# neonnnnn/sparsepoly

Hardware: AMD Instinct MI355X
Metric: pcd_epochs_per_sec (higher is better)
Workload: dtype f32; 1 GPU; BASELINE configs[1]: degree=2 n_components=30 regularizer=squaredl12 solver=pcd fit_linear=True fit_lower=explicit on 1000000x100000 CSR nnz=49987865 (~50/row); schedule=colored, parallelism=single GPU, ranks=1, launcher=external, persistent_fallbacks=0

## Files before the change

### include/spfm.h

```cpp
#ifndef SPFM_H
#define SPFM_H

#include <stdint.h>

#ifdef __cplusplus
extern "C" {
#endif

typedef struct spfm_engine* spfm_handle;

#define SPFM_OK 0
#define SPFM_ERR_INVALID (-1)
#define SPFM_ERR_RUNTIME (-2)
#define SPFM_ERR_UNSUPPORTED (-3)

#define SPFM_F32 0
#define SPFM_F64 1

#define SPFM_LOSS_SQUARED 0
#define SPFM_LOSS_SQUARED_HINGE 1
#define SPFM_LOSS_LOGISTIC 2

#define SPFM_REG_L1 0
#define SPFM_REG_L21 1
#define SPFM_REG_SQUAREDL12 2
#define SPFM_REG_SQUAREDL21 3
#define SPFM_REG_OMEGATI 4
#define SPFM_REG_OMEGACS 5

#define SPFM_SOLVER_PCD 0
#define SPFM_SOLVER_PBCD 1
#define SPFM_SOLVER_PSGD 2

#define SPFM_SCHED_EXACT 0
#define SPFM_SCHED_COLORED 1
#define SPFM_SCHED_COLORED_RLF 2

#define SPFM_MAX_DEGREE 6

int spfm_create(spfm_handle* out, int device_id, int dtype);
void spfm_destroy(spfm_handle h);
const char* spfm_last_error(spfm_handle h);
int spfm_device_name(spfm_handle h, char* out, int cap);
const char* spfm_build_tag(void);

int spfm_set_data_csc(spfm_handle h, int64_t n, int32_t d, const int64_t* indptr,
                      const int32_t* indices, const double* data, const double* y);

int spfm_set_data_csr(spfm_handle h, int64_t n, int32_t d, const int64_t* indptr,
                      const int32_t* indices, const double* data, const double* y);

int spfm_share_data(spfm_handle dst, spfm_handle src, const double* y);

int spfm_set_params(spfm_handle h, int n_orders, int k, int32_t d, const double* P,
                    const double* w, const double* lams);
int spfm_get_params(spfm_handle h, double* P, double* w);

int spfm_configure(spfm_handle h, int solver, int loss, int regularizer, int top_degree);

int spfm_init_pred(spfm_handle h, int degree, int fit_linear, int add_lower_deg2);
int spfm_get_y_pred(spfm_handle h, double* out);
int spfm_loss_sum(spfm_handle h, double* out);

int spfm_predict_csr(spfm_handle h, int64_t n, const int64_t* indptr, const int32_t* indices,
                     const double* data, int degree, int fit_linear, int add_lower_deg2,
                     double* out);

int spfm_set_schedule(spfm_handle h, int mode, const int32_t* indices_feature,
                      const int64_t* conflict_indptr, const int32_t* conflict_indices,
                      int64_t conflict_n_rows, int32_t* order_out, int32_t* n_batches_out);

int spfm_set_schedule_raw(spfm_handle h, const int32_t* order, const int32_t* batch_ptr,
                          int32_t n_batches, const int64_t* conflict_indptr,
                          const int32_t* conflict_indices, int64_t conflict_n_rows);

int spfm_get_schedule(spfm_handle h, int32_t* order_out, int32_t* batch_ptr_out,
                      int32_t* n_batches_out);

int spfm_schedule_build(int mode, int64_t n_rows, int32_t d, const int64_t* indptr,
                        const int32_t* indices, const int32_t* indices_feature, int max_batch,
                        int32_t* order_out, int32_t* batch_ptr_out, int32_t* n_batches_out);


int spfm_cd_linear_epoch(spfm_handle h, double alpha, double* viol);

int spfm_pcd_epoch(spfm_handle h, int order_idx, int degree, double beta, double gamma,
                   double eta, const int32_t* indices_component, int n_comp, double* viol);

int spfm_pbcd_epoch(spfm_handle h, int order_idx, int degree, double beta, double gamma,
                    double eta, double* viol);

int spfm_host_epoch_begin(spfm_handle h, int order_idx, int degree);
int spfm_host_pass_begin(spfm_handle h, int component);
int spfm_host_step_sums(spfm_handle h, int step, double* sums_out);
int spfm_host_step_apply(spfm_handle h, int step, const double* p_new, const double* p_old);
int spfm_host_epoch_end(spfm_handle h, double* viol);

int spfm_psgd_epoch(spfm_handle h, int degree, double alpha, double beta, double gamma,
                    double eta0, int learning_rate, double power_t, int64_t batch_size,
                    const int32_t* indices_samples, int64_t n_samples, int fit_linear,
                    int64_t* it, double* sum_loss);
int spfm_psgd_epoch_sharded(spfm_handle h, int degree, double alpha, double beta, double gamma,
                            double eta0, int learning_rate, double power_t, int64_t batch_size,
                            const int32_t* indices_samples, int64_t n_global, int64_t row_lo,
                            int fit_linear, int64_t* it, double* sum_loss);

int spfm_comm_unique_id(char* id128);
int spfm_comm_init(spfm_handle h, const char* id128, int n_ranks, int rank);
int spfm_comm_init_shm(spfm_handle h, const char* shm_name, int n_ranks, int rank);

int spfm_peer_alloc(spfm_handle h, char* handle64);
int spfm_peer_connect(spfm_handle h, int n_ranks, int rank, const char* handles);

int spfm_profile_enable(spfm_handle h, int on);
int spfm_profile_get(spfm_handle h, int which, double* ms, int64_t* launches, int64_t* nnz);
int spfm_profile_reset(spfm_handle h);
int spfm_set_use_graph(spfm_handle h, int on);

int spfm_set_option(spfm_handle h, const char* key, int value);
int spfm_get_option(spfm_handle h, const char* key, int* value);


int spfm_debug_prb_stamps(spfm_handle h, long long* out, int cap);
int spfm_debug_hop_latency(spfm_handle h, int partner, int rounds, double* ns_per_hop,
                           int* xcc_ids);
int spfm_debug_exchange_cost(spfm_handle h, int groups, int ncols, int readers_mod, int rounds,
                             double* ns_per_round);

int spfm_debug_stream_probe(spfm_handle h, int64_t* bytes_out);
int spfm_debug_write_probe(spfm_handle h, int bytes_per_record, int64_t* bytes_out);
int spfm_debug_branch_counts(spfm_handle h, unsigned* out8, int reset);

#define SPFM_GRAM_ANOVA 0
#define SPFM_GRAM_POLY 1
#define SPFM_GRAM_ALL_SUBSETS 2
#define SPFM_GRAM_MAX_DEGREE 64

int spfm_gram_csr_dense(spfm_handle h, int kind, int degree, int64_t n1, int32_t d,
                        const int64_t* indptr, const int32_t* indices, const double* data,
                        int64_t n2, const double* B, const double* lams, int transpose_out,
                        int64_t max_block_bytes, double* out);
int spfm_gram_csr_csr(spfm_handle h, int kind, int degree, int64_t n1, int32_t d,
                      const int64_t* indptr1, const int32_t* indices1, const double* data1,
                      int64_t n2, const int64_t* indptr2, const int32_t* indices2,
                      const double* data2, const double* lams, int64_t max_block_bytes,
                      double* out);

int spfm_objective_terms(spfm_handle h, int order_idx, int degree, double* out8);

int spfm_set_eval_csr(spfm_handle h, int64_t n, int32_t d, const int64_t* indptr,
                      const int32_t* indices, const double* data, const double* y);
int spfm_eval_loss(spfm_handle h, int degree, int fit_linear, int add_lower_deg2,
                   double* loss_sum, double* y_pred_out);

#define SPFM_INTERACTION_BLOCK_MAX_BYTES (1LL << 30)
int spfm_interaction_stats(spfm_handle h, int order_idx, double tol, int64_t* counts2,
                           double* sums3);
int spfm_interaction_topk(spfm_handle h, int order_idx, int64_t K, int32_t* rows, int32_t* cols,
                          double* vals, int64_t* n_out);
int spfm_interaction_list(spfm_handle h, int order_idx, double tol, int64_t capacity,
                          int32_t* rows, int32_t* cols, double* vals, int64_t* n_out);
int spfm_interaction_values(spfm_handle h, int order_idx, int64_t L, const int32_t* rows,
                            const int32_t* cols, double* vals);
int spfm_interaction_block(spfm_handle h, int order_idx, int64_t nJ, const int32_t* J,
                           int64_t nJ2, const int32_t* J2, double* out);

#define SPFM_INTERACTION3_MAX_ACTIVE (1 << 15)
int spfm_interaction3_stats(spfm_handle h, int order_idx, double tol, int64_t* counts2,
                            double* sums3);
int spfm_interaction3_topk(spfm_handle h, int order_idx, int64_t K, int32_t* i, int32_t* j,
                           int32_t* l, double* vals, int64_t* n_out);
int spfm_interaction3_list(spfm_handle h, int order_idx, double tol, int64_t capacity, int32_t* i,
                           int32_t* j, int32_t* l, double* vals, int64_t* n_out);
int spfm_interaction3_values(spfm_handle h, int order_idx, int64_t L, const int32_t* i,
                             const int32_t* j, const int32_t* l, double* vals);

#ifdef __cplusplus
}
#endif
#endif
```

### sparsepoly_amd/_capi.py

```python
import ctypes as C
import os

import numpy as np



def hip_initialised():
    try:
        for fd in os.listdir("/proc/self/fd"):
            try:
                if os.readlink("/proc/self/fd/" + fd) == "/dev/kfd":
                    return True
            except OSError:
                continue
    except OSError:
        pass
    return False


HIP_INITIALISED_BEFORE_IMPORT = hip_initialised()
QUEUES_SET_BY_PACKAGE = False


def ensure_hw_queues(n_streams):
    global QUEUES_SET_BY_PACKAGE
    import warnings

    need = int(n_streams) + 1
    val = os.environ.get("GPU_MAX_HW_QUEUES")
    have = int(val) if (val and val.isdigit()) else None
    if not hip_initialised():
        if have is None:
            os.environ["GPU_MAX_HW_QUEUES"] = "8"
            QUEUES_SET_BY_PACKAGE = True
            have = 8
        return have
    eff = have if have is not None else 4
    if eff < need and n_streams > 1:
        warnings.warn(
            "sparsepoly_amd: %d concurrent fits, but the HIP runtime of this process was "
            "initialised with %d hardware queues (GPU_MAX_HW_QUEUES %s): fits that share a queue "
            "run one after the other.  Export GPU_MAX_HW_QUEUES=8 before the process first "
            "touches the GPU (PyTorch users: before the first torch.cuda call)."
            % (n_streams, eff, "= %d" % have if have is not None else "unset"),
            RuntimeWarning, stacklevel=3)
    return eff


_HERE = os.path.dirname(os.path.abspath(__file__))
LIB_PATH = os.environ.get("SPFM_HIP_LIB") or os.path.join(_HERE, "lib", "libspfm_hip.so")

SPFM_OK, SPFM_ERR_INVALID, SPFM_ERR_RUNTIME, SPFM_ERR_UNSUPPORTED = 0, -1, -2, -3
DTYPES = {"f32": 0, "f64": 1}
LOSSES = {"squared": 0, "squared_hinge": 1, "logistic": 2}
REGULARIZERS = {"l1": 0, "l21": 1, "squaredl12": 2, "squaredl21": 3, "omegati": 4, "omegacs": 5}
SOLVERS = {"pcd": 0, "pbcd": 1, "psgd": 2}
LEARNING_RATE = {"constant": 0, "optimal": 1, "pegasos": 2, "invscaling": 3}
SCHEDULES = {"exact": 0, "colored": 1, "colored_rlf": 2}
GRAM_KINDS = {"anova": 0, "poly": 1, "all-subsets": 2}
GRAM_MAX_DEGREE = 64

SYMBOLS = [
    "spfm_create", "spfm_destroy", "spfm_last_error", "spfm_device_name", "spfm_build_tag", "spfm_set_data_csc", "spfm_set_data_csr", "spfm_share_data",
    "spfm_set_params", "spfm_get_params", "spfm_configure", "spfm_init_pred", "spfm_get_y_pred",
    "spfm_loss_sum", "spfm_predict_csr", "spfm_set_schedule", "spfm_set_schedule_raw",
    "spfm_get_schedule", "spfm_schedule_build",
    "spfm_cd_linear_epoch",
    "spfm_pcd_epoch", "spfm_pbcd_epoch", "spfm_psgd_epoch", "spfm_psgd_epoch_sharded",
    "spfm_host_epoch_begin",
    "spfm_host_pass_begin", "spfm_host_step_sums", "spfm_host_step_apply", "spfm_host_epoch_end", "spfm_comm_unique_id", "spfm_comm_init", "spfm_comm_init_shm", "spfm_peer_alloc", "spfm_peer_connect",
    "spfm_profile_enable", "spfm_profile_get", "spfm_profile_reset", "spfm_set_use_graph",
    "spfm_set_option", "spfm_get_option", "spfm_debug_prb_stamps", "spfm_debug_hop_latency", "spfm_debug_exchange_cost",
    "spfm_debug_branch_counts", "spfm_debug_stream_probe", "spfm_debug_write_probe",
    "spfm_gram_csr_dense", "spfm_gram_csr_csr",
    "spfm_objective_terms", "spfm_set_eval_csr", "spfm_eval_loss",
    "spfm_interaction_stats", "spfm_interaction_topk", "spfm_interaction_list",
    "spfm_interaction_values", "spfm_interaction_block",
    "spfm_interaction3_stats", "spfm_interaction3_topk", "spfm_interaction3_list",
    "spfm_interaction3_values",
]
INTERACTION_BLOCK_MAX_BYTES = 1 << 30
INTERACTION3_MAX_ACTIVE = 1 << 15

_dp = C.POINTER(C.c_double)
_ip = C.POINTER(C.c_int32)
_lp = C.POINTER(C.c_int64)
_h = C.c_void_p

_lib = None


def load():
    global _lib
    if _lib is not None:
        return _lib
    if not os.path.exists(LIB_PATH):
        raise RuntimeError(
            "sparsepoly_amd: HIP extension %s is missing. Build it with "
            "`python -c 'import __graft_entry__ as g; g.build()'` or "
            "`bash sparsepoly_amd/csrc/build.sh`; there is no CPU fallback." % LIB_PATH
        )
    L = C.CDLL(LIB_PATH)
    L.spfm_create.argtypes = [C.POINTER(_h), C.c_int, C.c_int]
    L.spfm_destroy.argtypes = [_h]
    L.spfm_destroy.restype = None
    L.spfm_last_error.argtypes = [_h]
    L.spfm_last_error.restype = C.c_char_p
    L.spfm_device_name.argtypes = [_h, C.c_char_p, C.c_int]
    L.spfm_build_tag.argtypes = []
    L.spfm_build_tag.restype = C.c_char_p
    L.spfm_set_data_csc.argtypes = [_h, C.c_int64, C.c_int32, _lp, _ip, _dp, _dp]
    L.spfm_set_data_csr.argtypes = [_h, C.c_int64, C.c_int32, _lp, _ip, _dp, _dp]
    L.spfm_share_data.argtypes = [_h, _h, _dp]
    L.spfm_set_params.argtypes = [_h, C.c_int, C.c_int, C.c_int32, _dp, _dp, _dp]
    L.spfm_get_params.argtypes = [_h, _dp, _dp]
    L.spfm_configure.argtypes = [_h, C.c_int, C.c_int, C.c_int, C.c_int]
    L.spfm_init_pred.argtypes = [_h, C.c_int, C.c_int, C.c_int]
    L.spfm_get_y_pred.argtypes = [_h, _dp]
    L.spfm_loss_sum.argtypes = [_h, _dp]
    L.spfm_predict_csr.argtypes = [_h, C.c_int64, _lp, _ip, _dp, C.c_int, C.c_int, C.c_int, _dp]
    L.spfm_set_schedule.argtypes = [_h, C.c_int, _ip, _lp, _ip, C.c_int64, _ip, _ip]
    L.spfm_set_schedule_raw.argtypes = [_h, _ip, _ip, C.c_int32, _lp, _ip, C.c_int64]
    L.spfm_get_schedule.argtypes = [_h, _ip, _ip, _ip]
    L.spfm_schedule_build.argtypes = [C.c_int, C.c_int64, C.c_int32, _lp, _ip, _ip, C.c_int, _ip,
                                      _ip, _ip]
    L.spfm_cd_linear_epoch.argtypes = [_h, C.c_double, _dp]
    L.spfm_pcd_epoch.argtypes = [_h, C.c_int, C.c_int, C.c_double, C.c_double, C.c_double, _ip,
                                 C.c_int, _dp]
    L.spfm_pbcd_epoch.argtypes = [_h, C.c_int, C.c_int, C.c_double, C.c_double, C.c_double, _dp]
    L.spfm_psgd_epoch.argtypes = [_h, C.c_int, C.c_double, C.c_double, C.c_double, C.c_double,
                                  C.c_int, C.c_double, C.c_int64, _ip, C.c_int64, C.c_int, _lp,
                                  _dp]
    L.spfm_psgd_epoch_sharded.argtypes = [_h, C.c_int, C.c_double, C.c_double, C.c_double,
                                          C.c_double, C.c_int, C.c_double, C.c_int64, _ip,
                                          C.c_int64, C.c_int64, C.c_int, _lp, _dp]
    L.spfm_host_epoch_begin.argtypes = [_h, C.c_int, C.c_int]
    L.spfm_host_pass_begin.argtypes = [_h, C.c_int]
    L.spfm_host_step_sums.argtypes = [_h, C.c_int, _dp]
    L.spfm_host_step_apply.argtypes = [_h, C.c_int, _dp, _dp]
    L.spfm_host_epoch_end.argtypes = [_h, _dp]
    L.spfm_comm_unique_id.argtypes = [C.c_char_p]
    L.spfm_comm_init.argtypes = [_h, C.c_char_p, C.c_int, C.c_int]
    L.spfm_comm_init_shm.argtypes = [_h, C.c_char_p, C.c_int, C.c_int]
    L.spfm_profile_enable.argtypes = [_h, C.c_int]
    L.spfm_profile_get.argtypes = [_h, C.c_int, _dp, _lp, _lp]
    L.spfm_profile_reset.argtypes = [_h]
    L.spfm_set_use_graph.argtypes = [_h, C.c_int]
    L.spfm_set_option.argtypes = [_h, C.c_char_p, C.c_int]
    L.spfm_get_option.argtypes = [_h, C.c_char_p, C.POINTER(C.c_int)]
    L.spfm_debug_prb_stamps.argtypes = [_h, _lp, C.c_int]
    L.spfm_debug_hop_latency.argtypes = [_h, C.c_int, C.c_int, _dp, _ip]
    L.spfm_debug_exchange_cost.argtypes = [_h, C.c_int, C.c_int, C.c_int, C.c_int, _dp]
    L.spfm_peer_alloc.argtypes = [_h, C.c_char_p]
    L.spfm_peer_connect.argtypes = [_h, C.c_int, C.c_int, C.c_char_p]
    L.spfm_debug_branch_counts.argtypes = [_h, C.POINTER(C.c_uint32), C.c_int]
    L.spfm_debug_stream_probe.argtypes = [_h, _lp]
    L.spfm_debug_write_probe.argtypes = [_h, C.c_int, _lp]
    L.spfm_gram_csr_dense.argtypes = [_h, C.c_int, C.c_int, C.c_int64, C.c_int32, _lp, _ip, _dp,
                                      C.c_int64, _dp, _dp, C.c_int, C.c_int64, _dp]
    L.spfm_gram_csr_csr.argtypes = [_h, C.c_int, C.c_int, C.c_int64, C.c_int32, _lp, _ip, _dp,
                                    C.c_int64, _lp, _ip, _dp, _dp, C.c_int64, _dp]
    L.spfm_objective_terms.argtypes = [_h, C.c_int, C.c_int, _dp]
    L.spfm_set_eval_csr.argtypes = [_h, C.c_int64, C.c_int32, _lp, _ip, _dp, _dp]
    L.spfm_eval_loss.argtypes = [_h, C.c_int, C.c_int, C.c_int, _dp, _dp]
    L.spfm_interaction_stats.argtypes = [_h, C.c_int, C.c_double, _lp, _dp]
    L.spfm_interaction_topk.argtypes = [_h, C.c_int, C.c_int64, _ip, _ip, _dp, _lp]
    L.spfm_interaction_list.argtypes = [_h, C.c_int, C.c_double, C.c_int64, _ip, _ip, _dp, _lp]
    L.spfm_interaction_values.argtypes = [_h, C.c_int, C.c_int64, _ip, _ip, _dp]
    L.spfm_interaction_block.argtypes = [_h, C.c_int, C.c_int64, _ip, C.c_int64, _ip, _dp]
    L.spfm_interaction3_stats.argtypes = [_h, C.c_int, C.c_double, _lp, _dp]
    L.spfm_interaction3_topk.argtypes = [_h, C.c_int, C.c_int64, _ip, _ip, _ip, _dp, _lp]
    L.spfm_interaction3_list.argtypes = [_h, C.c_int, C.c_double, C.c_int64, _ip, _ip, _ip, _dp,
                                         _lp]
    L.spfm_interaction3_values.argtypes = [_h, C.c_int, C.c_int64, _ip, _ip, _ip, _dp]
    for name in SYMBOLS:
        f = getattr(L, name)
        if name not in ("spfm_destroy", "spfm_last_error", "spfm_build_tag"):
            f.restype = C.c_int
    _lib = L
    return L


def f64(a):
    a = np.ascontiguousarray(a, dtype=np.float64)
    return a, a.ctypes.data_as(_dp)


def i32(a):
    a = np.ascontiguousarray(a, dtype=np.int32)
    return a, a.ctypes.data_as(_ip)


def i64(a):
    a = np.ascontiguousarray(a, dtype=np.int64)
    return a, a.ctypes.data_as(_lp)


def build_tag():
    return load().spfm_build_tag().decode()
```

### sparsepoly_amd/csrc/spfm_engine.hip.h

```cpp
#pragma once
#include <dlfcn.h>
#include <fcntl.h>
#include <sys/mman.h>
#include <unistd.h>
#include <chrono>
#include <hip/hip_runtime.h>

#include <cerrno>
#include <cmath>
#include <cstdio>
#include <cstdlib>
#include <cstring>
#include <atomic>
#include <map>
#include <memory>
#include <mutex>
#include <string>
#include <type_traits>
#include <thread>
#include <vector>

#include "../../include/spfm.h"
#include "spfm_common.hip.h"
#include "spfm_prb.hip.h"
#include "spfm_pcdw.hip.h"
#include "spfm_psgd.hip.h"

namespace spfm {
struct IntArgs;
void schedule_exact(int64_t, int32_t, const int64_t*, const int32_t*, const int32_t*, int,
                    std::vector<int32_t>&);
void schedule_colored(int64_t, int32_t, const int64_t*, const int32_t*, const int32_t*, int,
                      std::vector<int32_t>&, std::vector<int32_t>&);
void schedule_rlf(int64_t, int32_t, const int64_t*, const int32_t*, const int32_t*, int,
                  std::vector<int32_t>&, std::vector<int32_t>&);
bool csr_to_csc(int64_t, int32_t, const int64_t*, const int32_t*, std::vector<int64_t>&,
                std::vector<int32_t>&, std::vector<int64_t>&);
int schedule_threads();
void csc_to_csr(int64_t, int32_t, const int64_t*, const int32_t*, std::vector<int64_t>&,
                std::vector<int32_t>&, std::vector<int64_t>&);
void build_wide_stream(int64_t, const int64_t*, const int32_t*, const std::vector<int32_t>&,
                       const std::vector<int32_t>&, int, std::vector<int32_t>&,
                       std::vector<int32_t>&, std::vector<int32_t>&, std::vector<uint8_t>&);
void build_pb_stream(int64_t, const int64_t*, const int32_t*, const std::vector<int32_t>&,
                     const std::vector<int32_t>&, int, int, bool, const uint8_t*,
                     std::vector<int32_t>&, std::vector<int32_t>&, std::vector<uint8_t>&,
                     std::vector<uint8_t>&);
void build_rowblock_stream(int64_t, const int64_t*, const int32_t*, const std::vector<int32_t>&,
                           const std::vector<int32_t>&, int, int, std::vector<int32_t>&,
                           std::vector<int32_t>&, std::vector<uint32_t>&, const uint8_t*);
void schedule_relax(int64_t, int32_t, const int64_t*, const int32_t*, const int32_t*, int, int,
                    std::vector<int32_t>&, std::vector<int32_t>&, std::vector<int32_t>&,
                    std::vector<int32_t>&, std::vector<int64_t>&, std::vector<int64_t>&,
                    std::vector<int16_t>&, std::vector<uint8_t>&);
template <typename T>
hipError_t device_csr_to_csc(int64_t, int32_t, int64_t, const int64_t*, const int32_t*, const T*,
                             int64_t*, int32_t*, T*, int*, hipStream_t);
extern template hipError_t device_csr_to_csc<float>(int64_t, int32_t, int64_t, const int64_t*,
                                                    const int32_t*, const float*, int64_t*,
                                                    int32_t*, float*, int*, hipStream_t);
extern template hipError_t device_csr_to_csc<double>(int64_t, int32_t, int64_t, const int64_t*,
                                                     const int32_t*, const double*, int64_t*,
                                                     int32_t*, double*, int*, hipStream_t);
hipError_t device_rowblock_stream(int64_t, int32_t, int64_t, int, int, int, const int32_t*,
                                  const int32_t*, const int64_t*, const int32_t*, const uint8_t*,
                                  int32_t*, int32_t*, uint32_t*, int*, int64_t*, hipStream_t);
hipError_t device_pb_stream(int64_t, int32_t, int64_t, int, int, int, int, const int32_t*,
                            const int32_t*, const int64_t*, const int32_t*, const int64_t*,
                            const int32_t*, int32_t*, int32_t*, uint8_t*, uint8_t*, hipStream_t);
hipError_t device_wide_stream(int64_t, int32_t, int64_t, int, int, const int32_t*, const int32_t*,
                              const int64_t*, const int32_t*, const int64_t*, const int32_t*,
                              int32_t*, int32_t*, uint8_t*, hipStream_t);
hipError_t device_first_fit(int64_t, int32_t, int64_t, const int64_t*, const int32_t*, const int64_t*,
                            const int32_t*, int, int32_t*, int*, int*, hipStream_t);
hipError_t device_rlf(int64_t, int32_t, int64_t, const int64_t*, const int32_t*, const int64_t*,
                      const int32_t*, int, std::vector<int32_t>&, std::vector<int32_t>&, int*,
                      hipStream_t);
}

using namespace spfm;
struct IntPass;

typedef struct ncclComm* ncclComm_t;

struct DevBuf {
    struct Block {
        void* p;
        std::atomic<int> refs;
    };
    Block* blk = nullptr;
    void* p = nullptr;
    size_t bytes = 0;
    DevBuf() = default;
    DevBuf(const DevBuf&) = delete;
    DevBuf& operator=(const DevBuf&) = delete;
    ~DevBuf() { release(); }
    void release() {
        if (blk && blk->refs.fetch_sub(1) == 1) {
            (void)hipFree(blk->p);
            delete blk;
        }
        blk = nullptr;
        p = nullptr;
        bytes = 0;
    }
    bool shared() const { return blk && blk->refs.load() > 1; }
    hipError_t alloc(size_t b) {
        if (b <= bytes && p && !shared()) return hipSuccess;
        release();
        if (b == 0) b = 16;
        void* q = nullptr;
        hipError_t e = hipMalloc(&q, b);
        if (e != hipSuccess) return e;
        blk = new Block{q, {1}};
        p = q;
        bytes = b;
        return e;
    }
    void share(const DevBuf& o) {
        if (o.blk == blk) return;
        release();
        if (!o.blk) return;
        o.blk->refs.fetch_add(1);
        blk = o.blk;
        p = o.p;
        bytes = o.bytes;
    }
    template <typename U>
    U* as() const {
        return reinterpret_cast<U*>(p);
    }
};

#define HIPC(expr)                                                                       \
    do {                                                                                 \
        hipError_t _e = (expr);                                                          \
        if (_e != hipSuccess) {                                                          \
            err = std::string(#expr) + ": " + hipGetErrorString(_e);                     \
            return SPFM_ERR_RUNTIME;                                                     \
        }                                                                                \
    } while (0)

#define FAIL(code, msg) \
    do {                \
        err = (msg);    \
        return (code);  \
    } while (0)

#define SPFM_TRY(call)       \
    do {                     \
        int _rc = (call);    \
        if (_rc) return _rc; \
    } while (0)

#define SPFM_GUARD(h)                              \
    if (!(h)) return SPFM_ERR_INVALID;             \
    if (hipSetDevice((h)->device) != hipSuccess) { \
        (h)->err = "hipSetDevice failed";          \
        return SPFM_ERR_RUNTIME;                   \
    }

#define SPFM_DISPATCH(dt, ...)                                    \
    ((dt) == SPFM_F32 ? [&] { using T = float; __VA_ARGS__; }()   \
                      : [&] { using T = double; __VA_ARGS__; }())

static inline unsigned cdiv(int64_t a, int64_t b) { return (unsigned)((a + b - 1) / b); }

struct StreamCache {
    std::mutex mu;
    struct Prb {
        std::string key;
        DevBuf sp, erow, eval, lmask;
        int has_long = 0;
    };
    struct Pb {
        std::string key;
        DevBuf sp, erow, eval, meta, tab;
    };
    std::vector<std::unique_ptr<Prb>> prb;
    std::vector<std::unique_ptr<Pb>> pb;
    static constexpr size_t kKeep = 2;
};

struct ProfSlot {
    std::vector<hipEvent_t> ev;
    size_t used = 0;
    double ms = 0.0;
    int64_t launches = 0, nnz = 0;
};

struct spfm_engine {
    int device = 0, dtype = SPFM_F32;
    hipStream_t stream = nullptr;
    std::string err;
    std::string devname;

    int64_t n = 0, nnz = 0;
    int d = 0;
    bool have_data = false;
    DevBuf cptr, cidx, cval, rptr, ridx, rval, yy, A, col_norm;
    std::vector<int64_t> h_cptr;
    std::vector<int32_t> h_cidx;
    bool col_norm_reduced = false;
    std::shared_ptr<StreamCache> scache;
    uint64_t sched_hash = 0;
    int share_data_from(spfm_engine* src, const double* y);

    int n_orders = 0, k = 0;
    bool have_params = false;
    DevBuf P, Pt, w, lams;
    bool p_valid = true, pt_valid = false;
    std::vector<double> h_lams;

    int solver = -1, loss = 0, reg = 0, top_degree = 0;
    bool configured = false;
    DevBuf norms, cache, dcache;

    std::vector<int32_t> order, batch_ptr;
    DevBuf d_order, d_desc;
    int max_batch_cols = 0;
    bool have_schedule = false;
    int64_t sched_version = 0;

    DevBuf part, delta, pold, viol_col, scalar, ctl, comp_order, pred_tmp, partial, pb_scal,
        pb_ticket;
    bool pbcd_fuse = true;
    double* h_scalar = nullptr;

    DevBuf sg_gradP, sg_gradw, sg_samples, sg_part, sg_cond, sg_thr, sg_theta, sg_done,
        sg_norms, sg_conv, sg_sched, sg_idx, sg_snapP, sg_snapw, sg_snapc;
    bool psgd_force_eager = false;
    int psgd_graph_sweeps = 4;
    bool psgd_warm = false;
    int psgd_redone = 0;
    std::vector<PsgdBatch> h_sched;

    bool use_graph = true;
    bool fuse_chain = true;
    int max_batch_opt = 4096;

    bool pers_failed = false;
    int pers_fallbacks = 0;
    std::string pers_reason;
    int spin_max = 1 << 21;
    int debug_drop = 0;
    bool keep_last_error = false;
    bool have_pred_args = false;
    int pa_degree = 0, pa_lin = 0, pa_lower = 0;
    DevBuf snapP, snapW, snapC;
    std::map<const void*, int> resident_cache;
    std::map<std::string, bool> resident_agreed;

    bool persistent = true;
    int prb_G = 64;
    bool prb_lds = true;
    int prb_lds_active = 0;
    bool y_pm1 = false;
    bool prb_ready = false;
    int prb_has_long = 0;
    int prb_long = kPrbLong;
    DevBuf prb_sp, prb_erow, prb_eval, prb_slab, prb_abort, prow_old, d_bptr, prb_stamps,
        prb_viol, prb_cn, prb_lmask, prb_rec;
    bool prb_pack = true;
    int prb_pack_active = 0;
    bool prb_stamp_on = false;
    int wide_min_cols = 110;
    bool wide_stamp_on = false;
    DevBuf wide_stamps;
    DevBuf w_rec;
    static constexpr size_t kPrbLds = 84 * 1024;
    bool relax_on = true;
    int relax_state = 0;
    std::vector<int32_t> r_batch_ptr;
    int relax_has_long = 0;
    DevBuf r_bptr, r_sp, r_erow, r_eval, r_lmask, r_cfptr, r_cf, r_clist, r_cslab;
    bool wide_on = true;
    int pcdw_G = 0;
    bool wide_ready = false;
    int wide_G = 0, wide_tot = 0;
    int wide_lr_active = 0;
    int wide_lds_cap = -1;
    bool wide_ep = true;
    int wide_ep_active = 0;
    bool wide_rec8 = true;
    DevBuf w_wbase, w_wsp, w_erow, w_eval, w_slabA, w_slabB;
    bool pb_persistent = true;
    int pbprb_G = 256;
    int probe_xcd = 0, probe_lds = 60 * 1024;
    bool pb_stream_ready = false;
    int pb_stream_G = 0, pb_stream_NG = 0;
    DevBuf pb_tab;
    int pbr_state = 0;
    int pbr_G = 0, pb_relax_active = 0;
    std::vector<int32_t> pbr_batch_ptr;
    DevBuf pbr_bptr, pbr_sp, pbr_erow, pbr_eval, pbr_meta, pbr_tab, pbr_cfptr, pbr_cf, pbr_clist,
        pbr_slabR;
    bool pb_balance = true;
    DevBuf pb_sp, pb_erow, pb_eval, pb_meta, pb_slabA, pb_slabB, pb_slabC, pb_stamps, pb_rec;
    bool pb_stamp_on = false;
    int pbprb_active = 0;
    int pb_dbg = 0;
    DevBuf pb_dbgbuf;
    std::map<std::string, hipGraphExec_t> graphs;

    ncclComm_t comm = nullptr;
    struct ShmComm {
        static constexpr size_t kMaxDoubles = 1 << 16;
        struct Hdr {
            volatile int arrive;
            volatile int sense;
            int pad[14];
        };
        Hdr* hdr = nullptr;
        double* slots = nullptr;
        size_t bytes = 0;
        int local_sense = 0;
    } shm;
    std::vector<double> shm_host;
    bool dist() const { return comm != nullptr || shm.hdr != nullptr; }
    int n_ranks = 1, rank = 0;
    static constexpr size_t kPeerPcdOff = 0, kPeerPbOff = 16 * 1024;
    static constexpr size_t kPeerProbeOff = kPeerPbOff + (size_t)2 * 64 * 8 * 64;
    static constexpr size_t kPeerDoubles = kPeerProbeOff + 64;
    int peer_generation = 0;
    void* peer_own = nullptr;
    std::vector<void*> peer_ptr;
    DevBuf peer_tab_pcd, peer_tab_pb;
    bool peer_ready = false;

    bool prof_on = false;
    ProfSlot prof[5];

    ~spfm_engine();

    void clear_graphs() {
        for (auto& kv : graphs) (void)hipGraphExecDestroy(kv.second);
        graphs.clear();
    }

    enum : unsigned {
        kInvPrbStream = 1,
        kInvPbStream = 2,
        kInvWideStream = 4,
        kInvRelax = 8,
        kInvPbRelax = 16,
        kInvSchedule = 32,
        kInvGraphs = 64,
        kInvStreams = kInvPrbStream | kInvPbStream | kInvWideStream,
    };
    void invalidate(unsigned mask) {
        if (mask & kInvPrbStream) prb_ready = false;
        if (mask & kInvPbStream) pb_stream_ready = false;
        if (mask & kInvWideStream) wide_ready = false;
        if (mask & kInvRelax) relax_state = 0;
        if (mask & kInvPbRelax) pbr_state = 0;
        if (mask & kInvSchedule) have_schedule = false;
        if (mask & kInvGraphs) clear_graphs();
    }

    RegState regstate() {
        RegState rs;
        rs.norms = norms.as<double>();
        rs.cache = cache.as<double>();
        rs.dcache = dcache.as<double>();
        return rs;
    }

    size_t tsize() const { return dtype == SPFM_F32 ? 4 : 8; }

    int sync() {
        HIPC(hipStreamSynchronize(stream));
        return SPFM_OK;
    }

    template <typename U>
    int upload_to(void* dst, const U* src, size_t count) {
        if (count) HIPC(hipMemcpyAsync(dst, src, sizeof(U) * count, hipMemcpyHostToDevice, stream));
        return SPFM_OK;
    }
    template <typename U>
    int upload(DevBuf& b, const U* src, size_t count, size_t min_count = 0) {
        HIPC(b.alloc(sizeof(U) * std::max(count, min_count)));
        return upload_to(b.p, src, count);
    }
    template <typename U>
    int download(U* dst, const void* src, size_t count) {
        if (count) HIPC(hipMemcpyAsync(dst, src, sizeof(U) * count, hipMemcpyDeviceToHost, stream));
        return SPFM_OK;
    }

    template <typename T>
    int stage_csr_rows(DevBuf& rp, DevBuf& ri, DevBuf& rv, std::vector<T>& hv,
                       const int64_t* indptr, const int32_t* indices, const double* data,
                       int64_t r0, int64_t r1, size_t min_entries = 0) {
        const int64_t e0 = r0 ? indptr[r0] : 0, ne = indptr[r1] - e0;
        const T* vals;
        if constexpr (std::is_same<T, double>::value) {
            vals = data + e0;
        } else {
            hv.resize((size_t)ne);
            const int nt = (ne >= (1 << 20)) ? schedule_threads() : 1;
            const int64_t per = (ne + nt - 1) / nt;
            auto work = [&](int tid) {
                const int64_t lo = per * tid, hi = std::min<int64_t>(ne, lo + per);
                for (int64_t ii = lo; ii < hi; ++ii) hv[(size_t)ii] = (T)data[e0 + ii];
            };
            std::vector<std::thread> pool;
            for (int t = 1; t < nt; ++t) pool.emplace_back(work, t);
            work(0);
            for (auto& th : pool) th.join();
            vals = hv.data();
        }
        SPFM_TRY(upload(rp, indptr + r0, (size_t)(r1 - r0 + 1)));
        SPFM_TRY(upload(ri, indices + e0, (size_t)ne, min_entries));
        return upload(rv, vals, (size_t)ne, min_entries);
    }

    template <typename T>
    int upload_targets(const double* y, std::vector<T>& hy) {
        hy.resize((size_t)n * 2);
        for (int64_t i = 0; i < n; ++i) {
            hy[(size_t)2 * i] = (T)0;
            hy[(size_t)2 * i + 1] = (T)y[i];
        }
        return upload_to(yy.p, hy.data(), hy.size());
    }

    struct BlockView {
        const double* base;
        int64_t ss, sj;
    };
    BlockView live_block(int order_idx) const {
        const double* img = p_valid ? P.as<double>() : Pt.as<double>();
        return {img + (size_t)order_idx * k * d, p_valid ? (int64_t)d : 1, p_valid ? 1 : (int64_t)k};
    }

    static constexpr size_t kProfPool = 32768;
    bool prof_armed = false;
    void prof_begin(int which, int64_t nnz_launch) {
        prof_armed = false;
        if (!prof_on) return;
        ProfSlot& ps = prof[which];
        if (ps.used + 2 > kProfPool) return;
        if (ps.used + 2 > ps.ev.size()) {
            hipEvent_t a, b;
            if (hipEventCreate(&a) != hipSuccess) return;
            if (hipEventCreate(&b) != hipSuccess) {
                (void)hipEventDestroy(a);
                return;
            }
            ps.ev.push_back(a);
            ps.ev.push_back(b);
        }
        ps.launches++;
        ps.nnz += nnz_launch;
        (void)hipEventRecord(ps.ev[ps.used], stream);
        prof_armed = true;
    }
    void prof_cancel(int which, int64_t nnz_launch) {
        if (!prof_armed) return;
        prof[which].launches--;
        prof[which].nnz -= nnz_launch;
        prof_armed = false;
    }
    void prof_end(int which) {
        if (!prof_armed) return;
        ProfSlot& ps = prof[which];
        (void)hipEventRecord(ps.ev[ps.used + 1], stream);
        ps.used += 2;
        prof_armed = false;
    }
    void prof_collect() {
        if (!prof_on) return;
        (void)hipStreamSynchronize(stream);
        for (auto& ps : prof) {
            for (size_t i = 0; i + 1 < ps.used; i += 2) {
                float ms = 0.f;
                if (hipEventElapsedTime(&ms, ps.ev[i], ps.ev[i + 1]) == hipSuccess) ps.ms += ms;
            }
            ps.used = 0;
        }
    }

    int64_t batch_nnz(int b) const {
        int64_t s = 0;
        for (int q = batch_ptr[b]; q < batch_ptr[b + 1]; ++q)
            s += h_cptr[order[q] + 1] - h_cptr[order[q]];
        return s;
    }

    int shm_barrier();

    int allreduce_shm(double* buf, size_t count);
    int allreduce_shm_piece(double* buf, size_t count);

    int allreduce(double* buf, size_t count);

    int ensure_col_norm();

    int ensure_p();
    int ensure_pt();

    template <typename F>
    int run_cached(const std::string& key, F&& body) {
// ... 19 lines not shown
            if (e != hipSuccess) {
                err = std::string("hipGraphInstantiate: ") + hipGetErrorString(e);
                return SPFM_ERR_RUNTIME;
            }
            it = graphs.emplace(key, ge).first;
        }
        HIPC(hipGraphLaunch(it->second, stream));
        return SPFM_OK;
    }

    template <typename T>
    int upload_images(const int64_t* h_cp, const int32_t* h_ci, const int64_t* h_rp,
                      const int32_t* h_ri, const double* data_csc, const double* data_csr,
                      const int64_t* perm, const double* y);

    template <typename T>
    int set_data_t(const int64_t* indptr, const int32_t* indices, const double* data,
                   const double* y);

    int data_installed(const double* y);

    bool ingest_device = true;
    int ingest_device_used = 0;
    int co_tenants = 1;
    static constexpr int kIngestFallback = 2;
    template <typename T>
    int set_data_csr_device(const int64_t* indptr, const int32_t* indices, const double* data,
                            const double* y);

    int set_data_csr(int64_t n_, int32_t d_, const int64_t* indptr, const int32_t* indices,
                     const double* data, const double* y);

    int set_data(int64_t n_, int32_t d_, const int64_t* indptr, const int32_t* indices,
                 const double* data, const double* y);

    int set_params(int n_orders_, int k_, int32_t d_, const double* P_, const double* w_,
                   const double* lams_);

    int get_params(double* P_, double* w_);

    int configure(int solver_, int loss_, int reg_, int top_degree_);

    int alloc_work();

    bool colour_device = true;
    int colour_device_used = 0;
    bool stream_device = true;
    int stream_device_used = 0;
    int pb_stream_device_used = 0, wide_stream_device_used = 0;
    int colour_columns(int mode, int64_t rows, const int64_t* cp, const int32_t* ci, bool own,
                       const int32_t* jf, int max_batch);

    int set_schedule(int mode, const int32_t* indices_feature, const int64_t* cf_indptr,
                     const int32_t* cf_indices, int64_t cf_rows, int32_t* order_out,
                     int32_t* n_batches_out);

    int install_schedule();

    int set_schedule_raw(const int32_t* order_in, const int32_t* bptr_in, int32_t nb,
                         const int64_t* cf_indptr, const int32_t* cf_indices, int64_t cf_rows);

    int n_batches() const { return (int)batch_ptr.size() - 1; }

    template <typename T, int M>
    void launch_anova(int64_t rows, const int64_t* rp, const int32_t* ri, const T* rv,
                      const double* Pt_o, double* out);
    template <typename T>
    int anova_dispatch(int M, int64_t rows, const int64_t* rp, const int32_t* ri, const T* rv,
                       const double* Pt_o, double* out);

    template <typename T>
    int output_t(int64_t rows, const int64_t* rp, const int32_t* ri, const T* rv, int degree,
                 int fit_linear, int add_lower, double* out);

    template <typename T>
    int init_pred_t(int degree, int fit_linear, int add_lower);

    int init_pred(int degree, int fit_linear, int add_lower);

    template <typename T>
    int get_y_pred_t(double* out);

    template <typename T>
    int loss_sum_t(double* out);

    template <typename T>
    int predict_csr_t(int64_t rows, const int64_t* indptr, const int32_t* indices,
                      const double* data, int degree, int fit_linear, int add_lower,
                      double* out);

    int epoch_prologue();

    int epoch_epilogue(double* viol);

    static std::string fkey(const char* tag, std::initializer_list<double> v,
                            std::initializer_list<int64_t> iv) {
        std::string s(tag);
        char buf[64];
        for (double x : v) {
            snprintf(buf, sizeof buf, "|%a", x);
            s += buf;
        }
        for (int64_t x : iv) {
            snprintf(buf, sizeof buf, "|%lld", (long long)x);
            s += buf;
        }
        return s;
    }

    template <typename T>
    int lin_body(double alpha);

    template <typename T, int LOSS>
    int lin_prb(double alpha);
    template <typename T>
    int lin_prb_loss(double alpha);

    void mark_not_resident(const char* what) {
        pers_failed = true;
        pers_fallbacks += 1;
        pers_reason = std::string(what) + ": its workgroups cannot all be resident on this device";
        if (getenv("SPFM_VERBOSE")) fprintf(stderr, "spfm: fall-back: %s\n", pers_reason.c_str());
    }

    int cd_linear_epoch(double alpha, double* viol);

    template <typename T, int M>
    int pcd_pass_body(int order_idx, double beta, double gamma, double eta);

    bool prb_usable() const {
        return persistent && !pers_failed && (!dist() || peer_ready) && max_batch_cols <= 64 &&
               nnz < ((int64_t)1 << 31) && n > 0;
    }

    bool resident_ok(const void* fn, int threads, size_t lds, int G);
    static constexpr int kNotResident = 1;
    int launch_groups(int G) {
        if (debug_drop > 0 && G > 1) {
            --debug_drop;
            return G - 1;
        }
        return G;
    }
    int snapshot_state(const double* params, size_t count, DevBuf& dst);
    int persistent_aborted(bool* out);
    int recover_from_abort(double* params, size_t count, const DevBuf& src, const char* what);

    template <typename T>
    int ensure_prb();
    template <typename T>
    int build_prb_stream(int nb_);

    PrbArgs prb_args();

    bool relax_candidate() const {
        return relax_on && prb_usable() && !dist() && n_batches() > 0 &&
               (double)d / (double)n_batches() < 12.0;
    }
    template <typename T>
    int ensure_relax();
    PrbArgs relax_args();

    template <typename T, int M, int LOSS>
    int pcd_pass_prb(int order_idx, double beta, double gamma, double eta);

    template <typename T, int M>
    int pcd_prb_loss(int order_idx, double beta, double gamma, double eta);

    template <typename T>
    int pcd_prb_dispatch(int M, int order_idx, double beta, double gamma, double eta);

    int peer_clear(size_t off_doubles, size_t n_doubles);
    int host_barrier();

    bool wide_usable() const {
        return persistent && !pers_failed && wide_on && (!dist() || peer_ready) &&
               max_batch_cols > 64 && max_batch_cols <= 512 && nnz < ((int64_t)1 << 31) && n > 0;
    }

    int wide_groups(int ncu, size_t lds_max) const;

    template <typename T>
    int ensure_wide();

    PcdwArgs wide_args();

    template <typename T, int KIND>
    int wide_launch(PcdwArgs& a, PcdwParams& pp, T* Aptr);

    template <typename T>
    int pcd_pass_wide(int order_idx, double beta, double gamma, double eta);

    template <typename T>
    int lin_wide(double alpha);

    static int kind_of(int degree) { return degree == -1 ? 0 : degree; }
    bool degree_ok(int degree) const {
        return top_degree == -1 ? degree == -1 : (degree >= 2 && degree <= top_degree);
    }

    template <typename T, int M>
    int pcd_precompute_all(int order_idx);
    template <typename T>
    int pcd_precompute_all_dispatch(int M, int order_idx);

    template <typename T>
    int pcd_pass_dispatch(int M, int order_idx, double beta, double gamma, double eta);

    int pcd_epoch(int order_idx, int degree, double beta, double gamma, double eta,
                  const int32_t* ic, int n_comp, double* viol);

    template <typename T, int M, int L, int C>
    int pbcd_body_lc(int order_idx, double beta, double gamma, double eta);

    static bool pbprb_degree_ok(int M) { return M == 0 || M == 2 || M == 3 || M == 4; }
    bool pbprb_usable(int M) const {
        return persistent && !pers_failed && pb_persistent && (!dist() || peer_ready) &&
               max_batch_cols <= 64 && nnz < ((int64_t)1 << 31) && n > 0 && k <= 62 &&
               pbprb_degree_ok(M);
    }

    const char* validate_pb_stream(int G, int NG, const std::vector<int32_t>& gsp,
                                   const std::vector<int32_t>& src,
                                   const std::vector<uint8_t>& meta,
                                   const std::vector<uint8_t>& tab) const;

    template <typename T>
    int ensure_pb_stream(int NG);
    template <typename T>
    int ensure_pb_relax(int NG);

    template <typename T, int M, int L>
    int pbcd_prb_l(int order_idx, double beta, double gamma, double eta);

    template <typename T, int M>
    int pbcd_prb_m(int order_idx, double beta, double gamma, double eta);

    template <typename T>
    int pbcd_prb_dispatch(int M, int order_idx, double beta, double gamma, double eta);

    template <typename T, int M>
    int pbcd_body(int order_idx, double beta, double gamma, double eta);

    template <typename T>
    int pbcd_dispatch(int M, int order_idx, double beta, double gamma, double eta);

    int pbcd_epoch(int order_idx, int degree, double beta, double gamma, double eta,
                   double* viol);

    int host_order = -1, host_degree = 0;
    std::vector<double> host_stage;

    int host_epoch_begin(int order_idx, int degree);
    template <typename T>
    int host_pbcd_precompute(int M, int order_idx);
    int host_pass_begin(int s);
    int host_step_check(int b) {
        if (host_order < 0) FAIL(SPFM_ERR_INVALID, "host step: call spfm_host_epoch_begin first");
        if (b < 0 || b >= n_batches()) FAIL(SPFM_ERR_INVALID, "host step: step index out of range");
        return SPFM_OK;
    }

    template <typename T, int M>
    int host_sums_pcd(int b, double* out);
    template <typename T, int M>
    int host_apply_pcd(int b, const double* p_new);
    template <typename T, int M, int L, int C>
    int host_sums_pbcd(int b, double* out);
    template <typename T, int M, int L, int C>
    int host_apply_pbcd(int b, const double* p_new, const double* p_old);
    template <typename T>
    int host_step_pcd_t(bool sums, int b, double* out, const double* p_new);
    template <typename T>
    int host_step_pbcd_t(bool sums, int b, double* out, const double* p_new, const double* p_old);
    int host_step(bool sums, int b, double* out, const double* p_new, const double* p_old);
    int host_epoch_end(double* viol);

    int configure_psgd(int loss_, int reg_, int top_degree_);

    static void psgd_eta(int lr, double eta0, double alpha, double beta, double power_t,
                         int64_t it, double* eta_P, double* eta_w) {
        if (lr == 0) {
            *eta_P = eta0;
            *eta_w = eta0;
        } else if (lr == 1) {
            const double eta_it = eta0 * (double)it;
            *eta_P = eta0 / std::pow(1.0 + eta_it * beta, power_t);
            *eta_w = eta0 / std::pow(1.0 + eta_it * alpha, power_t);
        } else if (lr == 2) {
            *eta_P = 1.0 / (beta * (double)it);
            *eta_w = 1.0 / (alpha * (double)it);
        } else {
            const double eta = eta0 / std::pow((double)it, power_t);
            *eta_P = eta;
            *eta_w = eta;
        }
    }

    template <typename T, int L>
    int psgd_epoch_tl(int degree, double alpha, double beta, double gamma, double eta0, int lr,
                      double power_t, int64_t batch_size, int fit_linear, int64_t* it);

    int psgd_epoch(int degree, double alpha, double beta, double gamma, double eta0, int lr,
                   double power_t, int64_t batch_size, const int32_t* indices_samples,
                   int64_t n_samples, int64_t row_lo, int fit_linear, int64_t* it, double* sum_loss);
    std::vector<int64_t> sg_lpos;
// ... 95 lines not shown
```

### sparsepoly_amd/csrc/spfm_engine_core.hip

```cpp
#include "spfm_engine.hip.h"
#include "spfm_linear.hip.h"
#include "spfm_predict.hip.h"
#include "spfm_pbcd.hip.h"

using namespace spfm;

static thread_local std::string g_create_error;

namespace {
struct ncclUniqueId_ {
    char internal[128];
};
enum { ncclSum_ = 0 };
enum { ncclFloat64_ = 8 };
struct Rccl {
    void* lib = nullptr;
    int (*GetUniqueId)(ncclUniqueId_*) = nullptr;
    int (*CommInitRank)(ncclComm_t*, int, ncclUniqueId_, int) = nullptr;
    int (*AllReduce)(const void*, void*, size_t, int, int, ncclComm_t, hipStream_t) = nullptr;
    int (*CommDestroy)(ncclComm_t) = nullptr;
    const char* (*GetErrorString)(int) = nullptr;
    const char* (*GetLastError)(ncclComm_t) = nullptr;
    int (*GetVersion)(int*) = nullptr;
    std::string path;
// ... 756 lines not shown
    SPFM_TRY(download(out, o.p, (size_t)rows));
    return sync();
}

int spfm_engine::epoch_prologue() {
    if (!have_data || !have_params || !configured)
        FAIL(SPFM_ERR_INVALID, "epoch: data, parameters and configuration are required");
    if (!have_schedule) FAIL(SPFM_ERR_INVALID, "epoch: call spfm_set_schedule first");
    int rc = ensure_col_norm();
    if (rc) return rc;
    HIPC(hipMemsetAsync(viol_col.p, 0, sizeof(double) * (size_t)d, stream));
    return SPFM_OK;
}

int spfm_engine::epoch_epilogue(double* viol) {
    hipLaunchKernelGGL(reduce_sum_kernel, dim3(1), dim3(kBlock), 0, stream,
                       viol_col.as<double>(), d, scalar.as<double>());
    HIPC(hipGetLastError());
    SPFM_TRY(download(h_scalar, scalar.p, 1));
    HIPC(hipStreamSynchronize(stream));
    prof_collect();
    if (viol) *viol = h_scalar[0];
    return SPFM_OK;
}

bool spfm_engine::resident_ok(const void* fn, int threads, size_t lds, int G) {
    int per_cu = 0;
    auto it = resident_cache.find(fn);
    if (it != resident_cache.end()) {
        per_cu = it->second;
    } else {
        if (hipOccupancyMaxActiveBlocksPerMultiprocessor(&per_cu, fn, threads, lds) !=
            hipSuccess) {
            (void)hipGetLastError();
            per_cu = 1;
        }
        resident_cache[fn] = per_cu;
    }
    int ncu = 0;
    if (hipDeviceGetAttribute(&ncu, hipDeviceAttributeMultiprocessorCount, device) != hipSuccess)
        return true;
    const int64_t sharers = (int64_t)(shm.hdr ? n_ranks : 1) * co_tenants;
    const bool mine = (int64_t)per_cu * ncu >= (int64_t)G * sharers;
    if (!dist()) return mine;
    char key[96];
    snprintf(key, sizeof key, "%p|%d|%lld|%zu", fn, G, (long long)sharers, lds);
    auto ag = resident_agreed.find(key);
    if (ag != resident_agreed.end()) return ag->second;
    double no = mine ? 0.0 : 1.0;
    bool agreed = mine;
    double* slot = scalar.as<double>() + 7;
    if (scalar.p && upload_to(slot, &no, 1) == SPFM_OK && sync() == SPFM_OK &&
        allreduce(slot, 1) == SPFM_OK && download(&no, slot, 1) == SPFM_OK && sync() == SPFM_OK)
        agreed = no == 0.0;
    resident_agreed[key] = agreed;
    return agreed;
}

int spfm_engine::snapshot_state(const double* params, size_t count, DevBuf& dst) {
    HIPC(dst.alloc(sizeof(double) * count));
    HIPC(hipMemcpyAsync(dst.p, params, sizeof(double) * count, hipMemcpyDeviceToDevice, stream));
    const size_t nc = kMaxDegree + 2;
    HIPC(snapC.alloc(sizeof(double) * nc * 3));
    HIPC(hipMemcpyAsync(snapC.p, cache.p, sizeof(double) * nc * 2, hipMemcpyDeviceToDevice,
                        stream));
    HIPC(hipMemcpyAsync(snapC.as<double>() + nc * 2, dcache.p, sizeof(double) * nc,
                        hipMemcpyDeviceToDevice, stream));
    return SPFM_OK;
}

int spfm_engine::persistent_aborted(bool* out) {
    *out = false;
    if (!prb_abort.p) return SPFM_OK;
    unsigned flag = 0;
    SPFM_TRY(download(&flag, prb_abort.p, 1));
    HIPC(hipStreamSynchronize(stream));
    double any = flag ? 1.0 : 0.0;
    if (dist()) {
        double* slot = scalar.as<double>() + 6;
        SPFM_TRY(upload_to(slot, &any, 1));
        HIPC(hipStreamSynchronize(stream));
        SPFM_TRY(allreduce(slot, 1));
        SPFM_TRY(download(&any, slot, 1));
        HIPC(hipStreamSynchronize(stream));
    }
    if (flag) HIPC(hipMemsetAsync(prb_abort.p, 0, sizeof(unsigned) * 4, stream));
    *out = any != 0.0;
    return SPFM_OK;
}

int spfm_engine::recover_from_abort(double* params, size_t count, const DevBuf& src, const char* what) {
    pers_failed = true;
    pers_fallbacks += 1;
    pers_reason = std::string(what) +
                  " timed out waiting for its workgroups (not all resident, or a peer GPU "
                  "did not answer)";
    if (getenv("SPFM_VERBOSE")) fprintf(stderr, "spfm: fall-back: %s\n", pers_reason.c_str());
    if (!have_pred_args)
        FAIL(SPFM_ERR_RUNTIME, pers_reason + "; the model is half-updated (no spfm_init_pred "
                                             "call to recompute y_pred from)");
    const size_t nc = kMaxDegree + 2;
    HIPC(hipMemcpyAsync(params, src.p, sizeof(double) * count, hipMemcpyDeviceToDevice, stream));
    HIPC(hipMemcpyAsync(cache.p, snapC.p, sizeof(double) * nc * 2, hipMemcpyDeviceToDevice,
                        stream));
    HIPC(hipMemcpyAsync(dcache.p, snapC.as<double>() + nc * 2, sizeof(double) * nc,
                        hipMemcpyDeviceToDevice, stream));
    clear_graphs();
    return init_pred(pa_degree, pa_lin, pa_lower);
}

int spfm_engine::peer_clear(size_t off_doubles, size_t n_doubles) {
    if (!peer_ready) return SPFM_OK;
    HIPC(hipMemsetAsync(reinterpret_cast<double*>(peer_own) + off_doubles, 0,
                        sizeof(double) * n_doubles, stream));
    HIPC(hipStreamSynchronize(stream));
    return host_barrier();
}

int spfm_engine::host_barrier() {
    if (shm.hdr) return shm_barrier();
    if (comm) {
        int rc = allreduce(scalar.as<double>() + 4, 1);
        if (rc) return rc;
        HIPC(hipStreamSynchronize(stream));
    }
    return SPFM_OK;
}

extern "C" {

int spfm_create(spfm_handle* out, int device_id, int dtype) {
    if (!out) return SPFM_ERR_INVALID;
    *out = nullptr;
    if (dtype != SPFM_F32 && dtype != SPFM_F64) {
        g_create_error = "dtype must be SPFM_F32 or SPFM_F64";
        return SPFM_ERR_INVALID;
    }
    int ndev = 0;
    hipError_t e = hipGetDeviceCount(&ndev);
    if (e != hipSuccess || ndev == 0) {
        g_create_error = std::string("no HIP device available: ") + hipGetErrorString(e);
        return SPFM_ERR_RUNTIME;
    }
    if (device_id < 0 || device_id >= ndev) {
        g_create_error = "device id out of range";
        return SPFM_ERR_INVALID;
    }
    if ((e = hipSetDevice(device_id)) != hipSuccess) {
        g_create_error = std::string("hipSetDevice: ") + hipGetErrorString(e);
        return SPFM_ERR_RUNTIME;
    }
    spfm_engine* h = new spfm_engine();
    h->device = device_id;
    h->dtype = dtype;
    hipDeviceProp_t prop;
    if (hipGetDeviceProperties(&prop, device_id) == hipSuccess) h->devname = prop.gcnArchName;
    if ((e = hipStreamCreateWithFlags(&h->stream, hipStreamNonBlocking)) != hipSuccess) {
        g_create_error = std::string("hipStreamCreate: ") + hipGetErrorString(e);
        delete h;
        return SPFM_ERR_RUNTIME;
    }
    *out = h;
    return SPFM_OK;
}

void spfm_destroy(spfm_handle h) {
    if (!h) return;
    (void)hipSetDevice(h->device);
    (void)hipStreamSynchronize(h->stream);
    delete h;
}

const char* spfm_last_error(spfm_handle h) { return h ? h->err.c_str() : g_create_error.c_str(); }

#ifndef SPFM_BUILD_TAG
#define SPFM_BUILD_TAG "untagged"
#endif
const char* spfm_build_tag(void) { return SPFM_BUILD_TAG; }

int spfm_device_name(spfm_handle h, char* out, int cap) {
    if (!h || !out || cap <= 0) return SPFM_ERR_INVALID;
    snprintf(out, (size_t)cap, "%s", h->devname.c_str());
    return SPFM_OK;
}

int spfm_set_data_csc(spfm_handle h, int64_t n, int32_t d, const int64_t* indptr,
                      const int32_t* indices, const double* data, const double* y) {
    SPFM_GUARD(h);
    return h->set_data(n, d, indptr, indices, data, y);
}

int spfm_set_data_csr(spfm_handle h, int64_t n, int32_t d, const int64_t* indptr,
                      const int32_t* indices, const double* data, const double* y) {
    SPFM_GUARD(h);
    return h->set_data_csr(n, d, indptr, indices, data, y);
}

int spfm_share_data(spfm_handle dst, spfm_handle src, const double* y) {
    SPFM_GUARD(dst);
    return dst->share_data_from(src, y);
}

int spfm_set_params(spfm_handle h, int n_orders, int k, int32_t d, const double* P,
                    const double* w, const double* lams) {
    SPFM_GUARD(h);
    return h->set_params(n_orders, k, d, P, w, lams);
}

int spfm_get_params(spfm_handle h, double* P, double* w) {
    SPFM_GUARD(h);
    return h->get_params(P, w);
}

int spfm_configure(spfm_handle h, int solver, int loss, int regularizer, int top_degree) {
    SPFM_GUARD(h);
    return h->configure(solver, loss, regularizer, top_degree);
}

int spfm_init_pred(spfm_handle h, int degree, int fit_linear, int add_lower_deg2) {
    SPFM_GUARD(h);
    return h->init_pred(degree, fit_linear, add_lower_deg2);
}

int spfm_get_y_pred(spfm_handle h, double* out) {
    SPFM_GUARD(h);
    if (!h->have_data || !out) return SPFM_ERR_INVALID;
    return SPFM_DISPATCH(h->dtype, return h->get_y_pred_t<T>(out));
}

int spfm_loss_sum(spfm_handle h, double* out) {
    SPFM_GUARD(h);
    if (!h->have_data || !h->configured || !out) {
        h->err = "loss_sum: data and configuration required";
        return SPFM_ERR_INVALID;
    }
    return SPFM_DISPATCH(h->dtype, return h->loss_sum_t<T>(out));
}

int spfm_predict_csr(spfm_handle h, int64_t n, const int64_t* indptr, const int32_t* indices,
                     const double* data, int degree, int fit_linear, int add_lower_deg2,
                     double* out) {
    SPFM_GUARD(h);
    if (!h->have_params) {
        h->err = "predict: no parameters set";
        return SPFM_ERR_INVALID;
    }
    if (n < 0 || !indptr || !out) return SPFM_ERR_INVALID;
    return SPFM_DISPATCH(h->dtype, return h->predict_csr_t<T>(n, indptr, indices, data, degree,
                                                              fit_linear, add_lower_deg2, out));
}

int spfm_set_schedule(spfm_handle h, int mode, const int32_t* indices_feature,
                      const int64_t* conflict_indptr, const int32_t* conflict_indices,
                      int64_t conflict_n_rows, int32_t* order_out, int32_t* n_batches_out) {
    SPFM_GUARD(h);
    return h->set_schedule(mode, indices_feature, conflict_indptr, conflict_indices,
                           conflict_n_rows, order_out, n_batches_out);
}

int spfm_set_schedule_raw(spfm_handle h, const int32_t* order, const int32_t* batch_ptr,
                          int32_t n_batches, const int64_t* conflict_indptr,
                          const int32_t* conflict_indices, int64_t conflict_n_rows) {
    SPFM_GUARD(h);
    return h->set_schedule_raw(order, batch_ptr, n_batches, conflict_indptr, conflict_indices,
                               conflict_n_rows);
}

int spfm_get_schedule(spfm_handle h, int32_t* order_out, int32_t* batch_ptr_out,
                      int32_t* n_batches_out) {
    if (!h) return SPFM_ERR_INVALID;
    if (!h->have_schedule) {
        h->err = "get_schedule: no schedule installed";
        return SPFM_ERR_INVALID;
    }
    if (order_out)
        std::memcpy(order_out, h->order.data(), sizeof(int32_t) * h->order.size());
    if (batch_ptr_out)
        std::memcpy(batch_ptr_out, h->batch_ptr.data(), sizeof(int32_t) * h->batch_ptr.size());
    if (n_batches_out) *n_batches_out = (int32_t)h->batch_ptr.size() - 1;
    return SPFM_OK;
}

int spfm_schedule_build(int mode, int64_t n_rows, int32_t d, const int64_t* indptr,
                        const int32_t* indices, const int32_t* indices_feature, int max_batch,
                        int32_t* order_out, int32_t* batch_ptr_out, int32_t* n_batches_out) {
    if (n_rows < 0 || d <= 0 || !indptr || !indices_feature || !order_out || !batch_ptr_out ||
        !n_batches_out)
        return SPFM_ERR_INVALID;
    if (max_batch <= 0) max_batch = 4096;
    std::vector<char> seen((size_t)d, 0);
    for (int q = 0; q < d; ++q) {
        const int j = indices_feature[q];
        if (j < 0 || j >= d || seen[(size_t)j]) return SPFM_ERR_INVALID;
        seen[(size_t)j] = 1;
    }
    std::vector<int32_t> order, bp;
    if (mode == SPFM_SCHED_EXACT) {
        order.assign(indices_feature, indices_feature + d);
        schedule_exact(n_rows, d, indptr, indices, indices_feature, max_batch, bp);
    } else if (mode == SPFM_SCHED_COLORED) {
        schedule_colored(n_rows, d, indptr, indices, indices_feature, max_batch, order, bp);
    } else if (mode == SPFM_SCHED_COLORED_RLF) {
        schedule_rlf(n_rows, d, indptr, indices, indices_feature, max_batch, order, bp);
    } else {
        return SPFM_ERR_INVALID;
    }
// ... 263 lines not shown
    if (nnz) *nnz = h->prof[which].nnz;
    return SPFM_OK;
}

int spfm_profile_reset(spfm_handle h) {
    if (!h) return SPFM_ERR_INVALID;
    for (auto& ps : h->prof) {
        ps.ms = 0;
        ps.launches = 0;
        ps.nnz = 0;
        ps.used = 0;
    }
    return SPFM_OK;
}

#include "spfm_options.inc.h"

int spfm_debug_prb_stamps(spfm_handle h, long long* out, int cap) {
    SPFM_GUARD(h);
    if ((h->pb_dbg & 8) && out && cap >= 8) {
        static unsigned v[16 + 4096];
        if (hipMemcpy(v, h->pb_dbgbuf.p, sizeof v, hipMemcpyDeviceToHost) != hipSuccess)
            return SPFM_ERR_RUNTIME;
        int i = 0;
        for (; i < 16 + 4096 && i < cap; ++i) out[i] = (long long)v[i];
        return i - (i % 16);
    }
    if (h->wide_stamp_on && h->wide_stamps.p && out) {
        const int nv = (int)(h->wide_stamps.bytes / sizeof(long long));
        if (cap < nv) return SPFM_ERR_INVALID;
        if (hipMemcpy(out, h->wide_stamps.p, sizeof(long long) * (size_t)nv,
                      hipMemcpyDeviceToHost) != hipSuccess)
            return SPFM_ERR_RUNTIME;
        return nv;
    }
    if (h->pb_stamp_on && (h->pb_stream_ready || h->pbr_state == 1) && out) {
        const int nv = 16 * (h->pbr_state == 1 ? h->pbr_G : h->pb_stream_G);
        if (cap < nv) return SPFM_ERR_INVALID;
        if (hipMemcpy(out, h->pb_stamps.p, sizeof(long long) * (size_t)nv,
                      hipMemcpyDeviceToHost) != hipSuccess)
            return SPFM_ERR_RUNTIME;
        return nv;
    }
    if (!h->prb_ready || !out) return SPFM_ERR_INVALID;
    const int nval = 16 * h->prb_G;
    if (cap < nval) return SPFM_ERR_INVALID;
    if (hipMemcpy(out, h->prb_stamps.p, sizeof(long long) * (size_t)nval, hipMemcpyDeviceToHost) !=
        hipSuccess)
        return SPFM_ERR_RUNTIME;
    return nval;
}

int spfm_debug_hop_latency(spfm_handle h, int partner, int rounds, double* ns_per_hop,
                           int* xcc_ids ) {
    SPFM_GUARD(h);
    if (partner < 1 || partner > 255 || rounds < 1 || rounds > (1 << 20) || !ns_per_hop)
        return SPFM_ERR_INVALID;
    DevBuf words, info;
    if (words.alloc(sizeof(unsigned long long) * 32) != hipSuccess ||
        info.alloc(sizeof(int) * 4) != hipSuccess)
        return SPFM_ERR_RUNTIME;
    hipEvent_t e0, e1;
    if (hipEventCreate(&e0) != hipSuccess || hipEventCreate(&e1) != hipSuccess)
        return SPFM_ERR_RUNTIME;
    float best = 1e30f;
    int hinfo[4] = {0, 0, 0, 0};
    for (int rep = 0; rep < 3; ++rep) {
        (void)hipMemsetAsync(words.p, 0, sizeof(unsigned long long) * 32, h->stream);
        (void)hipMemsetAsync(info.p, 0, sizeof(int) * 4, h->stream);
        (void)hipEventRecord(e0, h->stream);
        hipLaunchKernelGGL(hop_pingpong_kernel, dim3(partner + 1), dim3(kWave), 0, h->stream,
                           words.as<unsigned long long>(), rounds, partner, info.as<int>());
        (void)hipEventRecord(e1, h->stream);
        if (hipStreamSynchronize(h->stream) != hipSuccess) {
            h->err = "hop_pingpong_kernel failed";
            return SPFM_ERR_RUNTIME;
        }
        float ms = 0.f;
        (void)hipEventElapsedTime(&ms, e0, e1);
        (void)hipMemcpy(hinfo, info.p, sizeof(int) * 4, hipMemcpyDeviceToHost);
        if (hinfo[2] != 0) {
            h->err = "hop latency probe: partner workgroup did not respond";
            (void)hipEventDestroy(e0);
            (void)hipEventDestroy(e1);
            return SPFM_ERR_RUNTIME;
        }
        if (rep > 0 && ms < best) best = ms;
    }
    (void)hipEventDestroy(e0);
    (void)hipEventDestroy(e1);
    *ns_per_hop = (double)best * 1e6 / (2.0 * rounds);
    if (xcc_ids) {
        xcc_ids[0] = hinfo[0];
        xcc_ids[1] = hinfo[1];
    }
    return SPFM_OK;
}

int spfm_debug_exchange_cost(spfm_handle h, int groups, int ncols, int readers_mod, int rounds,
                             double* ns_per_round) {
    SPFM_GUARD(h);
    if (groups < 1 || groups > 256 || ncols < 1 || ncols > 64 || readers_mod == 0 ||
        rounds < 1 || rounds > (1 << 20) || !ns_per_round)
        return SPFM_ERR_INVALID;
    DevBuf slab, abortw;
    const size_t bytes = sizeof(double) * 2 * (2 * (size_t)groups + 2) * 64 * 2;
    if (slab.alloc(bytes) != hipSuccess || abortw.alloc(16) != hipSuccess) return SPFM_ERR_RUNTIME;
    PrbArgs a{};
    a.G = groups;
    a.slab = slab.as<double>();
    a.abort_flag = abortw.as<unsigned>();
    a.spin_max = 1u << 21;
    hipEvent_t e0, e1;
    if (hipEventCreate(&e0) != hipSuccess || hipEventCreate(&e1) != hipSuccess)
        return SPFM_ERR_RUNTIME;
    (void)hipFuncSetAttribute((const void*)exchange_probe_kernel,
                              hipFuncAttributeMaxDynamicSharedMemorySize, (int)h->kPrbLds);
    float best = 1e30f;
    unsigned aborted = 0;
    for (int rep = 0; rep < 3; ++rep) {
        (void)hipMemsetAsync(slab.p, 0, bytes, h->stream);
        (void)hipMemsetAsync(abortw.p, 0, 16, h->stream);
        (void)hipEventRecord(e0, h->stream);
        hipLaunchKernelGGL(exchange_probe_kernel, dim3(h->probe_xcd ? 8 * groups + 64 : groups),
                           dim3(readers_mod == -12 ? 768 : 512),
                           h->probe_xcd ? (size_t)h->probe_lds : (size_t)h->kPrbLds, h->stream, a,
                           rounds, ncols, readers_mod, h->probe_xcd);
        (void)hipEventRecord(e1, h->stream);
        if (hipStreamSynchronize(h->stream) != hipSuccess) {
            h->err = "exchange_probe_kernel failed";
            return SPFM_ERR_RUNTIME;
        }
        float ms = 0.f;
        (void)hipEventElapsedTime(&ms, e0, e1);
        (void)hipMemcpy(&aborted, abortw.p, sizeof(unsigned), hipMemcpyDeviceToHost);
        if (aborted) break;
        if (rep > 0 && ms < best) best = ms;
    }
    (void)hipEventDestroy(e0);
    (void)hipEventDestroy(e1);
    if (aborted) {
        h->err = "exchange probe timed out (workgroups not co-resident?)";
        return SPFM_ERR_RUNTIME;
    }
    *ns_per_round = (double)best * 1e6 / rounds;
    return SPFM_OK;
}

int spfm_debug_stream_probe(spfm_handle h, int64_t* bytes_out) {
    SPFM_GUARD(h);
    return h->debug_stream_probe(bytes_out);
}

int spfm_debug_write_probe(spfm_handle h, int bytes_per_record, int64_t* bytes_out) {
    SPFM_GUARD(h);
    return h->debug_write_probe(bytes_per_record, bytes_out);
}

int spfm_debug_branch_counts(spfm_handle h, unsigned* out8, int reset) {
    SPFM_GUARD(h);
    if (!out8) return SPFM_ERR_INVALID;
    if (hipStreamSynchronize(h->stream) != hipSuccess) return SPFM_ERR_RUNTIME;
    for (int i = 0; i < BR_COUNT; ++i) out8[i] = 0;
    hipError_t (*const units[])(unsigned*, int) = {
        spfm_branch_counts_pcd,       spfm_branch_counts_prb_f32,   spfm_branch_counts_prb_f64,
        spfm_branch_counts_wide,      spfm_branch_counts_pbcd,      spfm_branch_counts_pbprb_f32,
        spfm_branch_counts_pbprb_f64};
    for (auto unit : units)
        if (unit(out8, reset) != hipSuccess) return SPFM_ERR_RUNTIME;
    return SPFM_OK;
}

int spfm_set_use_graph(spfm_handle h, int on) {
    if (!h) return SPFM_ERR_INVALID;
    h->use_graph = on != 0;
    if (!on) h->clear_graphs();
    return SPFM_OK;
}

}
```

### sparsepoly_amd/csrc/spfm_engine_pcd.hip

```cpp
#include "spfm_engine.hip.h"
#include "spfm_pcd.hip.h"
#include "spfm_linear.hip.h"

using namespace spfm;

template <typename T>
int spfm_engine::lin_body(double alpha) {
    const double mu = loss == SPFM_LOSS_SQUARED ? 1.0 : (loss == SPFM_LOSS_LOGISTIC ? 0.25 : 2.0);
    const int nb = n_batches();
    for (int b = 0; b < nb; ++b) {
        const int c0 = batch_ptr[b], nc = batch_ptr[b + 1] - c0;
        if (nc == 0) continue;
        const int32_t* cols = d_order.as<int32_t>() + c0;
        prof_begin(4, prof_on ? batch_nnz(b) : 0);
        if (!dist()) {
            hipLaunchKernelGGL((lin_fused_kernel<T>), dim3(nc), dim3(kBlock), 0, stream,
                               d_desc.as<ColDesc>() + c0, cidx.as<int32_t>(), cval.as<T>(),
                               yy.as<T>(), loss, w.as<double>(), col_norm.as<double>(), alpha,
                               mu, viol_col.as<double>());
        } else {
            hipLaunchKernelGGL((lin_grad_kernel<T>), dim3(nc), dim3(kBlock), 0, stream, cols,
                               cptr.as<int64_t>(), cidx.as<int32_t>(), cval.as<T>(),
                               yy.as<typename Vec2<T>::type>(), loss, part.as<double>());
            int rc = allreduce(part.as<double>(), (size_t)nc);
            if (rc) return rc;
            hipLaunchKernelGGL((lin_sync_kernel<T>), dim3(nc), dim3(kBlock), 0, stream, cols,
                               cptr.as<int64_t>(), cidx.as<int32_t>(), cval.as<T>(),
                               yy.as<T>(), part.as<double>(), w.as<double>(),
                               col_norm.as<double>(), alpha, mu, viol_col.as<double>());
        }
        prof_end(4);
    }
    HIPC(hipGetLastError());
    return SPFM_OK;
}

int spfm_engine::cd_linear_epoch(double alpha, double* viol) {
    int rc = epoch_prologue();
    if (rc) return rc;
    const bool wide = wide_usable();
    if (wide || prb_usable()) {
        const char* what = wide ? "wide persistent cd_linear pass" : "persistent cd_linear pass";
        rc = snapshot_state(w.as<double>(), (size_t)d, snapW);
        if (rc) return rc;
        if (wide) rc = SPFM_DISPATCH(dtype, return lin_wide<T>(alpha));
        else rc = SPFM_DISPATCH(dtype, return lin_prb_loss<T>(alpha));
        if (rc == kNotResident) {
            mark_not_resident(what);
            return cd_linear_epoch(alpha, viol);
        }
        if (rc) return rc;
        rc = epoch_epilogue(viol);
        if (rc) return rc;
        bool aborted = false;
        rc = persistent_aborted(&aborted);
        if (rc) return rc;
        if (aborted) {
            rc = recover_from_abort(w.as<double>(), (size_t)d, snapW, what);
            if (rc) return rc;
            return cd_linear_epoch(alpha, viol);
        }
        return SPFM_OK;
    }
    const std::string key = fkey("lin", {alpha}, {loss, sched_version});
    rc = run_cached(key, [&]() {
        return SPFM_DISPATCH(dtype, return lin_body<T>(alpha));
    });
    if (rc) return rc;
    return epoch_epilogue(viol);
}

template <typename T, int M>
int spfm_engine::pcd_pass_body(int order_idx, double beta, double gamma, double eta) {
    const double mu = loss == SPFM_LOSS_SQUARED ? 1.0 : (loss == SPFM_LOSS_LOGISTIC ? 0.25 : 2.0);
    double* Po = P.as<double>() + (size_t)order_idx * k * d;
    Ctl* c = ctl.as<Ctl>();
    double* cbuf[2] = {cache.as<double>(), cache.as<double>() + (kMaxDegree + 2)};
    hipLaunchKernelGGL(begin_pass_kernel, dim3(1), dim3(64), 0, stream, c,
                       comp_order.as<int32_t>(), lams.as<double>());
    const size_t a_stride = (size_t)n * Kind<M>::AS;
    if (reg != SPFM_REG_L1) {
        hipLaunchKernelGGL((pcd_compute_cache_kernel<M>), dim3(kCacheBlocks), dim3(kBlock), 0,
                           stream, c, Po, d, reg, partial.as<double>());
        hipLaunchKernelGGL((pcd_cache_combine_kernel<M>), dim3(1), dim3(64), 0, stream, reg,
                           kCacheBlocks, partial.as<double>(), cbuf[0]);
    }
    const int nb = n_batches();
    int par = 0;
    for (int b = 0; b < nb; ++b) {
        const int c0 = batch_ptr[b], nc = batch_ptr[b + 1] - c0;
        if (nc == 0) continue;
        const ColDesc* desc = d_desc.as<ColDesc>() + c0;
        const int64_t bn = prof_on ? batch_nnz(b) : 0;
        prof_begin(0, bn);
        hipLaunchKernelGGL((pcd_grad_kernel<T, M>), dim3(nc), dim3(kBlock), 0, stream, c, desc,
                           cidx.as<int32_t>(), cval.as<T>(), A.as<T>(), a_stride,
                           yy.as<typename Vec2<T>::type>(), Po, d, loss, part.as<double>(),
                           pold.as<double>());
        prof_end(0);
        int rc = allreduce(part.as<double>(), (size_t)2 * nc);
        if (rc) return rc;
        if (nc <= kWave && fuse_chain) {
            prof_begin(1, bn);
            hipLaunchKernelGGL((pcd_chain_sync_kernel<T, M>), dim3(nc), dim3(kBlock), 0, stream,
                               c, desc, nc, Po, d, part.as<double>(), pold.as<double>(), reg,
                               cbuf[par], cbuf[par ^ 1], mu, beta, gamma, eta,
                               cidx.as<int32_t>(), cval.as<T>(), A.as<T>(), a_stride,
                               yy.as<T>(), viol_col.as<double>());
            prof_end(1);
        } else {
            hipLaunchKernelGGL((pcd_chain_kernel<M>), dim3(1), dim3(kWave), 0, stream, c, desc,
                               nc, Po, d, part.as<double>(), pold.as<double>(), reg, cbuf[par],
                               cbuf[par ^ 1], mu, beta, gamma, eta, delta.as<double>(),
                               viol_col.as<double>());
            prof_begin(1, bn);
            hipLaunchKernelGGL((pcd_sync_kernel<T, M>), dim3(nc), dim3(kBlock), 0, stream, c,
                               desc, cidx.as<int32_t>(), cval.as<T>(), A.as<T>(), a_stride,
                               yy.as<T>(), delta.as<double>(), pold.as<double>());
            prof_end(1);
        }
        par ^= 1;
    }
    HIPC(hipGetLastError());
    return SPFM_OK;
}

PrbArgs spfm_engine::prb_args() {
    PrbArgs a;
    a.G = prb_G;
    a.nb = n_batches();
    a.bptr = d_bptr.as<int32_t>();
    a.desc = d_desc.as<ColDesc>();
    a.sp = prb_sp.as<int32_t>();
    a.lmask = prb_lmask.as<uint32_t>();
    a.has_long = prb_has_long;
    a.erow = prb_erow.as<int32_t>();
    a.slab = prb_slab.as<double>();
    a.rows_per = (int)std::max<int64_t>((n + prb_G - 1) / prb_G, 1);
    a.n_rows = (int)n;
    a.abort_flag = prb_abort.as<unsigned>();
    a.spin_max = spin_max;
    a.stamps = prb_stamp_on ? prb_stamps.as<long long>() : nullptr;
    a.n_ranks = peer_ready ? n_ranks : 1;
    a.rank = rank;
    a.xslab = peer_ready ? peer_tab_pcd.as<double*>() : nullptr;
    a.cf_ptr = nullptr;
    a.cf = nullptr;
    a.clist = nullptr;
    a.cslab = nullptr;
    a.rec = nullptr;
    return a;
}

PrbArgs spfm_engine::relax_args() {
    PrbArgs a = prb_args();
    a.nb = (int)r_batch_ptr.size() - 1;
    a.bptr = r_bptr.as<int32_t>();
    a.sp = r_sp.as<int32_t>();
    a.lmask = r_lmask.as<uint32_t>();
    a.has_long = relax_has_long;
    a.erow = r_erow.as<int32_t>();
    a.stamps = nullptr;
    a.cf_ptr = r_cfptr.as<int32_t>();
    a.cf = r_cf.p;
    a.clist = r_clist.as<int16_t>();
    a.cslab = r_cslab.as<double>();
    return a;
}

template <typename T, int M>
int spfm_engine::pcd_precompute_all(int order_idx) {
    if (n == 0) return SPFM_OK;
    pt_valid = false;
    int rc = ensure_pt();
    if (rc) return rc;
    const size_t lds = sizeof(T) * (size_t)Kind<M>::AS * kWave * 33;
    HIPC(hipFuncSetAttribute((const void*)pcd_precompute_all_kernel<T, M>,
                             hipFuncAttributeMaxDynamicSharedMemorySize, (int)lds));
    const int64_t tiles = (n + 31) / 32;
    const unsigned grid = (unsigned)std::min<int64_t>(tiles, 256 * 8);
    hipLaunchKernelGGL((pcd_precompute_all_kernel<T, M>), dim3(grid), dim3(kBlock), lds,
                       stream, n, k, rptr.as<int64_t>(), ridx.as<int32_t>(), rval.as<T>(),
                       Pt.as<double>() + (size_t)order_idx * k * d, A.as<T>());
    HIPC(hipGetLastError());
    return SPFM_OK;
}

template <typename T>
int spfm_engine::pcd_precompute_all_dispatch(int M, int order_idx) {
    switch (M) {
        case 0: return pcd_precompute_all<T, 0>(order_idx);
        case 2: return pcd_precompute_all<T, 2>(order_idx);
        case 3: return pcd_precompute_all<T, 3>(order_idx);
        case 4: return pcd_precompute_all<T, 4>(order_idx);
        case 5: return pcd_precompute_all<T, 5>(order_idx);
        case 6: return pcd_precompute_all<T, 6>(order_idx);
    }
    FAIL(SPFM_ERR_UNSUPPORTED, "degree outside 2..6");
}

template <typename T>
int spfm_engine::pcd_pass_dispatch(int M, int order_idx, double beta, double gamma, double eta) {
    switch (M) {
        case 0: return pcd_pass_body<T, 0>(order_idx, beta, gamma, eta);
        case 2: return pcd_pass_body<T, 2>(order_idx, beta, gamma, eta);
        case 3: return pcd_pass_body<T, 3>(order_idx, beta, gamma, eta);
        case 4: return pcd_pass_body<T, 4>(order_idx, beta, gamma, eta);
        case 5: return pcd_pass_body<T, 5>(order_idx, beta, gamma, eta);
        case 6: return pcd_pass_body<T, 6>(order_idx, beta, gamma, eta);
    }
    FAIL(SPFM_ERR_UNSUPPORTED, "degree outside 2..6");
}

int spfm_engine::pcd_epoch(int order_idx, int degree, double beta, double gamma, double eta,
              const int32_t* ic, int n_comp, double* viol) {
    int rc = epoch_prologue();
    if (rc) return rc;
    if (solver != SPFM_SOLVER_PCD) FAIL(SPFM_ERR_INVALID, "engine is not configured for pcd");
    if (order_idx < 0 || order_idx >= n_orders) FAIL(SPFM_ERR_INVALID, "bad order index");
    if (!degree_ok(degree)) FAIL(SPFM_ERR_INVALID, "bad degree");
    if (!ic || n_comp < 0 || n_comp > k) FAIL(SPFM_ERR_INVALID, "bad indices_component");
    for (int q = 0; q < n_comp; ++q)
        if (ic[q] < 0 || ic[q] >= k) FAIL(SPFM_ERR_INVALID, "indices_component out of range");
    rc = ensure_p();
    if (rc) return rc;
    pt_valid = false;
    if (n_comp > 0)
        SPFM_TRY(upload_to(comp_order.p, ic, (size_t)n_comp));
    HIPC(hipMemsetAsync(ctl.p, 0, sizeof(Ctl), stream));
    const std::string key = fkey("pcd", {beta, gamma, eta},
                                 {order_idx, degree, loss, reg, sched_version});
    const int M = kind_of(degree);
    rc = SPFM_DISPATCH(dtype, return pcd_precompute_all_dispatch<T>(M, order_idx));
    if (rc) return rc;
    bool use_prb = prb_usable();
    bool use_wide = wide_usable() && M == 2;
    const bool pers_epoch = use_prb || use_wide;
    double* Po_epoch = P.as<double>() + (size_t)order_idx * k * d;
    if (pers_epoch) {
        rc = snapshot_state(Po_epoch, (size_t)k * d, snapP);
        if (rc) return rc;
    }
    for (int pass = 0; pass < n_comp; ++pass) {
        rc = SPFM_OK;
        if (use_wide) {
            rc = SPFM_DISPATCH(dtype, return pcd_pass_wide<T>(order_idx, beta, gamma, eta));
        } else if (use_prb) {
            rc = SPFM_DISPATCH(dtype, return pcd_prb_dispatch<T>(M, order_idx, beta, gamma, eta));
        }
        if (rc == kNotResident) {
            mark_not_resident(use_wide ? "wide persistent pcd pass" : "persistent pcd pass");
            use_prb = use_wide = false;
            hipLaunchKernelGGL(unbegin_pass_kernel, dim3(1), dim3(1), 0, stream, ctl.as<Ctl>());
            HIPC(hipGetLastError());
        }
        if (!use_wide && !use_prb) {
            rc = run_cached(key, [&]() {
                return SPFM_DISPATCH(dtype, return pcd_pass_dispatch<T>(M, order_idx, beta, gamma,
                                     eta));
            });
        }
        if (rc) return rc;
    }
    pt_valid = false;
    rc = epoch_epilogue(viol);
    if (rc) return rc;
    if (pers_epoch) {
        bool aborted = false;
        rc = persistent_aborted(&aborted);
        if (rc) return rc;
        if (aborted) {
            rc = recover_from_abort(Po_epoch, (size_t)k * d, snapP,
                                    use_wide ? "wide persistent pcd pass" : "persistent pcd pass");
            if (rc) return rc;
            return pcd_epoch(order_idx, degree, beta, gamma, eta, ic, n_comp, viol);
        }
    }
    return SPFM_OK;
}

int spfm_engine::host_epoch_begin(int order_idx, int degree) {
    int rc = epoch_prologue();
    if (rc) return rc;
    if (solver != SPFM_SOLVER_PCD && solver != SPFM_SOLVER_PBCD)
        FAIL(SPFM_ERR_INVALID, "host-stepped epochs: configure for pcd or pbcd");
    if (order_idx < 0 || order_idx >= n_orders) FAIL(SPFM_ERR_INVALID, "bad order index");
    if (!degree_ok(degree)) FAIL(SPFM_ERR_INVALID, "bad degree");
    const int M = kind_of(degree);
    if (solver == SPFM_SOLVER_PCD) {
        rc = ensure_p();
        if (rc) return rc;
        pt_valid = false;
        HIPC(hipMemsetAsync(ctl.p, 0, sizeof(Ctl), stream));
        rc = SPFM_DISPATCH(dtype, return pcd_precompute_all_dispatch<T>(M, order_idx));
        if (rc) return rc;
        pt_valid = false;
    } else {
        rc = ensure_pt();
        if (rc) return rc;
        p_valid = false;
        rc = SPFM_DISPATCH(dtype, return host_pbcd_precompute<T>(M, order_idx));
        if (rc) return rc;
    }
    host_order = order_idx;
// ... 129 lines not shown
```

### sparsepoly_amd/csrc/spfm_engine_prb.inc.h

```cpp
#include "spfm_engine.hip.h"
#include "spfm_pcd.hip.h"

using namespace spfm;

template <typename T, int LOSS>
int spfm_engine::lin_prb(double alpha) {
    const double mu = loss == SPFM_LOSS_SQUARED ? 1.0 : (loss == SPFM_LOSS_LOGISTIC ? 0.25 : 2.0);
    int rc = ensure_prb<T>();
    if (rc) return rc;
    constexpr bool can_lr = std::is_same<T, float>::value;
    constexpr int LRV = (LOSS == LOSS_SQUARED) ? 1 : 2;
    bool relaxed = false;
    if (relax_candidate()) {
        rc = ensure_relax<T>();
        if (rc) return rc;
        relaxed = relax_state == 1;
    }
    const PrbArgs pa = relaxed ? relax_args() : prb_args();
    int lds_max = 0;
    HIPC(hipDeviceGetAttribute(&lds_max, hipDeviceAttributeMaxSharedMemoryPerBlock, device));
    const size_t lds_lr = sizeof(double) * (kPrbLdsFixed + (relaxed ? kPrbLdsCR : 0)) +
                          (size_t)pa.rows_per * 5 + 16;
    const bool use_lr = can_lr && prb_lds && lds_lr <= (size_t)lds_max && (LRV == 1 || y_pm1);
    const size_t lds_bytes = use_lr ? std::max(lds_lr, kPrbLds) : kPrbLds;
    if constexpr (can_lr) {
        if (use_lr)
            HIPC(hipFuncSetAttribute((const void*)lin_prb_kernel<T, LOSS, LRV>,
                                     hipFuncAttributeMaxDynamicSharedMemorySize,
                                     (int)lds_bytes));
    }
    HIPC(hipFuncSetAttribute((const void*)lin_prb_kernel<T, LOSS, 0>,
                             hipFuncAttributeMaxDynamicSharedMemorySize, (int)kPrbLds));
    hipLaunchKernelGGL(gather_sched_kernel, dim3(cdiv(d, 256)), dim3(256), 0, stream, d,
                       d_desc.as<ColDesc>(), w.as<double>(), prow_old.as<double>());
    HIPC(hipMemsetAsync(prb_slab.p, 0, prb_slab.bytes, stream));
    if (relaxed) HIPC(hipMemsetAsync(r_cslab.p, 0, r_cslab.bytes, stream));
    {
        int prc = peer_clear(kPeerPcdOff, kPeerPbOff);
        if (prc) return prc;
    }
    prof_begin(4, nnz);
    bool launched = false;
    auto launch_cr = [&](auto lr_tag, size_t lds) -> int {
        constexpr int LRc = decltype(lr_tag)::value;
        auto* fn = lin_prb_kernel<T, LOSS, LRc, false, true>;
        HIPC(hipFuncSetAttribute((const void*)fn, hipFuncAttributeMaxDynamicSharedMemorySize,
                                 (int)lds));
        if (!resident_ok((const void*)fn, kPrbThreads, lds, prb_G)) return kNotResident;
        hipLaunchKernelGGL(fn, dim3(launch_groups(prb_G)), dim3(kPrbThreads), lds, stream, pa,
                           r_eval.as<T>(), yy.as<T>(), prow_old.as<double>(),
                           prb_cn.as<double>(), w.as<double>(), alpha, mu,
                           prb_viol.as<double>());
        return SPFM_OK;
    };
    auto launch = [&](auto lr_tag, auto mg_tag, size_t lds) -> int {
        constexpr int LRc = decltype(lr_tag)::value;
        constexpr bool MGc = decltype(mg_tag)::value;
        HIPC(hipFuncSetAttribute((const void*)lin_prb_kernel<T, LOSS, LRc, MGc>,
                                 hipFuncAttributeMaxDynamicSharedMemorySize, (int)lds));
        if (!resident_ok((const void*)lin_prb_kernel<T, LOSS, LRc, MGc>, kPrbThreads, lds, prb_G))
            return kNotResident;
        hipLaunchKernelGGL((lin_prb_kernel<T, LOSS, LRc, MGc>), dim3(launch_groups(prb_G)),
                           dim3(kPrbThreads),
                           lds, stream, pa, prb_eval.as<T>(), yy.as<T>(),
                           prow_old.as<double>(), prb_cn.as<double>(), w.as<double>(), alpha,
                           mu, prb_viol.as<double>());
        return SPFM_OK;
    };
    int lrc = SPFM_OK;
    if (relaxed) {
        launched = true;
        bool done = false;
        if constexpr (can_lr) {
            if (use_lr) {
                lrc = launch_cr(std::integral_constant<int, LRV>{}, lds_bytes);
                done = true;
            }
        }
        if (!done) lrc = launch_cr(std::integral_constant<int, 0>{}, kPrbLds);
    }
    if constexpr (can_lr) {
        if (use_lr && !launched) {
            lrc = pa.n_ranks > 1
                      ? launch(std::integral_constant<int, LRV>{}, std::true_type{}, lds_bytes)
                      : launch(std::integral_constant<int, LRV>{}, std::false_type{}, lds_bytes);
            launched = true;
        }
    }
    if (!launched)
        lrc = pa.n_ranks > 1
                  ? launch(std::integral_constant<int, 0>{}, std::true_type{}, kPrbLds)
                  : launch(std::integral_constant<int, 0>{}, std::false_type{}, kPrbLds);
    if (lrc == kNotResident) prof_cancel(4, nnz);
    if (lrc) return lrc;
    prof_end(4);
    hipLaunchKernelGGL(fold_viol_kernel, dim3(cdiv(d, 256)), dim3(256), 0, stream, d,
                       d_desc.as<ColDesc>(), prb_viol.as<double>(), viol_col.as<double>());
    HIPC(hipGetLastError());
    return SPFM_OK;
}

template <typename T>
int spfm_engine::lin_prb_loss(double alpha) {
    switch (loss) {
        case SPFM_LOSS_SQUARED: return lin_prb<T, LOSS_SQUARED>(alpha);
        case SPFM_LOSS_SQUARED_HINGE: return lin_prb<T, LOSS_SQUARED_HINGE>(alpha);
        default: return lin_prb<T, LOSS_LOGISTIC>(alpha);
    }
}

template <typename T>
int spfm_engine::ensure_prb() {
    if (prb_ready) return SPFM_OK;
    int ncu = 0;
    HIPC(hipDeviceGetAttribute(&ncu, hipDeviceAttributeMultiprocessorCount, device));
    if (prb_G > ncu) prb_G = ncu;
    if (prb_G < 1) prb_G = 1;
    const int nb_ = n_batches();
    std::unique_lock<std::mutex> cache_lock;
    std::string ckey;
    bool hit = false;
    if (scache) {
        ckey = fkey("prb", {}, {(int64_t)sched_hash, prb_G, prb_long, (int64_t)sizeof(T), nb_});
        cache_lock = std::unique_lock<std::mutex>(scache->mu);
        for (auto& e : scache->prb)
            if (e->key == ckey) {
                prb_sp.share(e->sp);
                prb_erow.share(e->erow);
                prb_eval.share(e->eval);
                prb_lmask.share(e->lmask);
                prb_has_long = e->has_long;
                stream_device_used = 2;
                hit = true;
                break;
            }
    }
    if (!hit) {
        int rc = build_prb_stream<T>(nb_);
        if (rc) return rc;
        if (scache) {
            auto e = std::make_unique<StreamCache::Prb>();
            e->key = ckey;
            e->sp.share(prb_sp);
            e->erow.share(prb_erow);
            e->eval.share(prb_eval);
            e->lmask.share(prb_lmask);
            e->has_long = prb_has_long;
            scache->prb.insert(scache->prb.begin(), std::move(e));
            if (scache->prb.size() > StreamCache::kKeep) scache->prb.pop_back();
        }
    }
    if (cache_lock.owns_lock()) cache_lock.unlock();
    HIPC(prb_slab.alloc(sizeof(double) * 2 * ((size_t)prb_G + 1) * 64 * 2));
    HIPC(prb_abort.alloc(sizeof(unsigned) * 4));
    HIPC(prow_old.alloc(sizeof(double) * (size_t)d));
    HIPC(prb_viol.alloc(sizeof(double) * (size_t)d));
    HIPC(prb_cn.alloc(sizeof(double) * (size_t)d));
    HIPC(prb_stamps.alloc(sizeof(long long) * 16 * (size_t)prb_G));
    HIPC(hipMemsetAsync(prb_stamps.p, 0, prb_stamps.bytes, stream));
    HIPC(hipMemsetAsync(prb_abort.p, 0, sizeof(unsigned) * 4, stream));
    HIPC(hipMemsetAsync(prb_slab.p, 0, prb_slab.bytes, stream));
    hipLaunchKernelGGL(gather_sched_kernel, dim3(cdiv(d, 256)), dim3(256), 0, stream, d,
                       d_desc.as<ColDesc>(), col_norm.as<double>(), prb_cn.as<double>());
    HIPC(hipGetLastError());
    HIPC(hipStreamSynchronize(stream));
    prb_ready = true;
    return SPFM_OK;
}

template <typename T>
int spfm_engine::build_prb_stream(int nb_) {
    const size_t nsp = (size_t)prb_G * nb_ * 65 + 1;
    DevBuf d_src;
    HIPC(d_src.alloc(sizeof(int32_t) * (size_t)(nnz > 0 ? nnz : 1)));
    HIPC(prb_sp.alloc(sizeof(int32_t) * nsp));
    HIPC(prb_lmask.alloc(sizeof(uint32_t) * (size_t)prb_G * nb_ * 2));
    stream_device_used = 0;
    if (stream_device && nnz >= (1 << 20)) {
        int hl = 0;
        const hipError_t e = device_rowblock_stream(
            n, d, nnz, prb_G, nb_, prb_long, d_order.as<int32_t>(), d_bptr.as<int32_t>(),
            cptr.as<int64_t>(), cidx.as<int32_t>(), nullptr, prb_sp.as<int32_t>(),
            d_src.as<int32_t>(), prb_lmask.as<uint32_t>(), &hl, nullptr, stream);
        if (e == hipSuccess) {
            prb_has_long = hl;
            stream_device_used = 1;
        } else {
            (void)hipGetLastError();
        }
    }
    std::vector<int32_t> sp, src;
    std::vector<uint32_t> lmask;
    if (!stream_device_used) {
        build_rowblock_stream(n, h_cptr.data(), h_cidx.data(), order, batch_ptr, prb_G,
                              prb_long, sp, src, lmask, nullptr);
        prb_has_long = 0;
        for (uint32_t m : lmask) prb_has_long |= (m != 0u);
        SPFM_TRY(upload_to(prb_lmask.p, lmask.data(), lmask.size()));
    }
    HIPC(prb_erow.alloc(sizeof(int32_t) * (size_t)(nnz > 0 ? nnz : 1)));
    HIPC(prb_eval.alloc(sizeof(T) * (size_t)(nnz > 0 ? nnz : 1)));
    if (!stream_device_used)
        SPFM_TRY(upload_to(prb_sp.p, sp.data(), sp.size()));
    if (nnz > 0) {
        if (!stream_device_used)
            SPFM_TRY(upload_to(d_src.p, src.data(), (size_t)nnz));
        hipLaunchKernelGGL((prb_gather_kernel<T>), dim3(cdiv(nnz, 256)), dim3(256), 0, stream,
                           nnz, d_src.as<int32_t>(), cidx.as<int32_t>(), cval.as<T>(),
                           prb_erow.as<int32_t>(), prb_eval.as<T>());
        HIPC(hipGetLastError());
    }
    HIPC(hipStreamSynchronize(stream));
    return SPFM_OK;
}

template <typename T>
int spfm_engine::ensure_relax() {
    if (relax_state != 0) return SPFM_OK;
    relax_state = -1;
    int rc = ensure_prb<T>();
    if (rc) return rc;
    std::vector<int32_t> cf_ptr, cf_row, cf_qq, sp, src;
    std::vector<int64_t> cf_ia, cf_ib;
    std::vector<int16_t> clist;
    std::vector<uint8_t> skip;
    std::vector<uint32_t> lmask;
    schedule_relax(n, d, h_cptr.data(), h_cidx.data(), order.data(), 64, 64, r_batch_ptr, cf_ptr,
                   cf_row, cf_qq, cf_ia, cf_ib, clist, skip);
    const int nbr = (int)r_batch_ptr.size() - 1;
    if ((double)nbr > 0.6 * (double)n_batches()) return SPFM_OK;
    DevBuf d_src;
    HIPC(r_bptr.alloc(sizeof(int32_t) * r_batch_ptr.size()));
    SPFM_TRY(upload_to(r_bptr.p, r_batch_ptr.data(), r_batch_ptr.size()));
    const size_t nsp_r = (size_t)prb_G * nbr * 65 + 1;
    bool dev_stream = false;
    size_t ne = 0;
    if (stream_device && nnz >= (1 << 20)) {
        DevBuf d_skip;
        HIPC(d_skip.alloc((size_t)nnz));
        SPFM_TRY(upload_to(d_skip.p, skip.data(), (size_t)nnz));
        HIPC(d_src.alloc(sizeof(int32_t) * (size_t)nnz));
        HIPC(r_sp.alloc(sizeof(int32_t) * nsp_r));
        HIPC(r_lmask.alloc(sizeof(uint32_t) * (size_t)prb_G * nbr * 2));
        int hl = 0;
        int64_t tot = 0;
        const hipError_t e = device_rowblock_stream(
            n, d, nnz, prb_G, nbr, prb_long, d_order.as<int32_t>(), r_bptr.as<int32_t>(),
            cptr.as<int64_t>(), cidx.as<int32_t>(), d_skip.as<uint8_t>(), r_sp.as<int32_t>(),
            d_src.as<int32_t>(), r_lmask.as<uint32_t>(), &hl, &tot, stream);
        if (e == hipSuccess) {
            relax_has_long = hl;
            ne = (size_t)tot;
            dev_stream = true;
        } else {
            (void)hipGetLastError();
        }
    }
    if (!dev_stream) {
        build_rowblock_stream(n, h_cptr.data(), h_cidx.data(), order, r_batch_ptr, prb_G,
                              prb_long, sp, src, lmask, skip.data());
        relax_has_long = 0;
        for (uint32_t m : lmask) relax_has_long |= (m != 0u);
        ne = src.size();
    }
    const size_t ncf = cf_row.size();
    std::vector<PrbConf<T>> hcf(ncf ? ncf : 1);
    {
        std::vector<T> hv((size_t)(nnz > 0 ? nnz : 1));
        SPFM_TRY(download(hv.data(), cval.p, (size_t)nnz));
        HIPC(hipStreamSynchronize(stream));
        for (size_t c = 0; c < ncf; ++c) {
            hcf[c].row = cf_row[c];
            hcf[c].qq = cf_qq[c];
            hcf[c].xa = hv[(size_t)cf_ia[c]];
            hcf[c].xb = hv[(size_t)cf_ib[c]];
        }
    }
    if (!dev_stream) {
        HIPC(d_src.alloc(sizeof(int32_t) * (ne ? ne : 1)));
        HIPC(r_sp.alloc(sizeof(int32_t) * sp.size()));
        HIPC(r_lmask.alloc(sizeof(uint32_t) * lmask.size()));
    }
    HIPC(r_erow.alloc(sizeof(int32_t) * (ne ? ne : 1)));
    HIPC(r_eval.alloc(sizeof(T) * (ne ? ne : 1)));
    HIPC(r_cfptr.alloc(sizeof(int32_t) * cf_ptr.size()));
    HIPC(r_cf.alloc(sizeof(PrbConf<T>) * hcf.size()));
    HIPC(r_clist.alloc(sizeof(int16_t) * clist.size() + 16));
    HIPC(r_cslab.alloc(sizeof(double) * 2 * 64 * 8));
    if (!dev_stream) {
        SPFM_TRY(upload_to(r_sp.p, sp.data(), sp.size()));
        SPFM_TRY(upload_to(r_lmask.p, lmask.data(), lmask.size()));
    }
    SPFM_TRY(upload_to(r_cfptr.p, cf_ptr.data(), cf_ptr.size()));
    SPFM_TRY(upload_to(r_cf.p, hcf.data(), hcf.size()));
    SPFM_TRY(upload_to(r_clist.p, clist.data(), clist.size()));
    if (ne > 0) {
        if (!dev_stream)
            SPFM_TRY(upload_to(d_src.p, src.data(), ne));
        hipLaunchKernelGGL((prb_gather_kernel<T>), dim3(cdiv((int64_t)ne, 256)), dim3(256), 0,
                           stream, (int64_t)ne, d_src.as<int32_t>(), cidx.as<int32_t>(),
                           cval.as<T>(), r_erow.as<int32_t>(), r_eval.as<T>());
        HIPC(hipGetLastError());
    }
    HIPC(hipStreamSynchronize(stream));
    relax_state = 1;
    return SPFM_OK;
}

template <typename T, int M, int LOSS>
int spfm_engine::pcd_pass_prb(int order_idx, double beta, double gamma, double eta) {
    const double mu = loss == SPFM_LOSS_SQUARED ? 1.0 : (loss == SPFM_LOSS_LOGISTIC ? 0.25 : 2.0);
    int rc = ensure_prb<T>();
    if (rc) return rc;
    double* Po = P.as<double>() + (size_t)order_idx * k * d;
    Ctl* c = ctl.as<Ctl>();
    double* cb = cache.as<double>();
    constexpr bool can_lr = std::is_same<T, float>::value && Kind<M>::AS <= 2;
    constexpr int LRV = (LOSS == LOSS_SQUARED) ? 1 : 2;
    constexpr bool can_stamp = std::is_same<T, float>::value && M == 2 && LOSS == LOSS_SQUARED;
    constexpr bool can_stamp3 = std::is_same<T, float>::value && M == 3 && LOSS == LOSS_SQUARED;
    if (prb_stamp_on && !((can_stamp && prb_lds) || (can_stamp3 && !prb_lds)))
        FAIL(SPFM_ERR_UNSUPPORTED,
             "prb_stamps: built for float storage, squared loss and degree 2 with prb_lds=1 "
             "or degree 3 with prb_lds=0 only");
    bool relaxed = false;
    if constexpr (M == 2 || M == 3) {
        if (relax_candidate() && !prb_stamp_on) {
            rc = ensure_relax<T>();
            if (rc) return rc;
            relaxed = relax_state == 1;
        }
    }
    PrbArgs pa = relaxed ? relax_args() : prb_args();
    constexpr bool can_pk = std::is_same<T, float>::value && M == 3;
    bool packed = false;
    if (prb_stamp_on && pa.n_ranks > 1)
        FAIL(SPFM_ERR_UNSUPPORTED,
             "prb_stamps: the timer instantiation has no cross-GPU stage (single rank only)");
    int lds_max = 0;
    HIPC(hipDeviceGetAttribute(&lds_max, hipDeviceAttributeMaxSharedMemoryPerBlock, device));
    const size_t lds_lr = sizeof(double) * (kPrbLdsFixed + (relaxed ? kPrbLdsCR : 0)) +
                          (size_t)pa.rows_per * (4 * Kind<M>::AS + (LRV == 1 ? 4 : 5)) + 16;
    const bool use_lr = can_lr && prb_lds && lds_lr <= (size_t)lds_max &&
                        (LRV == 1 || y_pm1);
    const size_t lds_bytes = use_lr ? std::max(lds_lr, kPrbLds) : kPrbLds;
    prb_lds_active = use_lr ? LRV : 0;
    hipLaunchKernelGGL(begin_pass_kernel, dim3(1), dim3(64), 0, stream, c,
                       comp_order.as<int32_t>(), lams.as<double>());
    if (reg != SPFM_REG_L1) {
        hipLaunchKernelGGL((pcd_compute_cache_kernel<M>), dim3(kCacheBlocks), dim3(kBlock), 0,
                           stream, c, Po, d, reg, partial.as<double>());
        hipLaunchKernelGGL((pcd_cache_combine_kernel<M>), dim3(1), dim3(64), 0, stream, reg,
                           kCacheBlocks, partial.as<double>(), cb);
    }
    hipLaunchKernelGGL(snapshot_row_kernel, dim3(cdiv(d, 256)), dim3(256), 0, stream, c, Po, d,
                       d_desc.as<ColDesc>(), prow_old.as<double>());
    HIPC(hipMemsetAsync(prb_slab.p, 0, prb_slab.bytes, stream));
    if (relaxed) HIPC(hipMemsetAsync(r_cslab.p, 0, r_cslab.bytes, stream));
    if constexpr (can_pk) {
        if (!use_lr && !prb_stamp_on && prb_pack) {
            HIPC(prb_rec.alloc(sizeof(float) * 4 * (size_t)n));
            pa.rec = prb_rec.p;
            hipLaunchKernelGGL(prb_pack3_kernel, dim3(cdiv(n, 256)), dim3(256), 0, stream, c, n,
                               (size_t)n * 2, yy.as<float>(), A.as<float>(),
                               prb_rec.as<float4>());
            packed = true;
        }
    }
    {
        int prc = peer_clear(kPeerPcdOff, kPeerPbOff);
        if (prc) return prc;
    }
    prof_begin(0, nnz);
    auto go = [&](auto lr_tag, auto stamp_tag, auto reg_tag) -> int {
        constexpr int LRc = decltype(lr_tag)::value;
        constexpr bool STc = decltype(stamp_tag)::value;
        constexpr int RGc = decltype(reg_tag)::value;
        const size_t lds = (LRc == 1 || LRc == 2) ? lds_bytes : kPrbLds;
        auto launch = [&](auto mg_tag) -> int {
            constexpr bool MGc = decltype(mg_tag)::value;
            HIPC(hipFuncSetAttribute(
                (const void*)pcd_prb_kernel<T, M, LOSS, LRc, STc, RGc, MGc>,
                hipFuncAttributeMaxDynamicSharedMemorySize, (int)lds));
            if (!resident_ok((const void*)pcd_prb_kernel<T, M, LOSS, LRc, STc, RGc, MGc>,
                             kPrbThreads, lds, prb_G))
                return kNotResident;
            hipLaunchKernelGGL((pcd_prb_kernel<T, M, LOSS, LRc, STc, RGc, MGc>),
                               dim3(launch_groups(prb_G)), dim3(kPrbThreads), lds, stream, c, pa, prb_eval.as<T>(),
                               A.as<T>(), (size_t)n * Kind<M>::AS, yy.as<T>(),
                               prow_old.as<double>(), Po, d, reg, cb, mu, beta, gamma, eta,
                               prb_viol.as<double>());
            return SPFM_OK;
        };
        if constexpr (STc) {
            return launch(std::false_type{});
        } else {
            return pa.n_ranks > 1 ? launch(std::true_type{}) : launch(std::false_type{});
        }
    };
    using std::integral_constant;
    int lrc = SPFM_OK;
    bool launched = false;
    if constexpr (M == 2 || M == 3) {
        if (relaxed) {
            auto launch_cr = [&](auto lr_tag) -> int {
                constexpr int LRc = decltype(lr_tag)::value;
                const size_t lds = (LRc == 1 || LRc == 2) ? lds_bytes : kPrbLds;
                auto* fn = pcd_prb_kernel<T, M, LOSS, LRc, false, -1, false, true>;
                HIPC(hipFuncSetAttribute((const void*)fn,
                                         hipFuncAttributeMaxDynamicSharedMemorySize, (int)lds));
                if (!resident_ok((const void*)fn, kPrbThreads, lds, prb_G)) return kNotResident;
                hipLaunchKernelGGL(fn, dim3(launch_groups(prb_G)), dim3(kPrbThreads), lds, stream,
                                   c, pa, r_eval.as<T>(), A.as<T>(), (size_t)n * Kind<M>::AS,
                                   yy.as<T>(), prow_old.as<double>(), Po, d, reg, cb, mu, beta,
                                   gamma, eta, prb_viol.as<double>());
                return SPFM_OK;
            };
            launched = true;
            bool done = false;
            if constexpr (can_lr) {
                if (use_lr) {
                    lrc = launch_cr(integral_constant<int, LRV>{});
                    done = true;
                }
            }
            if constexpr (can_pk) {
                if (!done && packed) {
                    lrc = launch_cr(integral_constant<int, 3>{});
                    done = true;
                }
            }
            if (!done) lrc = launch_cr(integral_constant<int, 0>{});
        }
    }
    if constexpr (can_lr) {
        if (use_lr && !launched) {
            launched = true;
            if constexpr (can_stamp) {
                if (prb_stamp_on)
                    lrc = go(integral_constant<int, LRV>{}, std::true_type{},
                             integral_constant<int, -1>{});
            }
            if (!prb_stamp_on) {
                if (reg == SPFM_REG_L1)
                    lrc = go(integral_constant<int, LRV>{}, std::false_type{},
                             integral_constant<int, REG_L1>{});
                else if (reg == SPFM_REG_OMEGATI)
                    lrc = go(integral_constant<int, LRV>{}, std::false_type{},
                             integral_constant<int, REG_OMEGATI>{});
                else if constexpr (M == 2)
                    lrc = go(integral_constant<int, LRV>{}, std::false_type{},
                             integral_constant<int, REG_SQL12>{});
                else
                    lrc = go(integral_constant<int, LRV>{}, std::false_type{},
                             integral_constant<int, -1>{});
            }
        }
    }
    if constexpr (can_pk) {
        if (!launched && packed) {
            launched = true;
            lrc = go(integral_constant<int, 3>{}, std::false_type{}, integral_constant<int, -1>{});
        }
    }
    if constexpr (can_stamp3) {
        if (!launched && prb_stamp_on) {
            launched = true;
            lrc = go(integral_constant<int, 0>{}, std::true_type{}, integral_constant<int, -1>{});
        }
    }
    if (!launched)
        lrc = go(integral_constant<int, 0>{}, std::false_type{}, integral_constant<int, -1>{});
    prb_pack_active = packed ? 1 : 0;
    if (lrc == kNotResident) prof_cancel(0, nnz);
    if (lrc) return lrc;
    prof_end(0);
    if constexpr (can_pk) {
        if (packed)
            hipLaunchKernelGGL(prb_unpack3_kernel, dim3(cdiv(n, 256)), dim3(256), 0, stream, c, n,
                               (size_t)n * 2, prb_rec.as<float4>(), yy.as<float>(),
                               A.as<float>());
    }
    hipLaunchKernelGGL(fold_viol_kernel, dim3(cdiv(d, 256)), dim3(256), 0, stream, d,
                       d_desc.as<ColDesc>(), prb_viol.as<double>(), viol_col.as<double>());
    HIPC(hipGetLastError());
    return SPFM_OK;
}

template <typename T, int M>
int spfm_engine::pcd_prb_loss(int order_idx, double beta, double gamma, double eta) {
    switch (loss) {
        case SPFM_LOSS_SQUARED:
            return pcd_pass_prb<T, M, LOSS_SQUARED>(order_idx, beta, gamma, eta);
        case SPFM_LOSS_SQUARED_HINGE:
            return pcd_pass_prb<T, M, LOSS_SQUARED_HINGE>(order_idx, beta, gamma, eta);
        default:
            return pcd_pass_prb<T, M, LOSS_LOGISTIC>(order_idx, beta, gamma, eta);
    }
}

template <typename T>
int spfm_engine::pcd_prb_dispatch(int M, int order_idx, double beta, double gamma, double eta) {
    switch (M) {
        case 0: return pcd_prb_loss<T, 0>(order_idx, beta, gamma, eta);
        case 2: return pcd_prb_loss<T, 2>(order_idx, beta, gamma, eta);
        case 3: return pcd_prb_loss<T, 3>(order_idx, beta, gamma, eta);
        case 4: return pcd_prb_loss<T, 4>(order_idx, beta, gamma, eta);
        case 5: return pcd_prb_loss<T, 5>(order_idx, beta, gamma, eta);
        case 6: return pcd_prb_loss<T, 6>(order_idx, beta, gamma, eta);
    }
    FAIL(SPFM_ERR_UNSUPPORTED, "degree outside 2..6");
}


#define SPFM_CAT_(a, b) a##b
#define SPFM_CAT(a, b) SPFM_CAT_(a, b)
SPFM_DEFINE_BRANCH_COUNTS(SPFM_CAT(spfm_branch_counts_prb_, SPFM_TU_TAG))

template int spfm_engine::ensure_prb<SPFM_TU_T>();
template int spfm_engine::lin_prb_loss<SPFM_TU_T>(double);
template int spfm_engine::pcd_prb_dispatch<SPFM_TU_T>(int, int, double, double, double);
```

### sparsepoly_amd/csrc/spfm_ingest.hip

```cpp
#include <hip/hip_runtime.h>

#include <cstdint>
#include <cstring>

#include <rocprim/device/device_radix_sort.hpp>

namespace spfm {

__global__ void ingest_check_kernel(int64_t n, int32_t d, const int64_t* __restrict__ rptr,
                                    const int32_t* __restrict__ ridx, int* __restrict__ flag) {
    const int64_t i = (int64_t)blockIdx.x * blockDim.x + threadIdx.x;
    if (i >= n) return;
    int bad = 0;
    int32_t prev = -1;
    for (int64_t ii = rptr[i]; ii < rptr[i + 1]; ++ii) {
        const int32_t j = ridx[ii];
        bad |= (j <= prev) | (j >= d);
        prev = j;
    }
    if (bad) atomicOr(flag, 1);
}

__global__ void ingest_rows_kernel(int64_t n, int64_t nnz, const int64_t* __restrict__ rptr,
                                   int32_t* __restrict__ pos, int32_t* __restrict__ row) {
// ... 92 lines not shown
    if ((e = hipStreamSynchronize(stream)) != hipSuccess) return done(e);
    return done(hipSuccess);
}

template hipError_t device_csr_to_csc<float>(int64_t, int32_t, int64_t, const int64_t*,
                                             const int32_t*, const float*, int64_t*, int32_t*,
                                             float*, int*, hipStream_t);
template hipError_t device_csr_to_csc<double>(int64_t, int32_t, int64_t, const int64_t*,
                                              const int32_t*, const double*, int64_t*, int32_t*,
                                              double*, int*, hipStream_t);

}

#include <rocprim/device/device_scan.hpp>

namespace spfm {

__device__ __forceinline__ int64_t rbs_lower_bound(const int32_t* __restrict__ a, int64_t lo,
                                                   int64_t hi, int64_t key) {
    while (lo < hi) {
        const int64_t mid = (lo + hi) >> 1;
        if ((int64_t)a[mid] < key) lo = mid + 1;
        else hi = mid;
    }
    return lo;
}

__global__ void rbs_count_kernel(int32_t d, int G, int nb, int64_t rows_per,
                                 const int32_t* __restrict__ order, const int32_t* __restrict__ bptr,
                                 const int64_t* __restrict__ cptr, const int32_t* __restrict__ cidx,
                                 const uint8_t* __restrict__ skip, int32_t* __restrict__ cnt,
                                 int32_t* __restrict__ first) {
    const int64_t t = (int64_t)blockIdx.x * blockDim.x + threadIdx.x;
    if (t >= (int64_t)d * G) return;
    const int pos = (int)(t / G), g = (int)(t % G);
    int blo = 0, bhi = nb;
    while (bhi - blo > 1) {
        const int mid = (blo + bhi) >> 1;
        if (bptr[mid] <= pos) blo = mid;
        else bhi = mid;
    }
    const int b = blo, q = pos - bptr[b];
    const int32_t j = order[pos];
    const int64_t cb = cptr[j], ce = cptr[j + 1];
    const int64_t lo = rbs_lower_bound(cidx, cb, ce, (int64_t)g * rows_per);
    const int64_t hi = rbs_lower_bound(cidx, lo, ce, (int64_t)(g + 1) * rows_per);
    first[t] = (int32_t)lo;
    int32_t m = (int32_t)(hi - lo);
    if (skip)
        for (int64_t ii = lo; ii < hi; ++ii) m -= skip[ii] ? 1 : 0;
    cnt[((size_t)g * nb + b) * 65 + q] = m;
}

__global__ void rbs_fill_kernel(int32_t d, int G, int nb, const int32_t* __restrict__ bptr,
                                const int64_t* __restrict__ cptr, const int32_t* __restrict__ cidx,
                                const int32_t* __restrict__ order, int64_t rows_per,
                                const uint8_t* __restrict__ skip,
                                const int32_t* __restrict__ cnt, const int32_t* __restrict__ sp,
                                const int32_t* __restrict__ first, int32_t* __restrict__ src) {
    const int64_t t = (int64_t)blockIdx.x * blockDim.x + threadIdx.x;
    if (t >= (int64_t)d * G) return;
    const int pos = (int)(t / G), g = (int)(t % G);
    int blo = 0, bhi = nb;
    while (bhi - blo > 1) {
        const int mid = (blo + bhi) >> 1;
        if (bptr[mid] <= pos) blo = mid;
        else bhi = mid;
    }
    const size_t at = ((size_t)g * nb + blo) * 65 + (size_t)(pos - bptr[blo]);
    const int32_t m = cnt[at], dst = sp[at], lo = first[t];
    if (!skip) {
        for (int32_t u = 0; u < m; ++u) src[(size_t)dst + u] = lo + u;
    } else {
        const int32_t j = order[pos];
        const int64_t hi = rbs_lower_bound(cidx, lo, cptr[j + 1], (int64_t)(g + 1) * rows_per);
        int32_t u = 0;
        for (int64_t ii = lo; ii < hi; ++ii)
            if (!skip[ii]) src[(size_t)dst + u++] = (int32_t)ii;
    }
}

__global__ void rbs_lmask_kernel(int G, int nb, int long_thresh, const int32_t* __restrict__ bptr,
                                 const int32_t* __restrict__ cnt, uint32_t* __restrict__ lmask,
                                 int* __restrict__ any_long) {
    const int64_t t = (int64_t)blockIdx.x * blockDim.x + threadIdx.x;
    if (t >= (int64_t)G * nb) return;
    const int b = (int)(t % nb);
    const int ncols = bptr[b + 1] - bptr[b];
    uint32_t m0 = 0u, m1 = 0u;
    for (int q = 0; q < ncols && q < 64; ++q)
        if (cnt[(size_t)t * 65 + q] > long_thresh) {
            if (q < 32) m0 |= 1u << q;
            else m1 |= 1u << (q - 32);
        }
    lmask[(size_t)t * 2] = m0;
    lmask[(size_t)t * 2 + 1] = m1;
    if (m0 | m1) atomicOr(any_long, 1);
}

hipError_t device_rowblock_stream(int64_t n, int32_t d, int64_t nnz, int G, int nb, int long_thresh,
                                  const int32_t* order, const int32_t* bptr, const int64_t* cptr,
                                  const int32_t* cidx, const uint8_t* skip, int32_t* sp, int32_t* src,
                                  uint32_t* lmask, int* has_long, int64_t* n_entries,
                                  hipStream_t stream) {
    *has_long = 0;
    hipError_t e;
    int32_t *cnt = nullptr, *first = nullptr;
    int* flag = nullptr;
    void* temp = nullptr;
    auto done = [&](hipError_t rc) {
        (void)hipFree(cnt);
        (void)hipFree(first);
        (void)hipFree(flag);
        (void)hipFree(temp);
        return rc;
    };
    const int64_t rows_per = (n + G - 1) / G > 0 ? (n + G - 1) / G : 1;
    const size_t nsp = (size_t)G * nb * 65 + 1;
    const int64_t pairs = (int64_t)d * G;
    if ((e = hipMalloc(&cnt, sizeof(int32_t) * nsp)) != hipSuccess) return done(e);
    if ((e = hipMalloc(&first, sizeof(int32_t) * (size_t)(pairs > 0 ? pairs : 1))) != hipSuccess)
        return done(e);
    if ((e = hipMalloc(&flag, sizeof(int))) != hipSuccess) return done(e);
    if ((e = hipMemsetAsync(cnt, 0, sizeof(int32_t) * nsp, stream)) != hipSuccess) return done(e);
    if ((e = hipMemsetAsync(flag, 0, sizeof(int), stream)) != hipSuccess) return done(e);
    const unsigned blocks = (unsigned)((pairs + 255) / 256);
    hipLaunchKernelGGL(rbs_count_kernel, dim3(blocks), dim3(256), 0, stream, d, G, nb, rows_per,
                       order, bptr, cptr, cidx, skip, cnt, first);
    size_t temp_bytes = 0;
    if ((e = rocprim::exclusive_scan(nullptr, temp_bytes, cnt, sp, (int32_t)0, nsp,
                                     rocprim::plus<int32_t>(), stream)) != hipSuccess)
        return done(e);
    if ((e = hipMalloc(&temp, temp_bytes ? temp_bytes : 16)) != hipSuccess) return done(e);
    if ((e = rocprim::exclusive_scan(temp, temp_bytes, cnt, sp, (int32_t)0, nsp,
                                     rocprim::plus<int32_t>(), stream)) != hipSuccess)
        return done(e);
    hipLaunchKernelGGL(rbs_fill_kernel, dim3(blocks), dim3(256), 0, stream, d, G, nb, bptr, cptr, cidx,
                       order, rows_per, skip, cnt, sp, first, src);
    hipLaunchKernelGGL(rbs_lmask_kernel, dim3((unsigned)(((int64_t)G * nb + 255) / 256)), dim3(256),
                       0, stream, G, nb, long_thresh, bptr, cnt, lmask, flag);
    if ((e = hipGetLastError()) != hipSuccess) return done(e);
    int32_t total = 0;
    if ((e = hipMemcpyAsync(has_long, flag, sizeof(int), hipMemcpyDeviceToHost, stream)) !=
            hipSuccess ||
        (e = hipMemcpyAsync(&total, sp + (nsp - 1), sizeof(int32_t), hipMemcpyDeviceToHost,
                            stream)) != hipSuccess ||
        (e = hipStreamSynchronize(stream)) != hipSuccess)
        return done(e);
    if (n_entries) *n_entries = total;
    (void)nnz;
    return done(hipSuccess);
}



__global__ void sb_step_of_kernel(int32_t d, int nb, const int32_t* __restrict__ order,
                                  const int32_t* __restrict__ bptr, int32_t* __restrict__ step_of) {
    const int pos = blockIdx.x * blockDim.x + threadIdx.x;
    if (pos >= d) return;
    int blo = 0, bhi = nb;
    while (bhi - blo > 1) {
        const int mid = (blo + bhi) >> 1;
        if (bptr[mid] <= pos) blo = mid;
        else bhi = mid;
    }
    step_of[order[pos]] = blo;
}

__device__ __forceinline__ int sb_row_in_step(const int64_t* __restrict__ rptr,
                                              const int32_t* __restrict__ ridx,
                                              const int32_t* __restrict__ step_of, int32_t row,
                                              int step) {
    if (step < 0) return 0;
    int hit = 0;
    for (int64_t c = rptr[row]; c < rptr[row + 1]; ++c) hit |= (step_of[ridx[c]] == step);
    return hit;
}

__global__ void pbs_count_kernel(int32_t d, int G, int nb, int64_t rows_per,
                                 const int32_t* __restrict__ order, const int32_t* __restrict__ bptr,
                                 const int64_t* __restrict__ cptr, const int32_t* __restrict__ cidx,
                                 int32_t* __restrict__ cnt ,
                                 int32_t* __restrict__ first) {
    const int64_t t = (int64_t)blockIdx.x * blockDim.x + threadIdx.x;
    if (t >= (int64_t)d * G) return;
    const int pos = (int)(t / G), g = (int)(t % G);
    int blo = 0, bhi = nb;
    while (bhi - blo > 1) {
        const int mid = (blo + bhi) >> 1;
        if (bptr[mid] <= pos) blo = mid;
        else bhi = mid;
    }
    const int b = blo, q = pos - bptr[b];
    const int32_t j = order[pos];
    const int64_t cb = cptr[j], ce = cptr[j + 1];
    const int64_t lo = rbs_lower_bound(cidx, cb, ce, (int64_t)g * rows_per);
    const int64_t hi = rbs_lower_bound(cidx, lo, ce, (int64_t)(g + 1) * rows_per);
    first[t] = (int32_t)lo;
    cnt[((size_t)g * nb + b) * 64 + q] = (int32_t)(hi - lo);
}

__global__ void pbs_assign_kernel(int G, int nb, int NG, int balance,
                                  const int32_t* __restrict__ bptr, const int32_t* __restrict__ cnt,
                                  uint8_t* __restrict__ tab ,
                                  int32_t* __restrict__ gcnt ,
                                  int32_t* __restrict__ soff ,
                                  uint8_t* __restrict__ where ) {
    const int64_t t = (int64_t)blockIdx.x * blockDim.x + threadIdx.x;
    if (t >= (int64_t)G * nb) return;
    const int b = (int)(t % nb);
    const int QM = 64 / NG;
    const int nc = bptr[b + 1] - bptr[b];
    const int nc2 = b + 2 < nb ? bptr[b + 3] - bptr[b + 2] : 0;
    const int nw = min(64, max(nc, nc2));
    const int32_t* c = cnt + (size_t)t * 64;
    uint8_t* tb = tab + (size_t)t * 64;
    int32_t* gc = gcnt + (size_t)t * (NG + 1);
    int32_t* so = soff + (size_t)t * 64;
    uint8_t* wh = where + (size_t)t * 64;
    int load[16], used[16];
    for (int r = 0; r < NG; ++r) load[r] = used[r] = 0;
    for (int z = 0; z < 64; ++z) tb[z] = 0xFF;
    if (!balance) {
        for (int q = 0; q < nw; ++q) {
            const int r = q % NG, tt = q / NG;
            tb[r * QM + tt] = (uint8_t)q;
            wh[q] = (uint8_t)((r << 3) | tt);
            load[r] += q < nc ? c[q] : 0;
        }
    } else {
        uint8_t idx[64];
        for (int q = 0; q < nw; ++q) {
            const int cq = q < nc ? c[q] : 0;
            int z = q;
            while (z > 0) {
                const int pz = idx[z - 1];
                if ((pz < nc ? c[pz] : 0) >= cq) break;
                idx[z] = idx[z - 1];
                --z;
            }
            idx[z] = (uint8_t)q;
        }
        for (int z = 0; z < nw; ++z) {
            const int q = idx[z];
            int best = -1;
            for (int r = 0; r < NG; ++r)
                if (used[r] < QM && (best < 0 || load[r] < load[best])) best = r;
            tb[best * QM + used[best]] = (uint8_t)q;
            wh[q] = (uint8_t)((best << 3) | used[best]);
            used[best]++;
            load[best] += q < nc ? c[q] : 0;
        }
    }
    for (int r = 0; r < NG; ++r) {
        gc[r] = load[r];
        int at = 0;
        for (int tt = 0; tt < QM; ++tt) {
            const int q = tb[r * QM + tt];
            if (q == 0xFF) continue;
            so[q] = at;
            at += q < nc ? c[q] : 0;
        }
    }
    gc[NG] = 0;
}

__global__ void pbs_fill_kernel(int32_t d, int G, int nb, int NG, const int32_t* __restrict__ bptr,
                                const int32_t* __restrict__ cidx, const int32_t* __restrict__ cnt,
                                const int32_t* __restrict__ gsp, const int32_t* __restrict__ soff,
                                const uint8_t* __restrict__ where,
                                const int32_t* __restrict__ first, const int64_t* __restrict__ rptr,
                                const int32_t* __restrict__ ridx,
                                const int32_t* __restrict__ step_of, int32_t* __restrict__ src,
                                uint8_t* __restrict__ meta) {
    const int64_t t = (int64_t)blockIdx.x * blockDim.x + threadIdx.x;
    if (t >= (int64_t)d * G) return;
    const int pos = (int)(t / G), g = (int)(t % G);
    int blo = 0, bhi = nb;
    while (bhi - blo > 1) {
        const int mid = (blo + bhi) >> 1;
        if (bptr[mid] <= pos) blo = mid;
        else bhi = mid;
    }
    const int b = blo, q = pos - bptr[b];
    const size_t gb = (size_t)g * nb + b;
    const int32_t m = cnt[gb * 64 + q], lo = first[t];
    const int w = where[gb * 64 + q];
    const int32_t dst = gsp[gb * (NG + 1) + (w >> 3)] + soff[gb * 64 + q];
    for (int32_t u = 0; u < m; ++u) {
        src[(size_t)dst + u] = lo + u;
        const int hz = sb_row_in_step(rptr, ridx, step_of, cidx[lo + u], b - 1);
        meta[(size_t)dst + u] = (uint8_t)((w & 7) | (hz ? 0x80 : 0));
    }
}

hipError_t device_pb_stream(int64_t n, int32_t d, int64_t nnz, int G, int nb, int NG, int balance,
                            const int32_t* order, const int32_t* bptr, const int64_t* cptr,
                            const int32_t* cidx, const int64_t* rptr, const int32_t* ridx,
                            int32_t* gsp, int32_t* src, uint8_t* meta, uint8_t* tab,
                            hipStream_t stream) {
    hipError_t e;
    int32_t *cnt = nullptr, *first = nullptr, *gcnt = nullptr, *soff = nullptr, *step_of = nullptr;
    uint8_t* where = nullptr;
    void* temp = nullptr;
    auto done = [&](hipError_t rc) {
        (void)hipFree(cnt);
// ... 135 lines not shown
```

### sparsepoly_amd/csrc/spfm_prb.hip.h

```cpp
#pragma once
#include "spfm_common.hip.h"
#include "spfm_pcd.hip.h"

namespace spfm {


struct PrbArgs {
    int G;
    int nb;
    const int32_t* bptr;
    const ColDesc* desc;
    const int32_t* sp;
    const uint32_t* lmask;
    int has_long;
    const int32_t* erow;
    double* slab;
    int rows_per;
    int n_rows;
    unsigned* abort_flag;
    unsigned spin_max;
    long long* stamps;
    int n_ranks, rank;
    double* const* xslab;
    const int32_t* cf_ptr;
    const void* cf;
    const int16_t* clist;
    double* cslab;
    void* rec;
};

template <typename T>
struct __attribute__((aligned(8))) PrbConf {
    int32_t row;
    int32_t qq;
    T xa, xb;
};


__device__ __forceinline__ void st_agent(double* p, double v) {
    __hip_atomic_store(reinterpret_cast<unsigned long long*>(p),
                       (unsigned long long)__double_as_longlong(v), __ATOMIC_RELAXED,
                       __HIP_MEMORY_SCOPE_AGENT);
}
__device__ __forceinline__ double ld_agent(const double* p) {
    const unsigned long long u =
        __hip_atomic_load(reinterpret_cast<const unsigned long long*>(p), __ATOMIC_RELAXED,
                          __HIP_MEMORY_SCOPE_AGENT);
    return __longlong_as_double((long long)u);
}

__device__ __forceinline__ unsigned long long prb_tag(int b) {
    return (unsigned long long)(((b >> 1) % 3) + 1);
}
__device__ __forceinline__ void prb_store_granule(double* p, double v, unsigned long long tag) {
    const unsigned long long u =
        ((unsigned long long)__double_as_longlong(v) & ~3ull) | tag;
    __hip_atomic_store(reinterpret_cast<unsigned long long*>(p), u, __ATOMIC_RELAXED,
                       __HIP_MEMORY_SCOPE_AGENT);
}
__device__ __forceinline__ unsigned long long prb_load_granule(const double* p) {
    return __hip_atomic_load(reinterpret_cast<const unsigned long long*>(p), __ATOMIC_RELAXED,
                             __HIP_MEMORY_SCOPE_AGENT);
}

__device__ __forceinline__ void prb_store_granule_l2(double* p, double v, unsigned long long tag) {
    const unsigned long long u =
        ((unsigned long long)__double_as_longlong(v) & ~3ull) | tag;
    asm volatile("global_store_dwordx2 %0, %1, off" ::"v"(p), "v"(u) : "memory");
}

__device__ __forceinline__ void prb_store_granule_sys(double* p, double v, unsigned long long tag) {
    const unsigned long long u =
        ((unsigned long long)__double_as_longlong(v) & ~3ull) | tag;
    __hip_atomic_store(reinterpret_cast<unsigned long long*>(p), u, __ATOMIC_RELAXED,
                       __HIP_MEMORY_SCOPE_SYSTEM);
}
__device__ __forceinline__ unsigned long long prb_load_granule_sys(const double* p) {
    return __hip_atomic_load(reinterpret_cast<const unsigned long long*>(p), __ATOMIC_RELAXED,
                             __HIP_MEMORY_SCOPE_SYSTEM);
}

template <int NV>
__device__ __forceinline__ bool prb_cross_gpu(const PrbArgs& a, int g, int b, int lane,
                                              double* tot) {
    const unsigned long long tag = prb_tag(b);
    const size_t par_off = (size_t)(b & 1) * a.n_ranks * 64 * 2;
    if (g == 0) {
        for (int rr = 0; rr < a.n_ranks; ++rr) {
            double* dst = a.xslab[rr] + par_off + ((size_t)a.rank * 64 + lane) * 2;
#pragma unroll
            for (int v = 0; v < NV; ++v) prb_store_granule_sys(dst + v, tot[v], tag);
        }
    }
    const double* mine = a.xslab[a.rank] + par_off + (size_t)lane * 2;
    double acc[NV];
#pragma unroll
    for (int v = 0; v < NV; ++v) acc[v] = 0.0;
    for (int rr = 0; rr < a.n_ranks; ++rr) {
        unsigned long long t[NV];
        unsigned spins = 0;
        for (;;) {
            bool all = true;
#pragma unroll
            for (int v = 0; v < NV; ++v) {
                t[v] = prb_load_granule_sys(mine + (size_t)rr * 64 * 2 + v);
                all = all && ((t[v] & 3ull) == tag);
            }
            if (all) break;
            if ((++spins & 63u) == 0) {
                if (__hip_atomic_load(a.abort_flag, __ATOMIC_RELAXED, __HIP_MEMORY_SCOPE_AGENT) ||
                    spins > a.spin_max) {
                    __hip_atomic_store(a.abort_flag, 1u, __ATOMIC_RELAXED,
                                       __HIP_MEMORY_SCOPE_AGENT);
                    return false;
                }
            }
        }
#pragma unroll
        for (int v = 0; v < NV; ++v) acc[v] += __longlong_as_double((long long)(t[v] & ~3ull));
    }
#pragma unroll
    for (int v = 0; v < NV; ++v) tot[v] = acc[v];
    return true;
}

typedef unsigned __attribute__((ext_vector_type(4))) prb_u4;

__device__ __forceinline__ void prb_load_pairs8(const double* const* p, prb_u4* r) {
    asm volatile(
        "global_load_dwordx4 %0, %8, off sc1\n\t"
        "global_load_dwordx4 %1, %9, off sc1\n\t"
        "global_load_dwordx4 %2, %10, off sc1\n\t"
        "global_load_dwordx4 %3, %11, off sc1\n\t"
        "global_load_dwordx4 %4, %12, off sc1\n\t"
        "global_load_dwordx4 %5, %13, off sc1\n\t"
        "global_load_dwordx4 %6, %14, off sc1\n\t"
        "global_load_dwordx4 %7, %15, off sc1\n\t"
        "s_waitcnt vmcnt(0)"
        : "=&v"(r[0]), "=&v"(r[1]), "=&v"(r[2]), "=&v"(r[3]), "=&v"(r[4]), "=&v"(r[5]),
          "=&v"(r[6]), "=&v"(r[7])
        : "v"(p[0]), "v"(p[1]), "v"(p[2]), "v"(p[3]), "v"(p[4]), "v"(p[5]), "v"(p[6]), "v"(p[7])
        : "memory");
}

template <int NV>
__device__ __forceinline__ bool prb_collect_quarter(const PrbArgs& a, int b, int w, int lane,
                                                    int ncols, double* out ,
                                                    int nparts = 4) {
    const double* slab = a.slab + (size_t)(b & 1) * a.G * 64 * 2;
    const unsigned long long tag = prb_tag(b);
    const int g0 = (a.G * w) / nparts, g1 = (a.G * (w + 1)) / nparts;
    double tot[NV];
#pragma unroll
    for (int v = 0; v < NV; ++v) tot[v] = 0.0;
    bool ok = true;
    if (lane < ncols) {
        const double* sl = slab + (size_t)lane * 2;
        constexpr int GU = 8;
        for (int gg = g0; gg < g1; gg += GU) {
            unsigned long long t[GU][NV];
            unsigned spins = 0;
            for (;;) {
                bool all = true;
                if constexpr (NV == 2) {
                    const double* ptr[GU];
                    prb_u4 r[GU];
#pragma unroll
                    for (int u = 0; u < GU; ++u)
                        ptr[u] = sl + (size_t)((gg + u < g1) ? gg + u : g1 - 1) * 128;
                    prb_load_pairs8(ptr, r);
#pragma unroll
                    for (int u = 0; u < GU; ++u) {
                        t[u][0] = ((unsigned long long)r[u].y << 32) | r[u].x;
                        t[u][1] = ((unsigned long long)r[u].w << 32) | r[u].z;
                        all = all && ((t[u][0] & 3ull) == tag) && ((t[u][1] & 3ull) == tag);
                    }
                } else {
#pragma unroll
                    for (int u = 0; u < GU; ++u)
#pragma unroll
                        for (int v = 0; v < NV; ++v) {
                            const bool in = gg + u < g1;
                            t[u][v] = in ? prb_load_granule(sl + (size_t)(gg + u) * 128 + v) : tag;
                            all = all && ((t[u][v] & 3ull) == tag);
                        }
                }
                if (all) break;
                if ((++spins & 63u) == 0) {
                    if (__hip_atomic_load(a.abort_flag, __ATOMIC_RELAXED,
                                          __HIP_MEMORY_SCOPE_AGENT) ||
                        spins > a.spin_max) {
                        __hip_atomic_store(a.abort_flag, 1u, __ATOMIC_RELAXED,
                                           __HIP_MEMORY_SCOPE_AGENT);
                        ok = false;
                        break;
                    }
                }
            }
            if (!ok) break;
#pragma unroll
            for (int u = 0; u < GU; ++u)
#pragma unroll
                for (int v = 0; v < NV; ++v)
                    if (gg + u < g1) tot[v] += __longlong_as_double((long long)(t[u][v] & ~3ull));
        }
    }
#pragma unroll
    for (int v = 0; v < NV; ++v) out[((size_t)w * 64 + lane) * 2 + v] = tot[v];
    return ok;
}

constexpr int PRB_PF = 4;
constexpr int kPrbLong = 48;
template <typename T>
struct PrbEntries {
    int e0, e1;
    int row[PRB_PF];
    T x[PRB_PF];
};

__device__ __forceinline__ void prb_load_sp(const PrbArgs& a, int g, int b, int slot, int ncols,
                                            int& e0, int& e1, unsigned long long& lmask) {
    e0 = 0;
    e1 = 0;
    lmask = 0ull;
    const int32_t* spb = a.sp + ((size_t)g * a.nb + b) * 65;
    if (a.has_long) {
        const uint32_t* lm = a.lmask + ((size_t)g * a.nb + b) * 2;
        lmask = ((unsigned long long)lm[1] << 32) | (unsigned long long)lm[0];
        if (slot < ncols && !((lmask >> slot) & 1ull)) {
            e0 = spb[slot];
            e1 = spb[slot + 1];
        }
    } else if (slot < ncols) {
        e0 = spb[slot];
        e1 = spb[slot + 1];
    }
}

__device__ __forceinline__ int nth_set_bit(unsigned long long m, int q) {
    for (int t = 0; t < q; ++t) m &= m - 1;
    return __builtin_ctzll(m);
}

template <typename T>
__device__ __forceinline__ void prb_load_entries(const PrbArgs& a, const T* __restrict__ eval,
                                                 int e0, int e1, int sub, PrbEntries<T>& en,
                                                 int pad_row = 0) {
    en.e0 = e0;
    en.e1 = e1;
#pragma unroll
    for (int u = 0; u < PRB_PF; ++u) {
        const int e = e0 + sub + 4 * u;
        const bool v = e < e1;
        en.row[u] = v ? a.erow[e] : pad_row;
        en.x[u] = v ? eval[e] : (T)0;
    }
}

constexpr int kPrbThreads = 512;
constexpr int kPrbParts = 8;
constexpr int kPrbLdsFixed = 2560;

template <int NV>
__device__ __forceinline__ bool prb_poll(const PrbArgs& a, const double* p, unsigned long long tag,
                                         double* out);

__device__ __forceinline__ void pcd_sync_entry_rec(size_t i, double x, double p_old, double upd,
                                                   double lam, float4* __restrict__ rec) {
    const float4 r = rec[i];
    const double a1 = (double)r.z, a2 = (double)r.w;
    const double d1 = x * (a1 - p_old * x);
    const double d2 = x * (a2 - p_old * d1);
    float4 o;
    o.x = (float)((double)r.x - lam * upd * d2);
    o.y = r.y;
    o.z = (float)(a1 - upd * x);
    o.w = (float)(a2 - upd * d1);
    rec[i] = o;
}

static __global__ void prb_pack3_kernel(const Ctl* __restrict__ ctl, int64_t n, size_t a_stride,
                                 const float* __restrict__ yy, const float* __restrict__ A_all,
                                 float4* __restrict__ rec) {
    const int64_t i = (int64_t)blockIdx.x * blockDim.x + threadIdx.x;
    if (i < n) {
        const float* A = A_all + (size_t)ctl->s * a_stride;
        float4 r;
        r.x = yy[2 * i];
        r.y = yy[2 * i + 1];
        r.z = A[2 * i];
        r.w = A[2 * i + 1];
        rec[i] = r;
    }
}
static __global__ void prb_unpack3_kernel(const Ctl* __restrict__ ctl, int64_t n, size_t a_stride,
                                   const float4* __restrict__ rec, float* __restrict__ yy,
                                   float* __restrict__ A_all) {
    const int64_t i = (int64_t)blockIdx.x * blockDim.x + threadIdx.x;
    if (i < n) {
        float* A = A_all + (size_t)ctl->s * a_stride;
        const float4 r = rec[i];
        yy[2 * i] = r.x;
        A[2 * i] = r.z;
        A[2 * i + 1] = r.w;
    }
}

constexpr int kPrbLdsCR = 256;
template <typename T, int M, int LOSS, int LR, bool STAMP = false, int REGC = -1, bool MG = false,
          bool CR = false>
__global__ __launch_bounds__(kPrbThreads) void pcd_prb_kernel(
    const Ctl* __restrict__ ctl, PrbArgs a, const T* __restrict__ eval, T* __restrict__ A_all,
    size_t a_stride, T* __restrict__ yy, const double* __restrict__ pold_sched,
    double* __restrict__ P, int d, int reg, const double* __restrict__ cache_in, double mu,
    double beta, double gamma, double eta, double* __restrict__ viol_pos) {
    T* __restrict__ A = A_all + (size_t)ctl->s * a_stride;
    extern __shared__ __attribute__((aligned(16))) double dyn_lds[];
    double* sh_delta = dyn_lds + 128;
    double* sh_pold = dyn_lds + 192;
    double* sh_chain = dyn_lds + 256;
    double* sh_quart = dyn_lds + 1536;
    int* sh_ok = reinterpret_cast<int*>(dyn_lds + 768);
    int* sh_go = reinterpret_cast<int*>(dyn_lds + 770);
    const typename Vec2<T>::type* yy2 = reinterpret_cast<const typename Vec2<T>::type*>(yy);
    const int g = blockIdx.x;
    const int tid = threadIdx.x, lane = tid & 63, wave = tid >> 6;
    const bool control = wave == 0;
    const bool worker = wave >= 1 && wave <= 4;
    const int part = worker ? wave - 1 : (control ? 4 : wave);
    const int wt = tid - 64;
    const int slot = worker ? (wt >> 2) : 64, sub = wt & 3;
    const int s = ctl->s;
    const double lam = ctl->lam;
    double* ps = P + (size_t)s * d;
    double cache[M + 1];
#pragma unroll
    for (int t = 0; t <= M; ++t) cache[t] = cache_in[t];

    double* sh_long = dyn_lds + 1024;
    constexpr bool LDSR = (LR == 1 || LR == 2);
    constexpr bool PK = (LR == 3);
    static_assert(!LDSR || (Kind<M>::AS <= 2 && sizeof(T) == 4 &&
                            (LR == 2 || LOSS == LOSS_SQUARED)),
                  "LDS-resident rows: float storage, one or two cache values per row");
    static_assert(!PK || (sizeof(T) == 4 && Kind<M>::AS == 2),
                  "packed row records: float storage, two cache values per row");
    float4* __restrict__ rec = reinterpret_cast<float4*>(a.rec);
    constexpr int AS = Kind<M>::AS;
    static_assert(!CR || (M >= 2 && !MG && !STAMP), "relaxed runs: degree >= 2, single GPU");
    constexpr int CSN = 2 + Kind<M>::AS;
    constexpr int CSS = 8;
    const int row0 = LDSR ? g * a.rows_per : 0;
    double* sh_ce = dyn_lds + kPrbLdsFixed;
    double* sh_cv = sh_ce + 128;
    T* lds_a = reinterpret_cast<T*>(dyn_lds + kPrbLdsFixed + (CR ? kPrbLdsCR : 0));
    T* lds_r = lds_a + (size_t)a.rows_per * AS;
    unsigned char* lds_s = reinterpret_cast<unsigned char*>(lds_r + a.rows_per);
    if constexpr (LDSR) {
        const int nr = min(a.rows_per, a.n_rows - row0);
        for (int il = tid; il < nr; il += kPrbThreads) {
            const typename Vec2<T>::type yv = yy2[(size_t)(row0 + il)];
#pragma unroll
            for (int t = 0; t < AS; ++t) lds_a[il * AS + t] = A[(size_t)(row0 + il) * AS + t];
            if constexpr (LR == 1) {
                lds_r[il] = (T)((double)yv.x - (double)yv.y);
            } else {
                lds_r[il] = yv.x;
                lds_s[il] = yv.y > (T)0 ? 1 : 0;
            }
        }
        __syncthreads();
    }
    PrbEntries<T> cur, nxt;
    int c0 = a.bptr[0], c1 = a.bptr[1];
    int c2 = (a.nb > 1) ? a.bptr[2] : c1;
    int c3 = (a.nb > 2) ? a.bptr[3] : c2;
    unsigned long long lm0 = 0ull, lm1 = 0ull;
    {
        int e0, e1;
        prb_load_sp(a, g, 0, slot, c1 - c0, e0, e1, lm0);
        prb_load_entries<T>(a, eval, e0, e1, sub, cur, row0);
    }
    int ne0 = 0, ne1 = 0;
    if (a.nb > 1) prb_load_sp(a, g, 1, slot, c2 - c1, ne0, ne1, lm1);
    double p_slot = (slot < c1 - c0) ? pold_sched[c0 + slot] : 0.0;
    if (tid == 0) {
        *sh_ok = 1;
        *sh_go = 0;
    }
    int cp0 = 0, cp1 = 0, cp2 = 0, cp3 = 0;
    PrbConf<T> cfc, cfn;
    cfc.row = cfn.row = 0;
    cfc.qq = cfn.qq = 0;
    cfc.xa = cfc.xb = cfn.xa = cfn.xb = (T)0;
    prb_u4 clq = {~0u, ~0u, ~0u, ~0u}, clqn = {~0u, ~0u, ~0u, ~0u};
    if constexpr (CR) {
        if (control) {
            const PrbConf<T>* cfa = reinterpret_cast<const PrbConf<T>*>(a.cf);
            cp0 = a.cf_ptr[0];
            cp1 = a.cf_ptr[min(1, a.nb)];
            cp2 = a.cf_ptr[min(2, a.nb)];
            cp3 = a.cf_ptr[min(3, a.nb)];
            if (lane < cp1 - cp0) cfc = cfa[cp0 + lane];
            if (lane < c1 - c0)
                clq = reinterpret_cast<const prb_u4*>(a.clist)[c0 + lane];
        }
    }
    long long acc[8] = {0, 0, 0, 0, 0, 0, 0, 0};
    long long tprev = STAMP ? clock64() : 0;
#define PRB_STAMP(k)                        \
    if constexpr (STAMP) {                  \
        if (tid == 0) {                     \
            const long long tn = clock64(); \
            acc[k] += tn - tprev;           \
            tprev = tn;                     \
        }                                   \
    }
#define PRB_HSTAMP(k)                       \
    if constexpr (STAMP) {                  \
        if (tid == 320) {                   \
            const long long tn = clock64(); \
            acc[k] += tn - tprev;           \
            tprev = tn;                     \
        }                                   \
    }
#define PRB_WSTAMP(k)                       \
    if constexpr (STAMP) {                  \
        if (tid == 64) {                    \
            const long long tn = clock64(); \
            acc[k] += tn - tprev;           \
            tprev = tn;                     \
        }                                   \
    }

    for (int b = 0; b < a.nb; ++b) {
        const int ncols = c1 - c0;
        const int c4 = (b + 4 <= a.nb) ? a.bptr[b + 4] : c3;
        __builtin_amdgcn_s_waitcnt(0x0F70);
        double av[PRB_PF][AS];
        double yh[PRB_PF], yt[PRB_PF], dlast[PRB_PF];
        double pl = 0.0;
        int jl = 0;
        double cst[CSN];
#pragma unroll
        for (int t = 0; t < CSN; ++t) cst[t] = 0.0;
        if (control) {
            if (lane < ncols) {
                pl = pold_sched[c0 + lane];
                if (g == 0) jl = a.desc[c0 + lane].j;
            }
            if constexpr (CR) {
                const int nc = cp1 - cp0, ncw = max(nc, cp3 - cp2);
                const unsigned long long ctag = prb_tag(b);
                double* cs = a.cslab + ((size_t)(b & 1) * 64 + lane) * CSS;
                if (lane < nc) {
                    const int i = cfc.row;
                    if (i / a.rows_per == g) {
                        double st[CSN];
                        if constexpr (LDSR) {
                            st[0] = (double)lds_r[i - row0];
                            st[1] = (LR == 1) ? 0.0 : (lds_s[i - row0] ? 1.0 : -1.0);
#pragma unroll
                            for (int t = 0; t < AS; ++t) st[2 + t] = (double)lds_a[(i - row0) * AS + t];
                        } else if constexpr (PK) {
                            const float4 r = rec[(size_t)i];
                            st[0] = (double)r.x;
                            st[1] = (double)r.y;
                            st[2] = (double)r.z;
                            st[2 + AS - 1] = (double)r.w;
                        } else {
                            const typename Vec2<T>::type yv = yy2[(size_t)i];
                            st[0] = (double)yv.x;
                            st[1] = (double)yv.y;
#pragma unroll
                            for (int t = 0; t < AS; ++t) st[2 + t] = (double)A[(size_t)i * AS + t];
                        }
#pragma unroll
                        for (int t = 0; t < CSN; ++t) prb_store_granule(cs + t, st[t], ctag);
                    }
                } else if (lane < ncw && (lane % a.G) == g) {
#pragma unroll
                    for (int t = 0; t < CSN; ++t) prb_store_granule(cs + t, 0.0, ctag);
                }
            }
        } else if (worker) {
#pragma unroll
            for (int u = 0; u < PRB_PF; ++u) {
                if constexpr (LDSR) {
                    const int il = cur.row[u] - row0;
                    yh[u] = (double)lds_r[il];
                    yt[u] = (LR == 1) ? 0.0 : (lds_s[il] ? 1.0 : -1.0);
#pragma unroll
                    for (int t = 0; t < AS; ++t) av[u][t] = (double)lds_a[il * AS + t];
                } else if constexpr (PK) {
                    const float4 r = rec[(size_t)cur.row[u]];
                    yh[u] = (double)r.x;
                    yt[u] = (double)r.y;
                    av[u][0] = (double)r.z;
                    av[u][AS - 1] = (double)r.w;
                } else {
                    const size_t i = (size_t)cur.row[u];
                    const typename Vec2<T>::type yv = yy2[i];
                    yh[u] = (double)yv.x;
                    yt[u] = (double)yv.y;
#pragma unroll
                    for (int t = 0; t < AS; ++t) av[u][t] = (double)A[i * AS + t];
                }
            }
            double ag = 0.0, ah = 0.0;
#pragma unroll
            for (int u = 0; u < PRB_PF; ++u) {
                const double dprev = grad_factor<M>(av[u], (double)cur.x[u], p_slot);
                dlast[u] = dprev;
                const double dl = dloss_dev(LOSS, yh[u], yt[u]);
                const bool v = cur.e0 + sub + 4 * u < cur.e1;
                ag += v ? dl * dprev : 0.0;
                ah += v ? dprev * dprev : 0.0;
            }
            for (int e = cur.e0 + sub + 4 * PRB_PF; e < cur.e1; e += 4) {
                const int i = a.erow[e];
                const double x = (double)eval[e];
                double a1[AS], y0, y1;
                if constexpr (LDSR) {
                    y0 = (double)lds_r[i - row0];
                    y1 = (LR == 1) ? 0.0 : (lds_s[i - row0] ? 1.0 : -1.0);
#pragma unroll
                    for (int t = 0; t < AS; ++t) a1[t] = (double)lds_a[(i - row0) * AS + t];
                } else if constexpr (PK) {
                    const float4 r = rec[(size_t)i];
                    y0 = (double)r.x;
                    y1 = (double)r.y;
                    a1[0] = (double)r.z;
                    a1[AS - 1] = (double)r.w;
                } else {
                    const typename Vec2<T>::type yv = yy2[i];
                    y0 = (double)yv.x;
                    y1 = (double)yv.y;
#pragma unroll
                    for (int t = 0; t < AS; ++t) a1[t] = (double)A[(size_t)i * AS + t];
                }
                const double dprev = grad_factor<M>(a1, x, p_slot);
                ag += dloss_dev(LOSS, y0, y1) * dprev;
                ah += dprev * dprev;
            }
            ag += dpp_move_d<0xB1, 0xf>(0.0, ag);
            ah += dpp_move_d<0xB1, 0xf>(0.0, ah);
            ag += dpp_move_d<0x4E, 0xf>(0.0, ag);
            ah += dpp_move_d<0x4E, 0xf>(0.0, ah);
            PRB_WSTAMP(0)
            if (sub == 0 && !((lm0 >> slot) & 1ull)) {
                double* sl = a.slab + (size_t)(b & 1) * a.G * 64 * 2 + ((size_t)g * 64 + slot) * 2;
                const unsigned long long tag = prb_tag(b);
                prb_store_granule(sl, ag, tag);
                prb_store_granule(sl + 1, ah, tag);
            }
        }
        const unsigned long long lmu =
            ((unsigned long long)__builtin_amdgcn_readfirstlane((int)(lm0 >> 32)) << 32) |
            (unsigned)__builtin_amdgcn_readfirstlane((int)lm0);
        if (lmu != 0ull) {
            const int32_t* spb = a.sp + ((size_t)g * a.nb + b) * 65;
            int qi = 0;
            for (unsigned long long mm = lmu; mm != 0ull; mm &= mm - 1, ++qi) {
                const int q = __builtin_ctzll(mm);
                if (worker) {
                    const int le0 = spb[q], le1 = spb[q + 1];
                    const double pq = pold_sched[c0 + q];
                    double lg = 0.0, lh = 0.0;
                    for (int e = le0 + wt; e < le1; e += 256) {
                        const int i = a.erow[e];
                        const double x = (double)eval[e];
                        double a1[Kind<M>::AS], y0, y1;
                        if constexpr (LDSR) {
                            y0 = (double)lds_r[i - row0];
                            y1 = (LR == 1) ? 0.0 : (lds_s[i - row0] ? 1.0 : -1.0);
#pragma unroll
                            for (int t = 0; t < Kind<M>::AS; ++t)
                                a1[t] = (double)lds_a[(i - row0) * Kind<M>::AS + t];
                        } else if constexpr (PK) {
                            const float4 r = rec[(size_t)i];
                            y0 = (double)r.x;
                            y1 = (double)r.y;
                            a1[0] = (double)r.z;
                            a1[Kind<M>::AS - 1] = (double)r.w;
                        } else {
                            const typename Vec2<T>::type yv = yy2[i];
                            y0 = (double)yv.x;
                            y1 = (double)yv.y;
#pragma unroll
                            for (int t = 0; t < Kind<M>::AS; ++t)
                                a1[t] = (double)A[(size_t)i * Kind<M>::AS + t];
                        }
                        const double dprev = grad_factor<M>(a1, x, pq);
                        lg += dloss_dev(LOSS, y0, y1) * dprev;
                        lh += dprev * dprev;
                    }
                    lg = wave_sum(lg);
                    lh = wave_sum(lh);
                    if (lane == 0) {
                        sh_long[(qi * 4 + (wave - 1)) * 2] = lg;
                        sh_long[(qi * 4 + (wave - 1)) * 2 + 1] = lh;
                    }
                }
            }
            __syncthreads();
            if (worker && wt < qi) {
                const int q = nth_set_bit(lmu, wt);
                double tg = 0.0, th = 0.0;
                for (int w4 = 0; w4 < 4; ++w4) {
                    tg += sh_long[(wt * 4 + w4) * 2];
                    th += sh_long[(wt * 4 + w4) * 2 + 1];
                }
                double* sl = a.slab + (size_t)(b & 1) * a.G * 64 * 2 + ((size_t)g * 64 + q) * 2;
                const unsigned long long tag = prb_tag(b);
                prb_store_granule(sl, tg, tag);
                prb_store_granule(sl + 1, th, tag);
            }
        }
        PRB_STAMP(0)
        double p_next = 0.0;
        int n2e0 = 0, n2e1 = 0;
        unsigned long long lm2 = 0ull;
        if (b + 2 < a.nb) prb_load_sp(a, g, b + 2, slot, c3 - c2, n2e0, n2e1, lm2);
        if (worker) {
            PRB_WSTAMP(1)
            if (tid == 64 + 255)
                __hip_atomic_store(sh_go, b + 1, __ATOMIC_RELAXED, __HIP_MEMORY_SCOPE_WORKGROUP);
            if (LDSR && b + 1 < a.nb) {
                prb_load_entries<T>(a, eval, ne0, ne1, sub, nxt, row0);
                if (slot < c2 - c1) p_next = pold_sched[c1 + slot];
            }
            {
                const bool ok =
                    prb_collect_quarter<2>(a, b, part, lane, ncols, sh_quart, kPrbParts);
                if (!ok) *sh_ok = 0;
            }
            PRB_WSTAMP(2)
            if (!LDSR && b + 1 < a.nb) {
                prb_load_entries<T>(a, eval, ne0, ne1, sub, nxt, row0);
                if (slot < c2 - c1) p_next = pold_sched[c1 + slot];
            }
        } else {
            unsigned spins = 0;
            while (__hip_atomic_load(sh_go, __ATOMIC_RELAXED, __HIP_MEMORY_SCOPE_WORKGROUP) <
                       b + 1 &&
                   ++spins < (1u << 24))
                __builtin_amdgcn_s_sleep(1);
            PRB_HSTAMP(1)
            const bool ok = prb_collect_quarter<2>(a, b, part, lane, ncols, sh_quart, kPrbParts);
            if (!ok) *sh_ok = 0;
            PRB_HSTAMP(2)
            if constexpr (CR) {
                if (control) {
                    if (lane < cp1 - cp0) {
                        if (!prb_poll<CSN>(a, a.cslab + ((size_t)(b & 1) * 64 + lane) * CSS,
                                           prb_tag(b), cst))
                            *sh_ok = 0;
                    }
                    const PrbConf<T>* cfa = reinterpret_cast<const PrbConf<T>*>(a.cf);
                    if (lane < cp2 - cp1) cfn = cfa[cp1 + lane];
                    clqn = prb_u4{~0u, ~0u, ~0u, ~0u};
                    if (lane < c2 - c1) clqn = reinterpret_cast<const prb_u4*>(a.clist)[c1 + lane];
                }
            }
        }
        PRB_WSTAMP(3)
        asm volatile("s_waitcnt lgkmcnt(0)\n\ts_barrier" ::: "memory");
        if (!*sh_ok) break;
        PRB_STAMP(3)
        PRB_HSTAMP(7)
        PRB_WSTAMP(4)
        if (control) {
            double tot[2];
#pragma unroll
            for (int v = 0; v < 2; ++v) {
                tot[v] = sh_quart[lane * 2 + v];
#pragma unroll
                for (int w = 1; w < kPrbParts; ++w) tot[v] += sh_quart[(w * 64 + lane) * 2 + v];
            }
            if constexpr (MG) {
                if (!prb_cross_gpu<2>(a, g, b, lane, tot)) *sh_ok = 0;
            }
            const bool valid = lane < ncols;
            bool serial = false;
            if constexpr (CR) serial = (cp1 - cp0) > 0;
            if (!serial) {
                const double res = pcd_chain_lanes<M>(REGC >= 0 ? REGC : reg, lane, ncols - 1, valid,
                                                      pl, tot[0], tot[1], lam, mu, beta, gamma, eta,
                                                      cache, sh_chain);
                const double dl = valid ? (pl - res) : 0.0;
                sh_delta[lane] = dl;
                sh_pold[lane] = pl;
                if (g == 0 && valid) {
                    ps[jl] = res;
                    viol_pos[c0 + lane] = fabs(dl);
                }
            }
            if constexpr (CR) {
                if (serial) {
                    const int nc = cp1 - cp0;
                    const int qa = cfc.qq & 0xff, qb = cfc.qq >> 8;
                    const double xa = (double)cfc.xa, xb = (double)cfc.xb;
                    sh_pold[lane] = pl;
                    sh_delta[lane] = 0.0;
                    asm volatile("s_waitcnt lgkmcnt(0)" ::: "memory");
                    __builtin_amdgcn_wave_barrier();
                    double da[AS + 1], pb = 0.0;
#pragma unroll
                    for (int t = 0; t <= AS; ++t) da[t] = 0.0;
                    if (lane < nc) {
                        const double pa = sh_pold[qa];
                        pb = sh_pold[qb];
                        da[0] = xa;
#pragma unroll
                        for (int t = 1; t <= AS; ++t) da[t] = xa * (cst[1 + t] - pa * da[t - 1]);
                        sh_ce[lane * 2] = dloss_dev(LOSS, cst[0], cst[1]) * da[AS];
                        sh_ce[lane * 2 + 1] = da[AS] * da[AS];
                    }
                    auto after_a = [&](double Da, double* a1, double& y0n) __attribute__((always_inline)) {
#pragma unroll
                        for (int t = 0; t < AS; ++t) a1[t] = (double)(T)(cst[2 + t] - Da * da[t]);
                        y0n = (double)(T)(cst[0] - lam * Da * da[AS]);
                    };
                    asm volatile("s_waitcnt lgkmcnt(0)" ::: "memory");
                    __builtin_amdgcn_wave_barrier();
                    int le[8];
#pragma unroll
                    for (int t = 0; t < 8; ++t) {
                        const unsigned w = clq[t >> 1];
                        le[t] = (int)(short)((t & 1) ? (w >> 16) : (w & 0xffffu));
                    }
                    double g0 = tot[0], h0 = tot[1];
#pragma unroll
                    for (int t = 0; t < 8; ++t)
                        if (le[t] >= 0 && (le[t] >> 8) == 0) {
                            g0 += sh_ce[(le[t] & 0xff) * 2];
                            h0 += sh_ce[(le[t] & 0xff) * 2 + 1];
                        }
                    double cc0[M + 1];
#pragma unroll
                    for (int t = 0; t <= M; ++t) cc0[t] = cache[t];
                    double dl = 0.0, res = pl;
                    for (int round = 0; round <= ncols + 1; ++round) {
                        if (lane < nc) {
                            double a1[AS], y0n;
                            after_a(sh_delta[qa], a1, y0n);
                            const double dAb = grad_factor<M>(a1, xb, pb);
                            sh_cv[lane * 2] = dloss_dev(LOSS, y0n, cst[1]) * dAb;
                            sh_cv[lane * 2 + 1] = dAb * dAb;
                        }
                        asm volatile("s_waitcnt lgkmcnt(0)" ::: "memory");
                        __builtin_amdgcn_wave_barrier();
                        double gq = g0, hq = h0;
#pragma unroll
                        for (int t = 0; t < 8; ++t)
                            if (le[t] >= 0 && (le[t] >> 8) != 0) {
                                gq += sh_cv[(le[t] & 0xff) * 2];
                                hq += sh_cv[(le[t] & 0xff) * 2 + 1];
                            }
#pragma unroll
                        for (int t = 0; t <= M; ++t) cache[t] = cc0[t];
                        res = pcd_chain_lanes<M>(reg, lane, ncols - 1, valid, pl, gq, hq, lam, mu,
                                                 beta, gamma, eta, cache, sh_chain);
                        const double dn = valid ? (pl - res) : 0.0;
                        const bool same = __double_as_longlong(dn) == __double_as_longlong(dl);
                        dl = dn;
                        sh_delta[lane] = dl;
                        asm volatile("s_waitcnt lgkmcnt(0)" ::: "memory");
                        __builtin_amdgcn_wave_barrier();
                        if (__ballot(!same) == 0ull) {
                            if (lane == 0 && g == a.G - 1) {
                                atomicAdd(&g_branch_count[BR_RELAX_STEPS], 1u);
                                atomicAdd(&g_branch_count[BR_RELAX_ROUNDS], (unsigned)(round + 1));
                            }
                            break;
                        }
                    }
                    if (g == 0 && valid) {
                        ps[jl] = res;
                        viol_pos[c0 + lane] = fabs(dl);
                    }
                    if (lane < nc && cfc.row / a.rows_per == g) {
                        const int i = cfc.row;
                        const double Db = sh_delta[qb];
                        double a1[AS], y0n;
                        after_a(sh_delta[qa], a1, y0n);
                        T a2[AS];
                        double db = xb;
#pragma unroll
                        for (int t = 0; t < AS; ++t) {
                            const double dn = xb * (a1[t] - pb * db);
                            a2[t] = (T)(a1[t] - Db * db);
                            db = dn;
                        }
                        const T y0f = (T)(y0n - lam * Db * db);
                        if constexpr (LDSR) {
#pragma unroll
                            for (int t = 0; t < AS; ++t) lds_a[(i - row0) * AS + t] = a2[t];
                            lds_r[i - row0] = y0f;
                        } else if constexpr (PK) {
                            float4 o;
                            o.x = (float)y0f;
                            o.y = (float)cst[1];
                            o.z = (float)a2[0];
                            o.w = (float)a2[AS - 1];
                            rec[(size_t)i] = o;
                        } else {
#pragma unroll
                            for (int t = 0; t < AS; ++t) A[(size_t)i * AS + t] = a2[t];
                            yy[2 * (size_t)i] = y0f;
                        }
                    }
                }
            }
            PRB_STAMP(4)
        }
        asm volatile("s_waitcnt lgkmcnt(0)\n\ts_barrier" ::: "memory");
        PRB_STAMP(5)
        PRB_WSTAMP(5)
        if (slot < ncols) {
            const double upd = sh_delta[slot];
            if (upd != 0.0) {
                const double p_old = sh_pold[slot];
#pragma unroll
                for (int u = 0; u < PRB_PF; ++u) {
                    if (cur.e0 + sub + 4 * u < cur.e1) {
                        const size_t i = (size_t)cur.row[u];
                        const double x = (double)cur.x[u];
                        if constexpr (M == 0) {
                            double yn = yh[u] - lam * av[u][0];
                            double an = av[u][0] / (1.0 + x * p_old);
                            an *= 1.0 + x * (p_old - upd);
                            yn += lam * an;
                            if constexpr (LDSR) {
                                lds_a[i - row0] = (T)an;
                                lds_r[i - row0] = (T)yn;
                            } else {
                                A[i] = (T)an;
                                yy[2 * i] = (T)yn;
                            }
                        } else if constexpr (LDSR) {
                            const int il = (int)i - row0;
                            double dprev = x;
#pragma unroll
                            for (int t = 0; t < AS; ++t) {
                                const double a1 = av[u][t];
                                const double dcur = x * (a1 - p_old * dprev);
                                lds_a[il * AS + t] = (T)(a1 - upd * dprev);
                                dprev = dcur;
                            }
                            lds_r[il] = (T)(yh[u] - lam * upd * dlast[u]);
                        } else if constexpr (PK) {
                            const double d1 = x * (av[u][0] - p_old * x);
                            float4 o;
                            o.x = (float)(yh[u] - lam * upd * dlast[u]);
                            o.y = (float)yt[u];
                            o.z = (float)(av[u][0] - upd * x);
                            o.w = (float)(av[u][AS - 1] - upd * d1);
                            rec[i] = o;
                        } else {
                            double dprev = x;
#pragma unroll
                            for (int t = 1; t < M; ++t) {
                                const double a1 = av[u][t - 1];
                                const double dcur = x * (a1 - p_old * dprev);
                                A[i * (M - 1) + (t - 1)] = (T)(a1 - upd * dprev);
                                dprev = dcur;
                            }
                            yy[2 * i] = (T)(yh[u] - lam * upd * dlast[u]);
                        }
                    }
                }
                for (int e = cur.e0 + sub + 4 * PRB_PF; e < cur.e1; e += 4) {
                    if constexpr (LDSR)
                        pcd_sync_entry_lds<T, M>(a.erow[e] - row0, (double)eval[e], p_old, upd,
                                                 lam, lds_a, lds_r);
                    else if constexpr (PK)
                        pcd_sync_entry_rec((size_t)a.erow[e], (double)eval[e], p_old, upd, lam, rec);
                    else
                        pcd_sync_entry<T, M>((size_t)a.erow[e], (double)eval[e], p_old, upd, lam,
                                             A, yy);
                }
            }
        }
        if (lmu != 0ull && worker) {
            const int32_t* spb = a.sp + ((size_t)g * a.nb + b) * 65;
            for (unsigned long long mm = lmu; mm != 0ull; mm &= mm - 1) {
                const int q = __builtin_ctzll(mm);
                const double upd = sh_delta[q];
                if (upd != 0.0) {
                    const double p_old = sh_pold[q];
                    const int le0 = spb[q], le1 = spb[q + 1];
                    for (int e = le0 + wt; e < le1; e += 256) {
                        if constexpr (LDSR)
                            pcd_sync_entry_lds<T, M>(a.erow[e] - row0, (double)eval[e], p_old,
                                                     upd, lam, lds_a, lds_r);
                        else if constexpr (PK)
                            pcd_sync_entry_rec((size_t)a.erow[e], (double)eval[e], p_old, upd, lam,
                                               rec);
                        else
                            pcd_sync_entry<T, M>((size_t)a.erow[e], (double)eval[e], p_old, upd,
                                                 lam, A, yy);
                    }
                }
            }
        }
        cur = nxt;
        p_slot = p_next;
        ne0 = n2e0;
        ne1 = n2e1;
        lm0 = lm1;
        lm1 = lm2;
        if constexpr (CR) {
            if (control) {
                cp0 = cp1;
                cp1 = cp2;
                cp2 = cp3;
                cp3 = a.cf_ptr[min(b + 4, a.nb)];
                cfc = cfn;
                clq = clqn;
            }
        }
        c0 = c1;
        c1 = c2;
        c2 = c3;
        c3 = c4;
        PRB_WSTAMP(6)
        if constexpr (LDSR)
            asm volatile("s_waitcnt lgkmcnt(0)\n\ts_barrier" ::: "memory");
        else
            __syncthreads();
        PRB_STAMP(6)
        if constexpr (STAMP) {
            if (tid == 320) tprev = clock64();
        }
        PRB_WSTAMP(7)
    }
#undef PRB_STAMP
#undef PRB_HSTAMP
#undef PRB_WSTAMP
    if constexpr (LDSR) {
        __syncthreads();
        const int nr = min(a.rows_per, a.n_rows - row0);
        for (int il = tid; il < nr; il += kPrbThreads) {
            const size_t i = (size_t)(row0 + il);
#pragma unroll
            for (int t = 0; t < AS; ++t) A[i * AS + t] = lds_a[il * AS + t];
            if constexpr (LR == 1)
                yy[2 * i] = (T)((double)lds_r[il] + (double)yy[2 * i + 1]);
            else
                yy[2 * i] = lds_r[il];
        }
    }
    if (STAMP && a.stamps != nullptr && (tid == 0 || tid == 64)) {
#pragma unroll
        for (int q = 0; q < 8; ++q)
            if (tid == 64 || (q != 1 && q != 2 && q != 7))
                a.stamps[(size_t)g * 16 + (tid == 64 ? 8 : 0) + q] = acc[q];
    }
    if (STAMP && a.stamps != nullptr && tid == 320) {
        a.stamps[(size_t)g * 16 + 1] = acc[1];
        a.stamps[(size_t)g * 16 + 2] = acc[2];
        a.stamps[(size_t)g * 16 + 7] = acc[7];
    }
}

template <typename T, int LOSS, int LR, bool MG = false, bool CR = false>
__global__ __launch_bounds__(kPrbThreads) void lin_prb_kernel(
    PrbArgs a, const T* __restrict__ eval, T* __restrict__ yy,
    const double* __restrict__ w_sched, const double* __restrict__ cn_sched,
    double* __restrict__ w, double alpha, double mu, double* __restrict__ viol_pos) {
    extern __shared__ __attribute__((aligned(16))) double dyn_lds[];
    double* sh_delta = dyn_lds + 128;
    double* sh_quart = dyn_lds + 1536;
    int* sh_ok = reinterpret_cast<int*>(dyn_lds + 768);
    int* sh_go = reinterpret_cast<int*>(dyn_lds + 770);
    const typename Vec2<T>::type* yy2 = reinterpret_cast<const typename Vec2<T>::type*>(yy);
    const int g = blockIdx.x;
    const int tid = threadIdx.x, lane = tid & 63, wave = tid >> 6;
    const bool control = wave == 0;
    const bool worker = wave >= 1 && wave <= 4;
    const int part = worker ? wave - 1 : (control ? 4 : wave);
    const int wt = tid - 64;
    const int slot = worker ? (wt >> 2) : 64, sub = wt & 3;
    double* sh_long = dyn_lds + 1024;
    static_assert(LR == 0 || (sizeof(T) == 4 && (LR == 2 || LOSS == LOSS_SQUARED)),
                  "LDS-resident rows: float storage");
    const int row0 = LR ? g * a.rows_per : 0;
    static_assert(!CR || !MG, "relaxed runs: single GPU");
    double* sh_ce = dyn_lds + kPrbLdsFixed;
    double* sh_cv = sh_ce + 64;
    T* lds_r = reinterpret_cast<T*>(dyn_lds + kPrbLdsFixed + (CR ? kPrbLdsCR : 0));
    unsigned char* lds_s = reinterpret_cast<unsigned char*>(lds_r + a.rows_per);
    if constexpr (LR != 0) {
        const int nr = min(a.rows_per, a.n_rows - row0);
        for (int il = tid; il < nr; il += kPrbThreads) {
            const typename Vec2<T>::type yv = yy2[(size_t)(row0 + il)];
            if constexpr (LR == 1) {
                lds_r[il] = (T)((double)yv.x - (double)yv.y);
            } else {
                lds_r[il] = yv.x;
                lds_s[il] = yv.y > (T)0 ? 1 : 0;
            }
        }
        __syncthreads();
    }
    auto row_state = [&](int i, double& y0, double& y1) {
        if constexpr (LR != 0) {
            y0 = (double)lds_r[i - row0];
            y1 = (LR == 1) ? 0.0 : (lds_s[i - row0] ? 1.0 : -1.0);
        } else {
            const typename Vec2<T>::type yv = yy2[(size_t)i];
            y0 = (double)yv.x;
            y1 = (double)yv.y;
        }
    };
    auto row_update = [&](int i, double yold, double dec) {
        if constexpr (LR != 0) lds_r[i - row0] = (T)(yold - dec);
        else yy[2 * (size_t)i] = (T)(yold - dec);
    };
    PrbEntries<T> cur, nxt;
    int c0 = a.bptr[0], c1 = a.bptr[1];
    int c2 = (a.nb > 1) ? a.bptr[2] : c1;
    int c3 = (a.nb > 2) ? a.bptr[3] : c2;
    unsigned long long lm0 = 0ull, lm1 = 0ull;
    {
        int e0, e1;
        prb_load_sp(a, g, 0, slot, c1 - c0, e0, e1, lm0);
        prb_load_entries<T>(a, eval, e0, e1, sub, cur, row0);
    }
    int ne0 = 0, ne1 = 0;
    if (a.nb > 1) prb_load_sp(a, g, 1, slot, c2 - c1, ne0, ne1, lm1);
    if (tid == 0) {
        *sh_ok = 1;
        *sh_go = 0;
    }
    int cp0 = 0, cp1 = 0, cp2 = 0, cp3 = 0;
    PrbConf<T> cfc, cfn;
    cfc.row = cfn.row = 0;
    cfc.qq = cfn.qq = 0;
    cfc.xa = cfc.xb = cfn.xa = cfn.xb = (T)0;
    prb_u4 clq = {~0u, ~0u, ~0u, ~0u}, clqn = {~0u, ~0u, ~0u, ~0u};
    if constexpr (CR) {
        if (control) {
            const PrbConf<T>* cfa = reinterpret_cast<const PrbConf<T>*>(a.cf);
            cp0 = a.cf_ptr[0];
            cp1 = a.cf_ptr[min(1, a.nb)];
            cp2 = a.cf_ptr[min(2, a.nb)];
            cp3 = a.cf_ptr[min(3, a.nb)];
            if (lane < cp1 - cp0) cfc = cfa[cp0 + lane];
            if (lane < c1 - c0) clq = reinterpret_cast<const prb_u4*>(a.clist)[c0 + lane];
        }
    }
    for (int b = 0; b < a.nb; ++b) {
        const int ncols = c1 - c0;
        const int c4 = (b + 4 <= a.nb) ? a.bptr[b + 4] : c3;
        double yh[PRB_PF];
        double wl = 0.0, cnl = 0.0;
        int jl = 0;
        double cst[2] = {0.0, 0.0};
        int n2e0 = 0, n2e1 = 0;
        unsigned long long lm2 = 0ull;
        const unsigned long long lmu =
            ((unsigned long long)__builtin_amdgcn_readfirstlane((int)(lm0 >> 32)) << 32) |
            (unsigned)__builtin_amdgcn_readfirstlane((int)lm0);
        if (lmu != 0ull) {
            const int32_t* spb = a.sp + ((size_t)g * a.nb + b) * 65;
            int qi = 0;
            for (unsigned long long mm = lmu; mm != 0ull; mm &= mm - 1, ++qi) {
                const int q = __builtin_ctzll(mm);
                if (worker) {
                    const int le0 = spb[q], le1 = spb[q + 1];
                    double lg = 0.0;
                    for (int e = le0 + wt; e < le1; e += 256) {
                        double y0, y1;
                        row_state(a.erow[e], y0, y1);
                        lg += dloss_dev(LOSS, y0, y1) * (double)eval[e];
                    }
                    lg = wave_sum(lg);
                    if (lane == 0) sh_long[(qi * 4 + (wave - 1)) * 2] = lg;
                }
            }
            __syncthreads();
            if (worker && wt < qi) {
                const int q = nth_set_bit(lmu, wt);
                double tg = 0.0;
                for (int w4 = 0; w4 < 4; ++w4) tg += sh_long[(wt * 4 + w4) * 2];
                double* sl = a.slab + (size_t)(b & 1) * a.G * 64 * 2 + ((size_t)g * 64 + q) * 2;
                prb_store_granule(sl, tg, prb_tag(b));
            }
        }
        if (control) {
            if (lane < ncols) {
                wl = w_sched[c0 + lane];
                cnl = cn_sched[c0 + lane];
                if (g == 0) jl = a.desc[c0 + lane].j;
            }
            if constexpr (CR) {
                const int nc = cp1 - cp0, ncw = max(nc, cp3 - cp2);
                const unsigned long long ctag = prb_tag(b);
                double* cs = a.cslab + ((size_t)(b & 1) * 64 + lane) * 8;
                if (lane < nc) {
                    if (cfc.row / a.rows_per == g) {
                        double y0, y1;
                        row_state(cfc.row, y0, y1);
                        prb_store_granule(cs, y0, ctag);
                        prb_store_granule(cs + 1, y1, ctag);
                    }
                } else if (lane < ncw && (lane % a.G) == g) {
                    prb_store_granule(cs, 0.0, ctag);
                    prb_store_granule(cs + 1, 0.0, ctag);
                }
            }
        } else if (worker) {
            double yt[PRB_PF];
#pragma unroll
            for (int u = 0; u < PRB_PF; ++u) row_state(cur.row[u], yh[u], yt[u]);
            double ag = 0.0;
#pragma unroll
            for (int u = 0; u < PRB_PF; ++u) {
                const bool v = cur.e0 + sub + 4 * u < cur.e1;
                ag += v ? dloss_dev(LOSS, yh[u], yt[u]) * (double)cur.x[u] : 0.0;
            }
            for (int e = cur.e0 + sub + 4 * PRB_PF; e < cur.e1; e += 4) {
                double y0, y1;
                row_state(a.erow[e], y0, y1);
                ag += dloss_dev(LOSS, y0, y1) * (double)eval[e];
            }
            ag += dpp_move_d<0xB1, 0xf>(0.0, ag);
            ag += dpp_move_d<0x4E, 0xf>(0.0, ag);
            if (sub == 0 && !((lm0 >> slot) & 1ull)) {
                double* sl = a.slab + (size_t)(b & 1) * a.G * 64 * 2 + ((size_t)g * 64 + slot) * 2;
                prb_store_granule(sl, ag, prb_tag(b));
            }
            if (tid == 64 + 255)
                __hip_atomic_store(sh_go, b + 1, __ATOMIC_RELAXED, __HIP_MEMORY_SCOPE_WORKGROUP);
            if (b + 2 < a.nb) prb_load_sp(a, g, b + 2, slot, c3 - c2, n2e0, n2e1, lm2);
            {
                const bool ok =
                    prb_collect_quarter<1>(a, b, part, lane, ncols, sh_quart, kPrbParts);
                if (!ok) *sh_ok = 0;
            }
            if (b + 1 < a.nb) {
                prb_load_entries<T>(a, eval, ne0, ne1, sub, nxt, row0);
            }
        } else if (!control) {
            if (b + 2 < a.nb) prb_load_sp(a, g, b + 2, slot, c3 - c2, n2e0, n2e1, lm2);
            unsigned spins = 0;
            while (__hip_atomic_load(sh_go, __ATOMIC_RELAXED, __HIP_MEMORY_SCOPE_WORKGROUP) <
                       b + 1 &&
                   ++spins < (1u << 24))
                __builtin_amdgcn_s_sleep(1);
            const bool ok = prb_collect_quarter<1>(a, b, part, lane, ncols, sh_quart, kPrbParts);
            if (!ok) *sh_ok = 0;
        }
        if (control) {
            if (b + 2 < a.nb) prb_load_sp(a, g, b + 2, slot, c3 - c2, n2e0, n2e1, lm2);
            {
                unsigned spins = 0;
                while (__hip_atomic_load(sh_go, __ATOMIC_RELAXED, __HIP_MEMORY_SCOPE_WORKGROUP) <
                           b + 1 &&
                       ++spins < (1u << 24))
                    __builtin_amdgcn_s_sleep(1);
                const bool ok =
                    prb_collect_quarter<1>(a, b, part, lane, ncols, sh_quart, kPrbParts);
                if (!ok) *sh_ok = 0;
            }
            if constexpr (CR) {
                if (lane < cp1 - cp0) {
                    if (!prb_poll<2>(a, a.cslab + ((size_t)(b & 1) * 64 + lane) * 8, prb_tag(b), cst))
                        *sh_ok = 0;
                }
                const PrbConf<T>* cfa = reinterpret_cast<const PrbConf<T>*>(a.cf);
                if (lane < cp2 - cp1) cfn = cfa[cp1 + lane];
                clqn = prb_u4{~0u, ~0u, ~0u, ~0u};
                if (lane < c2 - c1) clqn = reinterpret_cast<const prb_u4*>(a.clist)[c1 + lane];
            }
        }
        asm volatile("s_waitcnt lgkmcnt(0)\n\ts_barrier" ::: "memory");
        if (!*sh_ok) break;
        if (control) {
            double tot = sh_quart[lane * 2];
#pragma unroll
            for (int w = 1; w < kPrbParts; ++w) tot += sh_quart[(w * 64 + lane) * 2];
            if constexpr (MG) {
                if (!prb_cross_gpu<1>(a, g, b, lane, &tot)) *sh_ok = 0;
            }
            const bool valid = lane < ncols;
            bool relaxed_step = false;
            if constexpr (CR) relaxed_step = (cp1 - cp0) > 0;
            const double inv = mu * cnl + alpha;
            double upd = 0.0;
            if (!relaxed_step) {
                upd = tot;
                upd += alpha * wl;
                upd /= inv;
                if (!valid) upd = 0.0;
                sh_delta[lane] = upd;
            }
            if constexpr (CR) {
                if (relaxed_step) {
                    const int nc = cp1 - cp0;
                    const int qa = cfc.qq & 0xff, qb = cfc.qq >> 8;
                    const double xa = (double)cfc.xa, xb = (double)cfc.xb;
                    sh_delta[lane] = 0.0;
                    if (lane < nc) sh_ce[lane] = dloss_dev(LOSS, cst[0], cst[1]) * xa;
                    asm volatile("s_waitcnt lgkmcnt(0)" ::: "memory");
                    __builtin_amdgcn_wave_barrier();
                    int le[8];
#pragma unroll
                    for (int t = 0; t < 8; ++t) {
                        const unsigned wv = clq[t >> 1];
                        le[t] = (int)(short)((t & 1) ? (wv >> 16) : (wv & 0xffffu));
                    }
                    double g0 = tot;
#pragma unroll
                    for (int t = 0; t < 8; ++t)
                        if (le[t] >= 0 && (le[t] >> 8) == 0) g0 += sh_ce[le[t] & 0xff];
                    for (int round = 0; round <= ncols + 1; ++round) {
                        if (lane < nc) {
                            const double y0n = (double)(T)(cst[0] - sh_delta[qa] * xa);
                            sh_cv[lane] = dloss_dev(LOSS, y0n, cst[1]) * xb;
                        }
                        asm volatile("s_waitcnt lgkmcnt(0)" ::: "memory");
                        __builtin_amdgcn_wave_barrier();
                        double gq = g0;
#pragma unroll
                        for (int t = 0; t < 8; ++t)
                            if (le[t] >= 0 && (le[t] >> 8) != 0) gq += sh_cv[le[t] & 0xff];
                        double un = gq;
                        un += alpha * wl;
                        un /= inv;
                        if (!valid) un = 0.0;
                        const bool same = __double_as_longlong(un) == __double_as_longlong(upd);
                        upd = un;
                        sh_delta[lane] = upd;
                        asm volatile("s_waitcnt lgkmcnt(0)" ::: "memory");
                        __builtin_amdgcn_wave_barrier();
                        if (__ballot(!same) == 0ull) break;
                    }
                    if (lane < nc && cfc.row / a.rows_per == g) {
                        const double y0n = (double)(T)(cst[0] - sh_delta[qa] * xa);
                        row_update(cfc.row, y0n, sh_delta[qb] * xb);
                    }
                }
            }
            if (g == 0 && valid) {
                w[jl] = wl - upd;
                viol_pos[c0 + lane] = fabs(upd);
            }
        }
        asm volatile("s_waitcnt lgkmcnt(0)\n\ts_barrier" ::: "memory");
        if (slot < ncols) {
            const double upd = sh_delta[slot];
            if (upd != 0.0) {
#pragma unroll
                for (int u = 0; u < PRB_PF; ++u)
                    if (cur.e0 + sub + 4 * u < cur.e1)
                        row_update(cur.row[u], yh[u], upd * (double)cur.x[u]);
                for (int e = cur.e0 + sub + 4 * PRB_PF; e < cur.e1; e += 4) {
                    double y0, y1;
                    row_state(a.erow[e], y0, y1);
                    row_update(a.erow[e], y0, upd * (double)eval[e]);
                }
            }
        }
        if (lmu != 0ull && worker) {
            const int32_t* spb = a.sp + ((size_t)g * a.nb + b) * 65;
            for (unsigned long long mm = lmu; mm != 0ull; mm &= mm - 1) {
                const int q = __builtin_ctzll(mm);
                const double upd = sh_delta[q];
                if (upd != 0.0) {
                    const int le0 = spb[q], le1 = spb[q + 1];
                    for (int e = le0 + wt; e < le1; e += 256) {
                        double y0, y1;
                        row_state(a.erow[e], y0, y1);
                        row_update(a.erow[e], y0, upd * (double)eval[e]);
                    }
                }
            }
        }
        cur = nxt;
        ne0 = n2e0;
        ne1 = n2e1;
        lm0 = lm1;
        lm1 = lm2;
        if constexpr (CR) {
            if (control) {
                cp0 = cp1;
                cp1 = cp2;
                cp2 = cp3;
                cp3 = a.cf_ptr[min(b + 4, a.nb)];
                cfc = cfn;
                clq = clqn;
            }
        }
// ... 271 lines not shown
```

### sparsepoly_amd/engine.py

```python
import collections
import contextlib
import ctypes as C
import threading

import numpy as np
import scipy.sparse as sp

from . import _capi


class SpfmError(RuntimeError):
    pass


def canonical_csc(X):
    if sp.issparse(X):
        Xc = sp.csc_matrix(X, dtype=np.float64, copy=True)
        Xc.sum_duplicates()
        Xc.sort_indices()
    else:
        Xc = sp.csc_matrix(np.asarray(X, dtype=np.float64))
        Xc.sort_indices()
    return Xc

# ... 522 lines not shown
            s = int(s)
            self._check(self._lib.spfm_host_pass_begin(self._h, s))
            reg.compute_cache_pcd(P, degree, s)
            for b in range(len(bp) - 1):
                cols = order[bp[b]:bp[b + 1]]
                nc = len(cols)
                if nc == 0:
                    continue
                self._check(self._lib.spfm_host_step_sums(self._h, b,
                                                          sums.ctypes.data_as(_capi._dp)))
                p_new = np.empty(nc)
                for q in range(nc):
                    j = int(cols[q])
                    p_old = float(P[s, j])
                    inv = mu * sums[q, 1] + beta
                    upd = (lams[s] * sums[q, 0] + beta * p_old) / inv
                    pn = float(reg.prox_cd(p_old - eta * upd, eta * gamma / inv, degree, j))
                    viol += abs(p_old - pn)
                    P[s, j] = pn
                    p_new[q] = pn
                    reg.update_cache_pcd(P, degree, s, j)
                self._check(self._lib.spfm_host_step_apply(
                    self._h, b, p_new.ctypes.data_as(_capi._dp), None))
        dv = C.c_double()
        self._check(self._lib.spfm_host_epoch_end(self._h, C.byref(dv)))
        return viol

    def pbcd_epoch_host(self, reg, Pt, lams, loss, order_idx, degree, beta, gamma, eta):
        mu = self._MU[loss]
        order, bp = self._host_steps()
        k = Pt.shape[1]
        lams = np.asarray(lams, dtype=np.float64)
        self._check(self._lib.spfm_host_epoch_begin(self._h, int(order_idx), int(degree)))
        reg.compute_cache_pbcd(Pt, degree)
        viol = 0.0
        sums = np.empty((int(np.diff(bp).max()), k + 1))
        for b in range(len(bp) - 1):
            cols = order[bp[b]:bp[b + 1]]
            nc = len(cols)
            if nc == 0:
                continue
            self._check(self._lib.spfm_host_step_sums(self._h, b, sums.ctypes.data_as(_capi._dp)))
            p_new = np.empty((nc, k))
            p_old = np.empty((nc, k))
            for q in range(nc):
                j = int(cols[q])
                p_old[q] = Pt[j]
                inv = mu * sums[q, k] + beta
                grad = (sums[q, :k] * lams + beta * Pt[j]) / inv
                pj = Pt[j] - eta * grad
                reg.prox_bcd(pj, eta * gamma / inv, degree, j)
                viol += float(np.abs(p_old[q] - pj).sum())
                Pt[j] = pj
                p_new[q] = pj
                reg.update_cache_pbcd(Pt, degree, j)
            self._check(self._lib.spfm_host_step_apply(
                self._h, b, p_new.ctypes.data_as(_capi._dp), p_old.ctypes.data_as(_capi._dp)))
        dv = C.c_double()
        self._check(self._lib.spfm_host_epoch_end(self._h, C.byref(dv)))
        return viol

    def psgd_epoch(self, degree, alpha, beta, gamma, eta0, learning_rate, power_t, batch_size,
                   indices_samples, fit_linear, it, row_lo=None):
        idx = np.ascontiguousarray(indices_samples, dtype=np.int32)
        itc = C.c_int64(int(it))
        sl = C.c_double()
        lr = (_capi.LEARNING_RATE[learning_rate] if isinstance(learning_rate, str)
              else int(learning_rate))
        if row_lo is not None:
            self._check(self._lib.spfm_psgd_epoch_sharded(
                self._h, int(degree), float(alpha), float(beta), float(gamma), float(eta0), lr,
                float(power_t), int(batch_size), idx.ctypes.data_as(_capi._ip), idx.size,
                int(row_lo), int(bool(fit_linear)), C.byref(itc), C.byref(sl)))
            return sl.value, itc.value
        self._check(self._lib.spfm_psgd_epoch(
            self._h, int(degree), float(alpha), float(beta), float(gamma), float(eta0), lr,
            float(power_t), int(batch_size), idx.ctypes.data_as(_capi._ip), idx.size,
            int(bool(fit_linear)), C.byref(itc), C.byref(sl)))
        return sl.value, itc.value

    @staticmethod
    def comm_unique_id():
        lib = _capi.load()
        buf = C.create_string_buffer(128)
        rc = lib.spfm_comm_unique_id(buf)
        if rc != 0:
            raise SpfmError("spfm_comm_unique_id: %s" % lib.spfm_last_error(None).decode())
        return buf.raw

    def comm_init(self, uid, n_ranks, rank):
        assert len(uid) == 128
        self._check(self._lib.spfm_comm_init(self._h, uid, int(n_ranks), int(rank)))

    def comm_init_shm(self, name, n_ranks, rank):
        self._check(self._lib.spfm_comm_init_shm(self._h, name.encode(), int(n_ranks), int(rank)))

    def peer_alloc(self):
        buf = C.create_string_buffer(64)
        self._check(self._lib.spfm_peer_alloc(self._h, buf))
        return buf.raw

    def peer_connect(self, n_ranks, rank, handles):
        blob = b"".join(handles)
        assert len(blob) == 64 * n_ranks
        self._check(self._lib.spfm_peer_connect(self._h, int(n_ranks), int(rank), blob))

    def profile_enable(self, on=True):
        self._check(self._lib.spfm_profile_enable(self._h, int(bool(on))))

    def profile_reset(self):
        self._check(self._lib.spfm_profile_reset(self._h))

    def profile_get(self, which):
        ms, nl, nz = C.c_double(), C.c_int64(), C.c_int64()
        self._check(self._lib.spfm_profile_get(self._h, int(which), C.byref(ms), C.byref(nl),
                                               C.byref(nz)))
        return ms.value, nl.value, nz.value

    def set_use_graph(self, on):
        self._check(self._lib.spfm_set_use_graph(self._h, int(bool(on))))

    def debug_hop_latency(self, partner=1, rounds=20000):
        ns = C.c_double()
        xcc = (C.c_int32 * 2)()
        self._check(self._lib.spfm_debug_hop_latency(self._h, int(partner), int(rounds),
                                                     C.byref(ns), xcc))
        return ns.value, (xcc[0], xcc[1])

    def debug_exchange_cost(self, groups=64, ncols=37, readers_mod=1, rounds=5000):
        ns = C.c_double()
        self._check(self._lib.spfm_debug_exchange_cost(self._h, int(groups), int(ncols),
                                                       int(readers_mod), int(rounds),
                                                       C.byref(ns)))
        return ns.value

    def debug_prb_stamps(self):
        buf = np.zeros(16 * 512, dtype=np.int64)
        nv = self._lib.spfm_debug_prb_stamps(self._h, buf.ctypes.data_as(_capi._lp), buf.size)
        if nv < 0:
            self._check(nv)
        return buf[:nv].reshape(-1, 16)

    def debug_branch_counts(self, reset=True):
        buf = (C.c_uint32 * 8)()
        self._check(self._lib.spfm_debug_branch_counts(self._h, buf, int(bool(reset))))
        return dict(omegati_clip=buf[0], omegacs_dcache=buf[1], omegacs_cache=buf[2],
                    squaredl21_resum=buf[3], relax_steps=buf[4], relax_rounds=buf[5])

    def debug_stream_probe(self):
        nb = C.c_int64()
        self._check(self._lib.spfm_debug_stream_probe(self._h, C.byref(nb)))
        return nb.value

    def debug_write_probe(self, bytes_per_record):
        nb = C.c_int64()
        self._check(self._lib.spfm_debug_write_probe(self._h, int(bytes_per_record), C.byref(nb)))
        return nb.value

    def get_option(self, key):
        v = C.c_int()
        self._check(self._lib.spfm_get_option(self._h, key.encode(), C.byref(v)))
        return v.value

    def set_option(self, key, value):
        self._check(self._lib.spfm_set_option(self._h, key.encode(), int(value)))
```

Measured before the change: 3.696 epochs/s.

## Add opt-in early LDS gather with precomputed row-hazard flags in persistent PCD kernel

Adds a hazard-flag kernel that marks nonzeros whose row was also touched in the previous batch of the same row block. An EG kernel variant uses these flags to gather the next batch's row state from LDS early, overlapping it with the current batch, and regathers only hazarded entries. The path is gated by the SPFM_PRB_EARLY environment variable and is off by default. One change does run by default: for LDS-resident variants the next batch's entry loads are moved ahead of the quarter collect. The extra template parameter and the live prefetch registers may raise register pressure.

```diff
diff --git a/include/spfm.h b/include/spfm.h
--- a/include/spfm.h
+++ b/include/spfm.h
@@ -129,6 +129,8 @@
 
 int spfm_debug_stream_probe(spfm_handle h, int64_t* bytes_out);
 int spfm_debug_write_probe(spfm_handle h, int bytes_per_record, int64_t* bytes_out);
+int spfm_debug_prb_hazards(spfm_handle h, int32_t* sp, int64_t sp_cap, int32_t* erow,
+                           int64_t erow_cap, uint32_t* hz, int64_t hz_cap, int64_t* sizes);
 int spfm_debug_branch_counts(spfm_handle h, unsigned* out8, int reset);
 
 #define SPFM_GRAM_ANOVA 0
diff --git a/sparsepoly_amd/_capi.py b/sparsepoly_amd/_capi.py
--- a/sparsepoly_amd/_capi.py
+++ b/sparsepoly_amd/_capi.py
@@ -72,6 +72,7 @@
     "spfm_profile_enable", "spfm_profile_get", "spfm_profile_reset", "spfm_set_use_graph",
     "spfm_set_option", "spfm_get_option", "spfm_debug_prb_stamps", "spfm_debug_hop_latency", "spfm_debug_exchange_cost",
     "spfm_debug_branch_counts", "spfm_debug_stream_probe", "spfm_debug_write_probe",
+    "spfm_debug_prb_hazards",
     "spfm_gram_csr_dense", "spfm_gram_csr_csr",
     "spfm_objective_terms", "spfm_set_eval_csr", "spfm_eval_loss",
     "spfm_interaction_stats", "spfm_interaction_topk", "spfm_interaction_list",
@@ -156,6 +157,8 @@
     L.spfm_debug_branch_counts.argtypes = [_h, C.POINTER(C.c_uint32), C.c_int]
     L.spfm_debug_stream_probe.argtypes = [_h, _lp]
     L.spfm_debug_write_probe.argtypes = [_h, C.c_int, _lp]
+    L.spfm_debug_prb_hazards.argtypes = [_h, _ip, C.c_int64, _ip, C.c_int64,
+                                         C.POINTER(C.c_uint32), C.c_int64, _lp]
     L.spfm_gram_csr_dense.argtypes = [_h, C.c_int, C.c_int, C.c_int64, C.c_int32, _lp, _ip, _dp,
                                       C.c_int64, _dp, _dp, C.c_int, C.c_int64, _dp]
     L.spfm_gram_csr_csr.argtypes = [_h, C.c_int, C.c_int, C.c_int64, C.c_int32, _lp, _ip, _dp,
diff --git a/sparsepoly_amd/csrc/spfm_engine.hip.h b/sparsepoly_amd/csrc/spfm_engine.hip.h
--- a/sparsepoly_amd/csrc/spfm_engine.hip.h
+++ b/sparsepoly_amd/csrc/spfm_engine.hip.h
@@ -65,6 +65,8 @@
 hipError_t device_rowblock_stream(int64_t, int32_t, int64_t, int, int, int, const int32_t*,
                                   const int32_t*, const int64_t*, const int32_t*, const uint8_t*,
                                   int32_t*, int32_t*, uint32_t*, int*, int64_t*, hipStream_t);
+hipError_t device_hazard_flags(int, int, int, const int32_t*, const int32_t*, uint32_t*, size_t,
+                               hipStream_t);
 hipError_t device_pb_stream(int64_t, int32_t, int64_t, int, int, int, int, const int32_t*,
                             const int32_t*, const int64_t*, const int32_t*, const int64_t*,
                             const int32_t*, int32_t*, int32_t*, uint8_t*, uint8_t*, hipStream_t);
@@ -170,7 +172,7 @@
     std::mutex mu;
     struct Prb {
         std::string key;
-        DevBuf sp, erow, eval, lmask;
+        DevBuf sp, erow, eval, lmask, hz;
         int has_long = 0;
     };
     struct Pb {
@@ -264,6 +266,9 @@
     bool prb_pack = true;
     int prb_pack_active = 0;
     bool prb_stamp_on = false;
+    bool prb_early = false;
+    DevBuf prb_hz;
+    std::string prb_ckey;
     int wide_min_cols = 110;
     bool wide_stamp_on = false;
     DevBuf wide_stamps;
@@ -349,7 +354,10 @@
         kInvStreams = kInvPrbStream | kInvPbStream | kInvWideStream,
     };
     void invalidate(unsigned mask) {
-        if (mask & kInvPrbStream) prb_ready = false;
+        if (mask & kInvPrbStream) {
+            prb_ready = false;
+            prb_hz.release();
+        }
         if (mask & kInvPbStream) pb_stream_ready = false;
         if (mask & kInvWideStream) wide_ready = false;
         if (mask & kInvRelax) relax_state = 0;
@@ -675,6 +683,9 @@
     int build_prb_stream(int nb_);
 
     PrbArgs prb_args();
+    int ensure_prb_hz();
+    int debug_prb_hazards(int32_t* sp, int64_t sp_cap, int32_t* erow, int64_t erow_cap,
+                          uint32_t* hz, int64_t hz_cap, int64_t* sizes);
 
     bool relax_candidate() const {
         return relax_on && prb_usable() && !dist() && n_batches() > 0 &&
diff --git a/sparsepoly_amd/csrc/spfm_engine_core.hip b/sparsepoly_amd/csrc/spfm_engine_core.hip
--- a/sparsepoly_amd/csrc/spfm_engine_core.hip
+++ b/sparsepoly_amd/csrc/spfm_engine_core.hip
@@ -932,6 +932,10 @@
     }
     spfm_engine* h = new spfm_engine();
     h->device = device_id;
+    {
+        const char* env = std::getenv("SPFM_PRB_EARLY");
+        h->prb_early = env && env[0] == '1';
+    }
     h->dtype = dtype;
     hipDeviceProp_t prop;
     if (hipGetDeviceProperties(&prop, device_id) == hipSuccess) h->devname = prop.gcnArchName;
@@ -1501,6 +1505,12 @@
     return h->debug_stream_probe(bytes_out);
 }
 
+int spfm_debug_prb_hazards(spfm_handle h, int32_t* sp, int64_t sp_cap, int32_t* erow,
+                           int64_t erow_cap, uint32_t* hz, int64_t hz_cap, int64_t* sizes) {
+    SPFM_GUARD(h);
+    return h->debug_prb_hazards(sp, sp_cap, erow, erow_cap, hz, hz_cap, sizes);
+}
+
 int spfm_debug_write_probe(spfm_handle h, int bytes_per_record, int64_t* bytes_out) {
     SPFM_GUARD(h);
     return h->debug_write_probe(bytes_per_record, bytes_out);
diff --git a/sparsepoly_amd/csrc/spfm_engine_pcd.hip b/sparsepoly_amd/csrc/spfm_engine_pcd.hip
--- a/sparsepoly_amd/csrc/spfm_engine_pcd.hip
+++ b/sparsepoly_amd/csrc/spfm_engine_pcd.hip
@@ -149,7 +149,59 @@
     a.clist = nullptr;
     a.cslab = nullptr;
     a.rec = nullptr;
+    a.hz = prb_hz.as<uint32_t>();
     return a;
+}
+
+int spfm_engine::ensure_prb_hz() {
+    if (prb_hz.p) return SPFM_OK;
+    std::unique_lock<std::mutex> cache_lock;
+    StreamCache::Prb* ent = nullptr;
+    if (scache && !prb_ckey.empty()) {
+        cache_lock = std::unique_lock<std::mutex>(scache->mu);
+        for (auto& e : scache->prb)
+            if (e->key == prb_ckey) {
+                ent = e.get();
+                break;
+            }
+        if (ent && ent->hz.p) {
+            prb_hz.share(ent->hz);
+            return SPFM_OK;
+        }
+    }
+    const size_t words = (size_t)((nnz + 31) / 32) + 2;
+    HIPC(prb_hz.alloc(sizeof(uint32_t) * words));
+    const int rows_per = (int)std::max<int64_t>((n + prb_G - 1) / prb_G, 1);
+    HIPC(device_hazard_flags(prb_G, n_batches(), rows_per, prb_sp.as<int32_t>(),
+                             prb_erow.as<int32_t>(), prb_hz.as<uint32_t>(), words, stream));
+    HIPC(hipStreamSynchronize(stream));
+    if (ent) ent->hz.share(prb_hz);
+    return SPFM_OK;
+}
+
+int spfm_engine::debug_prb_hazards(int32_t* sp, int64_t sp_cap, int32_t* erow, int64_t erow_cap,
+                                   uint32_t* hz, int64_t hz_cap, int64_t* sizes) {
+    if (!have_schedule || !prb_usable())
+        FAIL(SPFM_ERR_INVALID, "hazard flags: needs a schedule the 64-column persistent pass can run");
+    int rc = SPFM_DISPATCH(dtype, return ensure_prb<T>());
+    if (rc) return rc;
+    const int rows_per = (int)std::max<int64_t>((n + prb_G - 1) / prb_G, 1);
+    if ((size_t)((rows_per + 31) / 32) * sizeof(uint32_t) > 60 * 1024)
+        FAIL(SPFM_ERR_UNSUPPORTED, "hazard flags: the row block's bitmap does not fit in LDS");
+    rc = ensure_prb_hz();
+    if (rc) return rc;
+    const int64_t nsp = (int64_t)prb_G * n_batches() * 65 + 1;
+    const int64_t nhz = (nnz + 31) / 32 + 2;
+    if (sizes) {
+        sizes[0] = nsp;
+        sizes[1] = nnz;
+        sizes[2] = nhz;
+    }
+    if (sp && sp_cap >= nsp) SPFM_TRY(download(sp, prb_sp.p, (size_t)nsp));
+    if (erow && erow_cap >= nnz) SPFM_TRY(download(erow, prb_erow.p, (size_t)nnz));
+    if (hz && hz_cap >= nhz) SPFM_TRY(download(hz, prb_hz.p, (size_t)nhz));
+    HIPC(hipStreamSynchronize(stream));
+    return SPFM_OK;
 }
 
 PrbArgs spfm_engine::relax_args() {
diff --git a/sparsepoly_amd/csrc/spfm_engine_prb.inc.h b/sparsepoly_amd/csrc/spfm_engine_prb.inc.h
--- a/sparsepoly_amd/csrc/spfm_engine_prb.inc.h
+++ b/sparsepoly_amd/csrc/spfm_engine_prb.inc.h
@@ -112,6 +112,8 @@
 template <typename T>
 int spfm_engine::ensure_prb() {
     if (prb_ready) return SPFM_OK;
+    prb_hz.release();
+    prb_ckey.clear();
     int ncu = 0;
     HIPC(hipDeviceGetAttribute(&ncu, hipDeviceAttributeMultiprocessorCount, device));
     if (prb_G > ncu) prb_G = ncu;
@@ -129,6 +131,7 @@
                 prb_erow.share(e->erow);
                 prb_eval.share(e->eval);
                 prb_lmask.share(e->lmask);
+                prb_hz.share(e->hz);
                 prb_has_long = e->has_long;
                 stream_device_used = 2;
                 hit = true;
@@ -150,6 +153,7 @@
             if (scache->prb.size() > StreamCache::kKeep) scache->prb.pop_back();
         }
     }
+    prb_ckey = ckey;
     if (cache_lock.owns_lock()) cache_lock.unlock();
     HIPC(prb_slab.alloc(sizeof(double) * 2 * ((size_t)prb_G + 1) * 64 * 2));
     HIPC(prb_abort.alloc(sizeof(unsigned) * 4));
@@ -345,6 +349,12 @@
                         (LRV == 1 || y_pm1);
     const size_t lds_bytes = use_lr ? std::max(lds_lr, kPrbLds) : kPrbLds;
     prb_lds_active = use_lr ? LRV : 0;
+    const bool early = use_lr && !relaxed && prb_early;
+    if (early) {
+        rc = ensure_prb_hz();
+        if (rc) return rc;
+        pa.hz = prb_hz.as<uint32_t>();
+    }
     hipLaunchKernelGGL(begin_pass_kernel, dim3(1), dim3(64), 0, stream, c,
                        comp_order.as<int32_t>(), lams.as<double>());
     if (reg != SPFM_REG_L1) {
@@ -377,26 +387,31 @@
         constexpr bool STc = decltype(stamp_tag)::value;
         constexpr int RGc = decltype(reg_tag)::value;
         const size_t lds = (LRc == 1 || LRc == 2) ? lds_bytes : kPrbLds;
-        auto launch = [&](auto mg_tag) -> int {
+        auto launch = [&](auto mg_tag, auto eg_tag) -> int {
             constexpr bool MGc = decltype(mg_tag)::value;
-            HIPC(hipFuncSetAttribute(
-                (const void*)pcd_prb_kernel<T, M, LOSS, LRc, STc, RGc, MGc>,
-                hipFuncAttributeMaxDynamicSharedMemorySize, (int)lds));
-            if (!resident_ok((const void*)pcd_prb_kernel<T, M, LOSS, LRc, STc, RGc, MGc>,
-                             kPrbThreads, lds, prb_G))
-                return kNotResident;
-            hipLaunchKernelGGL((pcd_prb_kernel<T, M, LOSS, LRc, STc, RGc, MGc>),
-                               dim3(launch_groups(prb_G)), dim3(kPrbThreads), lds, stream, c, pa, prb_eval.as<T>(),
-                               A.as<T>(), (size_t)n * Kind<M>::AS, yy.as<T>(),
-                               prow_old.as<double>(), Po, d, reg, cb, mu, beta, gamma, eta,
-                               prb_viol.as<double>());
+            constexpr bool EGc = decltype(eg_tag)::value;
+            auto* fn = pcd_prb_kernel<T, M, LOSS, LRc, STc, RGc, MGc, false, EGc>;
+            HIPC(hipFuncSetAttribute((const void*)fn, hipFuncAttributeMaxDynamicSharedMemorySize,
+                                     (int)lds));
+            if (!resident_ok((const void*)fn, kPrbThreads, lds, prb_G)) return kNotResident;
+            hipLaunchKernelGGL(fn, dim3(launch_groups(prb_G)), dim3(kPrbThreads), lds, stream, c,
+                               pa, prb_eval.as<T>(), A.as<T>(), (size_t)n * Kind<M>::AS,
+                               yy.as<T>(), prow_old.as<double>(), Po, d, reg, cb, mu, beta, gamma,
+                               eta, prb_viol.as<double>());
             return SPFM_OK;
         };
-        if constexpr (STc) {
-            return launch(std::false_type{});
-        } else {
-            return pa.n_ranks > 1 ? launch(std::true_type{}) : launch(std::false_type{});
-        }
+        auto launch_mg = [&](auto eg_tag) -> int {
+            if constexpr (STc) {
+                return launch(std::false_type{}, eg_tag);
+            } else {
+                return pa.n_ranks > 1 ? launch(std::true_type{}, eg_tag)
+                                      : launch(std::false_type{}, eg_tag);
+            }
+        };
+        if constexpr (LRc == 1 || LRc == 2) {
+            if (early) return launch_mg(std::true_type{});
+        }
+        return launch_mg(std::false_type{});
     };
     using std::integral_constant;
     int lrc = SPFM_OK;
diff --git a/sparsepoly_amd/csrc/spfm_ingest.hip b/sparsepoly_amd/csrc/spfm_ingest.hip
--- a/sparsepoly_amd/csrc/spfm_ingest.hip
+++ b/sparsepoly_amd/csrc/spfm_ingest.hip
@@ -268,6 +268,42 @@
     return done(hipSuccess);
 }
 
+__global__ __launch_bounds__(256) void rbs_hazard_kernel(int G, int nb, int rows_per,
+                                                          const int32_t* __restrict__ sp,
+                                                          const int32_t* __restrict__ erow,
+                                                          uint32_t* __restrict__ hz) {
+    extern __shared__ uint32_t hz_rows[];
+    const int g = (int)(blockIdx.x / (unsigned)nb), b = (int)(blockIdx.x % (unsigned)nb);
+    if (b == 0) return;
+    const size_t at = ((size_t)g * nb + b) * 65;
+    const int p0 = sp[at - 65], p1 = sp[at], p2 = sp[at + 65];
+    if (p1 == p2 || p0 == p1) return;
+    const int nw = (rows_per + 31) >> 5;
+    const int row0 = g * rows_per;
+    for (int w = threadIdx.x; w < nw; w += blockDim.x) hz_rows[w] = 0u;
+    __syncthreads();
+    for (int e = p0 + (int)threadIdx.x; e < p1; e += blockDim.x) {
+        const int il = erow[e] - row0;
+        if (il >= 0 && il < rows_per) atomicOr(&hz_rows[il >> 5], 1u << (il & 31));
+    }
+    __syncthreads();
+    for (int e = p1 + (int)threadIdx.x; e < p2; e += blockDim.x) {
+        const int il = erow[e] - row0;
+        if (il >= 0 && il < rows_per && ((hz_rows[il >> 5] >> (il & 31)) & 1u))
+            atomicOr(&hz[e >> 5], 1u << (e & 31));
+    }
+}
+
+hipError_t device_hazard_flags(int G, int nb, int rows_per, const int32_t* sp, const int32_t* erow,
+                               uint32_t* hz, size_t hz_words, hipStream_t stream) {
+    hipError_t e;
+    if ((e = hipMemsetAsync(hz, 0, sizeof(uint32_t) * hz_words, stream)) != hipSuccess) return e;
+    if (nb < 2 || G < 1) return hipSuccess;
+    const size_t lds = sizeof(uint32_t) * (size_t)((rows_per + 31) >> 5);
+    hipLaunchKernelGGL(rbs_hazard_kernel, dim3((unsigned)((size_t)G * nb)), dim3(256), lds, stream,
+                       G, nb, rows_per, sp, erow, hz);
+    return hipGetLastError();
+}
 
 
 __global__ void sb_step_of_kernel(int32_t d, int nb, const int32_t* __restrict__ order,
diff --git a/sparsepoly_amd/csrc/spfm_prb.hip.h b/sparsepoly_amd/csrc/spfm_prb.hip.h
--- a/sparsepoly_amd/csrc/spfm_prb.hip.h
+++ b/sparsepoly_amd/csrc/spfm_prb.hip.h
@@ -27,6 +27,7 @@
     const int16_t* clist;
     double* cslab;
     void* rec;
+    const uint32_t* hz;
 };
 
 template <typename T>
@@ -309,7 +310,7 @@
 
 constexpr int kPrbLdsCR = 256;
 template <typename T, int M, int LOSS, int LR, bool STAMP = false, int REGC = -1, bool MG = false,
-          bool CR = false>
+          bool CR = false, bool EG = false>
 __global__ __launch_bounds__(kPrbThreads) void pcd_prb_kernel(
     const Ctl* __restrict__ ctl, PrbArgs a, const T* __restrict__ eval, T* __restrict__ A_all,
     size_t a_stride, T* __restrict__ yy, const double* __restrict__ pold_sched,
@@ -346,6 +347,7 @@
                   "LDS-resident rows: float storage, one or two cache values per row");
     static_assert(!PK || (sizeof(T) == 4 && Kind<M>::AS == 2),
                   "packed row records: float storage, two cache values per row");
+    static_assert(!EG || (LDSR && !CR), "early gather: rows in LDS, strict steps");
     float4* __restrict__ rec = reinterpret_cast<float4*>(a.rec);
     constexpr int AS = Kind<M>::AS;
     static_assert(!CR || (M >= 2 && !MG && !STAMP), "relaxed runs: degree >= 2, single GPU");
@@ -407,6 +409,33 @@
                 clq = reinterpret_cast<const prb_u4*>(a.clist)[c0 + lane];
         }
     }
+    double av_n[PRB_PF][Kind<M>::AS], yh_n[PRB_PF], yt_n[PRB_PF], dlast_n[PRB_PF], dl_n[PRB_PF];
+#pragma unroll
+    for (int u = 0; u < PRB_PF; ++u) {
+#pragma unroll
+        for (int t = 0; t < Kind<M>::AS; ++t) av_n[u][t] = 0.0;
+        yh_n[u] = yt_n[u] = dlast_n[u] = dl_n[u] = 0.0;
+    }
+    unsigned hzc = 0xfu, hzn = 0u;
+    uint32_t hzw0 = 0u, hzw1 = 0u;
+    auto gather_lds = [&](const PrbEntries<T>& en, double p, double (*av_)[Kind<M>::AS],
+                          double* yh_, double* yt_, double* dlast_,
+                          double* dl_) __attribute__((always_inline)) {
+#pragma unroll
+        for (int u = 0; u < PRB_PF; ++u) {
+            const int il = en.row[u] - row0;
+            yh_[u] = (double)lds_r[il];
+            yt_[u] = (LR == 1) ? 0.0 : (lds_s[il] ? 1.0 : -1.0);
+#pragma unroll
+            for (int t = 0; t < Kind<M>::AS; ++t) av_[u][t] = (double)lds_a[il * Kind<M>::AS + t];
+        }
+#pragma unroll
+        for (int u = 0; u < PRB_PF; ++u) {
+            dlast_[u] = grad_factor<M>(av_[u], (double)en.x[u], p);
+            dl_[u] = dloss_dev(LOSS, yh_[u], yt_[u]);
+        }
+    };
+    (void)gather_lds;
     long long acc[8] = {0, 0, 0, 0, 0, 0, 0, 0};
     long long tprev = STAMP ? clock64() : 0;
 #define PRB_STAMP(k)                        \
@@ -485,9 +514,39 @@
                 }
             }
         } else if (worker) {
+            double dlv[PRB_PF];
+            if constexpr (EG) {
+                bool need[PRB_PF], any = false;
+#pragma unroll
+                for (int u = 0; u < PRB_PF; ++u) {
+                    need[u] = ((hzc >> u) & 1u) && (cur.e0 + sub + 4 * u < cur.e1);
+                    any = any || need[u];
+#pragma unroll
+                    for (int t = 0; t < AS; ++t) av[u][t] = av_n[u][t];
+                    yh[u] = yh_n[u];
+                    yt[u] = yt_n[u];
+                    dlast[u] = dlast_n[u];
+                    dlv[u] = dl_n[u];
+                }
+                if (__ballot(any) != 0ull) {
+                    double av_l[PRB_PF][AS], yh_l[PRB_PF], yt_l[PRB_PF], dlast_l[PRB_PF],
+                        dl_l[PRB_PF];
+                    gather_lds(cur, p_slot, av_l, yh_l, yt_l, dlast_l, dl_l);
+#pragma unroll
+                    for (int u = 0; u < PRB_PF; ++u) {
+#pragma unroll
+                        for (int t = 0; t < AS; ++t) av[u][t] = need[u] ? av_l[u][t] : av[u][t];
+                        yh[u] = need[u] ? yh_l[u] : yh[u];
+                        yt[u] = need[u] ? yt_l[u] : yt[u];
+                        dlast[u] = need[u] ? dlast_l[u] : dlast[u];
+                        dlv[u] = need[u] ? dl_l[u] : dlv[u];
+                    }
+                }
+            }
 #pragma unroll
             for (int u = 0; u < PRB_PF; ++u) {
-                if constexpr (LDSR) {
+                if constexpr (EG) {
+                } else if constexpr (LDSR) {
                     const int il = cur.row[u] - row0;
                     yh[u] = (double)lds_r[il];
                     yt[u] = (LR == 1) ? 0.0 : (lds_s[il] ? 1.0 : -1.0);
@@ -511,9 +570,15 @@
             double ag = 0.0, ah = 0.0;
 #pragma unroll
             for (int u = 0; u < PRB_PF; ++u) {
-                const double dprev = grad_factor<M>(av[u], (double)cur.x[u], p_slot);
-                dlast[u] = dprev;
-                const double dl = dloss_dev(LOSS, yh[u], yt[u]);
+                double dprev, dl;
+                if constexpr (EG) {
+                    dprev = dlast[u];
+                    dl = dlv[u];
+                } else {
+                    dprev = grad_factor<M>(av[u], (double)cur.x[u], p_slot);
+                    dlast[u] = dprev;
+                    dl = dloss_dev(LOSS, yh[u], yt[u]);
+                }
                 const bool v = cur.e0 + sub + 4 * u < cur.e1;
                 ag += v ? dl * dprev : 0.0;
                 ah += v ? dprev * dprev : 0.0;
@@ -630,6 +695,10 @@
             if (LDSR && b + 1 < a.nb) {
                 prb_load_entries<T>(a, eval, ne0, ne1, sub, nxt, row0);
                 if (slot < c2 - c1) p_next = pold_sched[c1 + slot];
+                if constexpr (EG) {
+                    hzw0 = a.hz[ne0 >> 5];
+                    hzw1 = a.hz[(ne0 >> 5) + 1];
+                }
             }
             {
                 const bool ok =
@@ -671,6 +740,17 @@
         PRB_STAMP(3)
         PRB_HSTAMP(7)
         PRB_WSTAMP(4)
+        if constexpr (EG) {
+            if (worker && b + 1 < a.nb && (wave - 1) * 16 < c2 - c1) {
+                gather_lds(nxt, p_next, av_n, yh_n, yt_n, dlast_n, dl_n);
+                const unsigned long long win =
+                    ((((unsigned long long)hzw1) << 32) | (unsigned long long)hzw0) >> (nxt.e0 & 31);
+                hzn = 0u;
+#pragma unroll
+                for (int u = 0; u < PRB_PF; ++u)
+                    hzn |= (unsigned)((win >> (sub + 4 * u)) & 1ull) << u;
+            }
+        }
         if (control) {
             double tot[2];
 #pragma unroll
@@ -908,6 +988,7 @@
         }
         cur = nxt;
         p_slot = p_next;
+        hzc = hzn;
         ne0 = n2e0;
         ne1 = n2e1;
         lm0 = lm1;
@@ -1137,12 +1218,13 @@
             if (tid == 64 + 255)
                 __hip_atomic_store(sh_go, b + 1, __ATOMIC_RELAXED, __HIP_MEMORY_SCOPE_WORKGROUP);
             if (b + 2 < a.nb) prb_load_sp(a, g, b + 2, slot, c3 - c2, n2e0, n2e1, lm2);
+            if (LR != 0 && b + 1 < a.nb) prb_load_entries<T>(a, eval, ne0, ne1, sub, nxt, row0);
             {
                 const bool ok =
                     prb_collect_quarter<1>(a, b, part, lane, ncols, sh_quart, kPrbParts);
                 if (!ok) *sh_ok = 0;
             }
-            if (b + 1 < a.nb) {
+            if (LR == 0 && b + 1 < a.nb) {
                 prb_load_entries<T>(a, eval, ne0, ne1, sub, nxt, row0);
             }
         } else if (!control) {
diff --git a/sparsepoly_amd/engine.py b/sparsepoly_amd/engine.py
--- a/sparsepoly_amd/engine.py
+++ b/sparsepoly_amd/engine.py
@@ -698,6 +698,21 @@
         self._check(self._lib.spfm_debug_stream_probe(self._h, C.byref(nb)))
         return nb.value
 
+    def debug_prb_hazards(self):
+        sizes = np.zeros(3, dtype=np.int64)
+        self._check(self._lib.spfm_debug_prb_hazards(self._h, None, 0, None, 0, None, 0,
+                                                     sizes.ctypes.data_as(_capi._lp)))
+        sp = np.zeros(int(sizes[0]), dtype=np.int32)
+        erow = np.zeros(max(int(sizes[1]), 1), dtype=np.int32)
+        hz = np.zeros(int(sizes[2]), dtype=np.uint32)
+        self._check(self._lib.spfm_debug_prb_hazards(
+            self._h, sp.ctypes.data_as(_capi._ip), sp.size, erow.ctypes.data_as(_capi._ip),
+            erow.size, hz.ctypes.data_as(C.POINTER(C.c_uint32)), hz.size,
+            sizes.ctypes.data_as(_capi._lp)))
+        ne = int(sizes[1])
+        bits = ((hz[np.arange(ne) >> 5] >> (np.arange(ne) & 31).astype(np.uint32)) & 1)
+        return sp, erow[:ne], bits.astype(bool)
+
     def debug_write_probe(self, bytes_per_record):
         nb = C.c_int64()
         self._check(self._lib.spfm_debug_write_probe(self._h, int(bytes_per_record), C.byref(nb)))
```

After: 3.707 epochs/s, median of 6. No clear change (+0.3%).
